# Kuntz-Lab/interactive-rate-tendons

Hardware: AMD Instinct MI355X
Metric: FK+collision checks/sec (3-tendon, 256^3 voxel env) (higher is better)
Workload: dtype f64

## Files before the change

### interactive-rate-tendons_amd/csrc/edge_queue_kernel.hpp

```cpp
#pragma once
#include "verdict_kernel.hpp"
#define TRK_EDGE_DEVICE_ONLY
#include "edge_kernel.hpp"

namespace trk {

__device__ __forceinline__ uint32_t eq_load(const uint32_t *p) { return __hip_atomic_load(p, __ATOMIC_RELAXED, __HIP_MEMORY_SCOPE_AGENT); }
__device__ __forceinline__ void eq_wait_vm() { asm volatile("s_waitcnt vmcnt(0)" ::: "memory"); }
__device__ __forceinline__ void eq_release() {
  eq_wait_vm();
  __builtin_amdgcn_fence(__ATOMIC_RELEASE, "agent");
  eq_wait_vm();
}
__device__ __forceinline__ void eq_acquire() {
  __builtin_amdgcn_fence(__ATOMIC_ACQUIRE, "agent");
  eq_wait_vm();
}
__device__ __forceinline__ int eq_bcast(int v) { return __builtin_amdgcn_readfirstlane(v); }
struct EqClock {
  unsigned long long t;
  __device__ __forceinline__ void start() { t = wall_clock64(); }
  __device__ __forceinline__ void lap(uint32_t *ctl, int word) {
    const unsigned long long n = wall_clock64();
    if (threadIdx.x == 0) __hip_atomic_fetch_add((unsigned long long *)(ctl + word), n - t, __ATOMIC_RELAXED, __HIP_MEMORY_SCOPE_AGENT);
    t = n;
  }
};

constexpr int EQ_GROUP_IV = EQ_MAX_CAND;
#define EQ_MASK(i) (((unsigned long long *)vlds)[(i)])
#define EQ_I(i) (((int32_t *)vlds)[(i)])
#define EQ_U(i) (((uint32_t *)vlds)[(i)])
constexpr int EQ_PRE = 2 * EQ_GROUP_IV / 32, EQ_EOF = EQ_PRE + 64, EQ_BASEOF = EQ_EOF + 64, EQ_CNT = EQ_BASEOF + 64, EQ_DOM = EQ_CNT + 64,
              EQ_NBASE = EQ_DOM + 64, EQ_FILL = EQ_NBASE + 64, EQ_RELW = EQ_FILL + 64;
#define EQ_REL(i) (((double *)vlds)[EQ_RELW / 2 + (i)])

__device__ __forceinline__ int eq_stash_base(int NM) { return VLay<true>::MS + 4 * NM * 64 + SIG_LDS_WORDS; }

__device__ __forceinline__ void signatures_differ_lane2(const uint32_t *__restrict__ ra, const uint32_t *__restrict__ rm,
                                                        const uint32_t *__restrict__ rb, int P, int &fp, int &fd) {
  constexpr int U = 6;
  fp = 0; fd = 0;
  bool open_p = true, open_d = true;
  for (int k = (P - 1) >> 2; k >= 0 && (open_p || open_d); k -= U) {
    uint4 va[U], vm[U], vb[U];
#pragma unroll
    for (int u = 0; u < U; u++) {
      const int kk = k - u >= 0 ? k - u : 0;
      va[u] = *reinterpret_cast<const uint4 *>(ra + 4 * kk);
      vm[u] = *reinterpret_cast<const uint4 *>(rm + 4 * kk);
      vb[u] = *reinterpret_cast<const uint4 *>(rb + 4 * kk);
    }
#pragma unroll
    for (int u = 0; u < U; u++) {
      if (k - u < 0) break;
      const uint32_t wa[4] = {va[u].x, va[u].y, va[u].z, va[u].w}, wm[4] = {vm[u].x, vm[u].y, vm[u].z, vm[u].w},
                     wb[4] = {vb[u].x, vb[u].y, vb[u].z, vb[u].w};
#pragma unroll
      for (int w = 3; w >= 0; w--) {
        if (4 * (k - u) + w >= P) continue;
        const uint32_t a = wa[w], m = wm[w], b = wb[w];
        const uint32_t mx = m & 1023u, my = (m >> 10) & 1023u, mz = (m >> 20) & 1023u;
        const uint32_t px = (a & 1023u) + 1u - mx, py = ((a >> 10) & 1023u) + 1u - my, pz = ((a >> 20) & 1023u) + 1u - mz;
        const uint32_t dx = mx + 1u - (b & 1023u), dy = my + 1u - ((b >> 10) & 1023u), dz = mz + 1u - ((b >> 20) & 1023u);
        const int ep = ((a | m) & SIG_BAD) ? 2 : ((px > 2u || py > 2u || pz > 2u) ? 1 : 0);
        const int ed = ((m | b) & SIG_BAD) ? 2 : ((dx > 2u || dy > 2u || dz > 2u) ? 1 : 0);
        if (open_p && ep) { fp = ep; open_p = false; }
        if (open_d && ed) { fd = ed; open_d = false; }
      }
    }
  }
}

__device__ __forceinline__ bool eq_claim(const EdgeQueueArgs &q, int &pos, int &n) {
  const int lane = threadIdx.x;
  uint32_t *ctl = q.ctl;
  uint32_t seen = 0xffffffffu;
  unsigned idle = 0;
  int patience = 0;
  for (;;) {
    int r_fl = 0, r_pos = 0, r_n = 0, r_end = 0, r_wait = 0;
    uint32_t d = 0, t = 0;
    if (lane == 0) {
      r_fl = (int)eq_load(ctl + EQ_FLAGS);
      d = eq_load(ctl + EQ_DONE);
      eq_wait_vm();
      t = eq_load(ctl + EQ_TAIL);
      const int avail = (int)eq_load(ctl + EQ_AVAIL);
      const int out = (int)(t - d);
      const int want = out >= 4096 ? 64 : (out < 128 ? 1 : out >> 6);
      if (!r_fl && avail > 0 && avail < want && patience < 24) { patience++; r_wait = 1; }
      else if (!r_fl && avail > 0) {
        const int old = (int)__hip_atomic_fetch_add((int *)(ctl + EQ_AVAIL), -want, __ATOMIC_RELAXED, __HIP_MEMORY_SCOPE_AGENT);
        const int got = old >= want ? want : (old > 0 ? old : 0);
        if (got < want) __hip_atomic_fetch_add((int *)(ctl + EQ_AVAIL), want - got, __ATOMIC_RELAXED, __HIP_MEMORY_SCOPE_AGENT);
        if (got > 0) { r_pos = (int)__hip_atomic_fetch_add(ctl + EQ_HEAD, (uint32_t)got, __ATOMIC_RELAXED, __HIP_MEMORY_SCOPE_AGENT); r_n = got; }
      } else if (!r_fl && d == t) r_end = 1;
    }
    if (eq_bcast(r_fl) || eq_bcast(r_end)) return false;
    if (eq_bcast(r_wait)) { __builtin_amdgcn_s_sleep(16); continue; }
    n = eq_bcast(r_n);
    if (n > 0) { pos = eq_bcast(r_pos); return true; }
    d = (uint32_t)eq_bcast((int)d); t = (uint32_t)eq_bcast((int)t);
    if (d + t != seen) { seen = d + t; idle = 0; }
    else if (++idle > (1u << 19)) {
      if (lane == 0) __hip_atomic_fetch_or(ctl + EQ_FLAGS, EQF_STUCK, __ATOMIC_RELAXED, __HIP_MEMORY_SCOPE_AGENT);
      return false;
    }
    __builtin_amdgcn_s_sleep(127);
    if (idle > 16) __builtin_amdgcn_s_sleep(127);
    if (idle > 256) { __builtin_amdgcn_s_sleep(127); __builtin_amdgcn_s_sleep(127); }
  }
}

template <int N, bool ROT>
__global__ __launch_bounds__(64, (N <= TRK_VERDICT_TWO_WAVE_MAXN ? 2 : 1)) void fk_edge_queue(
    RobotK K, const double *__restrict__ tab, const StepK *__restrict__ steps, int nsteps,
    const VerdictArgs *__restrict__ va, const EdgeQueueArgs *__restrict__ qa, const FusedSweepArgs *__restrict__ sa) {
  const int lane = threadIdx.x;
  EqClock clk;
  clk.start();
#ifdef TRK_EQ_TRACE
  int tr_round = 0;
#endif
  for (;;) {
    int zero = 0;
    asm volatile("" : "+s"(zero));
    const EdgeQueueArgs &q = qa[zero];
    int h = 0, cnt = 0;
    if (!eq_claim(q, h, cnt)) break;
    clk.lap(q.ctl, EQ_T_CLAIM);
    const bool live = lane < cnt;
    const int slot = h + lane;
    int e_lane = -1;
    {
      bool bail = false;
      if (live) {
        const uint32_t *flag = (const uint32_t *)q.sample_edge + slot;
        unsigned spins = 0;
        while ((e_lane = (int)eq_load(flag)) < 0) {
          if (eq_load(q.ctl + EQ_FLAGS) != 0u) { bail = true; break; }
          if (++spins > (1u << 22)) {
            __hip_atomic_fetch_or(q.ctl + EQ_FLAGS, EQF_STUCK, __ATOMIC_RELAXED, __HIP_MEMORY_SCOPE_AGENT);
            bail = true; break;
          }
          __builtin_amdgcn_s_sleep(8);
        }
      }
      if (__any(bail)) break;
    }
    eq_acquire();
    clk.lap(q.ctl, EQ_T_READY);

    PointSweep<false, true> ps;
    ps.va = va;
    ps.dn_prev = 0.0f; ps.sph_state = 0u;
    ps.qhead = 0; ps.qcount = 0; ps.active = false;
    ps.P = va->P; ps.CH = va->CH; ps.NM = va->NM; ps.Kl = (ps.P - 1 + ps.CH - 1) / ps.CH; ps.ms_next = 0; ps.ms_k = 0;
    ps.sigst.init(); ps.sig_row_of = -1; ps.sig_first_row = 0; ps.sig_row0 = h; ps.sig_cnt = cnt;
    __syncthreads();
    VL_U(VLay<true>::HIT + lane) = 0u; VL_U(VLay<true>::INPREV + lane) = 0u; VL_F(VLay<true>::DIST + lane) = 0.0f;
    __syncthreads();
    const int S = K.state_size;
    const double *st_eff = q.states + ((int64_t)h - (int64_t)blockIdx.x * 64) * S;
    const int64_t n_eff = (int64_t)blockIdx.x * 64 + cnt;
    {
      const int sb = eq_stash_base(ps.NM);
      VL_I(sb + lane) = e_lane;
      if (lane == 0) { VL_I(sb + 64) = h; VL_I(sb + 65) = cnt; VL_U(sb + 66) = (uint32_t)clk.t; VL_U(sb + 67) = (uint32_t)(clk.t >> 32); }
    }
    FkLane<N> fl_;
    {
      FkOut out{nullptr, nullptr, nullptr, nullptr, nullptr, nullptr, nullptr, nullptr, nullptr, nullptr};
      fk_uniform_body<N, ROT, false, false>(st_eff, n_eff, 0, K, tab, steps, nsteps, out, ps, nullptr, &fl_);
    }
    ps.template sig_finish<false>();
    ps.finish();
    while (ps.qcount > 0) ps.flush();
    __syncthreads();
    LaneVerdict lv;
    int e2, h2, cnt2;
    {
      const VerdictArgs a = *va;
      const int sb = eq_stash_base(a.NM);
      e2 = VL_I(sb + lane); h2 = VL_I(sb + 64); cnt2 = VL_I(sb + 65);
      clk.t = (unsigned long long)VL_U(sb + 66) | ((unsigned long long)VL_U(sb + 67) << 32);
      lv = verdict_decide<N, false, true>(a, fl_, lane < cnt2);
    }
    const bool live2 = lane < cnt2;
    int zero2 = 0;
    asm volatile("" : "+s"(zero2));
    const EdgeQueueArgs &q2 = qa[zero2];
#ifdef TRK_EQ_TRACE
    const uint32_t tr_start = (uint32_t)clk.t;
    const unsigned long long tr_w0 = wall_clock64(), tr_c0 = (unsigned long long)clock64();
    { float x = (float)lane; for (int i = 0; i < 2000; i++) x = __builtin_fmaf(x, 1.0000001f, 0.5f); if (x == 12345.678f) asm volatile("s_nop 0"); }
    const unsigned long long tr_w1 = wall_clock64(), tr_c1 = (unsigned long long)clock64();
    const uint32_t tr_mhz = tr_w1 > tr_w0 ? (uint32_t)((tr_c1 - tr_c0) * 100ull / (tr_w1 - tr_w0)) : 0u;
#endif
    clk.lap(q2.ctl, EQ_T_FK);
#ifdef TRK_EQ_TRACE
    const uint32_t tr_fk = (uint32_t)clk.t;
#endif
    if (__any(lv.pending)) {
      __syncthreads();
      const double *st2 = q2.states + ((int64_t)h2 - (int64_t)blockIdx.x * 64) * K.state_size;
      const int64_t n2 = (int64_t)blockIdx.x * 64 + cnt2;
      fk_uniform_body<N, ROT, false, false>(st2, n2, q2.fb_ld, K, tab, steps, nsteps, q2.fb_out, NoPointHook(), nullptr, nullptr);
      __syncthreads();
      const FusedSweepArgs fa = *sa;
      bool exact = false;
      sweep_body<false>(q2.fb_in, n2, q2.fb_ld, fa.P, fa.CH, fa.NM, K, fa.g, fa.grid, fa.near_grid, 1, fa.debug, nullptr, nullptr, nullptr, &exact);
      __syncthreads();
      const uint32_t npend = (uint32_t)__popcll(__ballot(lv.pending));
      if (lane == 0) __hip_atomic_fetch_add(q2.ctl + EQ_PENDING, npend, __ATOMIC_RELAXED, __HIP_MEMORY_SCOPE_AGENT);
      if (lv.pending) lv.valid = exact;
      clk.lap(q2.ctl, EQ_T_EXACT);
    }

    if (live2 && !lv.valid) q2.edge_ok[e2] = 0u;
    eq_release();
    int old = 0;
    if (live2) old = __hip_atomic_fetch_add(q2.remaining + e2, -1, __ATOMIC_RELAXED, __HIP_MEMORY_SCOPE_AGENT);
    bool fin = live2 && old == 1;
    bool stop = false;
    EqClock sub = clk;
    sub.lap(q2.ctl, EQ_T_F0);
    if (__any(fin)) {
      eq_acquire();
      {
        const uint32_t nfin = (uint32_t)__popcll(__ballot(fin));
        if (lane == 0) __hip_atomic_fetch_add(q2.ctl + EQ_FINISHED, nfin, __ATOMIC_RELAXED, __HIP_MEMORY_SCOPE_AGENT);
      }
      int base_l = 0, ncand_l = 0;
      double rel_l = 0.0;
      if (fin && q2.edge_ok[e2] != 0u) {
        base_l = q2.lvl_base[e2]; ncand_l = q2.lvl_cnt[e2]; rel_l = q2.rel[e2];
        if (2 * ncand_l > EQ_MAX_CAND) {
          __hip_atomic_fetch_or(q2.ctl + EQ_FLAGS, EQF_DEEP, __ATOMIC_RELAXED, __HIP_MEMORY_SCOPE_AGENT);
          ncand_l = 0; stop = true;
        }
      }
      stop = __any(stop);
      sub.lap(q2.ctl, EQ_T_F1);
      unsigned long long todo = __ballot(ncand_l > 0);
      const int P = q2.P;
      const int S2 = q2.sk.S;
      while (todo && !stop) {
        const bool mine = (todo >> lane) & 1ull;
        int pre = mine ? ncand_l : 0;
#pragma unroll
        for (int o = 1; o < 64; o <<= 1) { const int v = __shfl_up(pre, o, 64); if (lane >= o) pre += v; }
        const bool in_group = mine && pre <= EQ_GROUP_IV;
        const unsigned long long gm = __ballot(in_group);
        todo &= ~gm;
        const int n_g = in_group ? ncand_l : 0;
        int ex = n_g;
#pragma unroll
        for (int o = 1; o < 64; o <<= 1) { const int v = __shfl_up(ex, o, 64); if (lane >= o) ex += v; }
        const int T = __shfl(ex, 63, 64);
        ex -= n_g;
        __syncthreads();
        EQ_I(EQ_PRE + lane) = ex; EQ_I(EQ_EOF + lane) = e2; EQ_I(EQ_BASEOF + lane) = base_l;
        EQ_I(EQ_CNT + lane) = 0; EQ_I(EQ_DOM + lane) = 0; EQ_I(EQ_FILL + lane) = 0;
        EQ_REL(lane) = rel_l;
        __syncthreads();
        if (lane == 0) __hip_atomic_fetch_add(q2.ctl + EQ_CAND, (uint32_t)(2 * T), __ATOMIC_RELAXED, __HIP_MEMORY_SCOPE_AGENT);
        auto owner_of = [&](int g) {
          int lo = 0;
#pragma unroll
          for (int st = 32; st > 0; st >>= 1) if (EQ_I(EQ_PRE + lo + st) <= g) lo += st;
          return lo;
        };
        for (int g0 = 0; g0 < T; g0 += 64) {
          const int g = g0 + lane;
          bool emit_p = false, emit_d = false;
          if (g < T) {
#pragma clang fp contract(off)
            const int ow = owner_of(g);
            const int sm = EQ_I(EQ_BASEOF + ow) + (g - EQ_I(EQ_PRE + ow));
            const EdgeIv iv = q2.iv[sm];
            const double tm = (iv.ta + iv.tb) / 2;
            int fp, fd;
            signatures_differ_lane2(q2.sig + (int64_t)iv.sa * q2.sig_stride, q2.sig + (int64_t)sm * q2.sig_stride,
                                    q2.sig + (int64_t)iv.sb * q2.sig_stride, P, fp, fd);
            if (fp == 2 || fd == 2) atomicOr(&EQ_U(EQ_DOM + ow), 1u);
            const double relv = EQ_REL(ow);
            emit_p = fp == 1 && (tm - iv.ta) > relv;
            emit_d = fd == 1 && (iv.tb - tm) > relv;
            const uint32_t k = (emit_p ? 1u : 0u) + (emit_d ? 1u : 0u);
            if (k) atomicAdd(&EQ_U(EQ_CNT + ow), k);
          }
          const unsigned long long mp = __ballot(emit_p), md = __ballot(emit_d);
          if (lane == 0) { EQ_MASK(2 * (g0 >> 6)) = mp; EQ_MASK(2 * (g0 >> 6) + 1) = md; }
        }
        __syncthreads();
        sub.lap(q2.ctl, EQ_T_F2);
        int total_l = 0;
        if (in_group) {
          if (EQ_I(EQ_DOM + lane)) {
            q2.edge_ok[e2] = 0u;
            __hip_atomic_fetch_add(q2.ctl + EQ_DOMAIN, 1u, __ATOMIC_RELAXED, __HIP_MEMORY_SCOPE_AGENT);
          } else total_l = EQ_I(EQ_CNT + lane);
        }
        int nex = total_l;
#pragma unroll
        for (int o = 1; o < 64; o <<= 1) { const int v = __shfl_up(nex, o, 64); if (lane >= o) nex += v; }
        const int Tnew = __shfl(nex, 63, 64);
        nex -= total_l;
        if (Tnew == 0) continue;
        int nb = 0;
        if (lane == 0) nb = (int)__hip_atomic_fetch_add(q2.ctl + EQ_TAIL, (uint32_t)Tnew, __ATOMIC_RELAXED, __HIP_MEMORY_SCOPE_AGENT);
        nb = eq_bcast(nb);
        if (nb + Tnew > q2.slot_hi) {
          if (lane == 0) __hip_atomic_fetch_or(q2.ctl + EQ_FLAGS, EQF_OVERFLOW, __ATOMIC_RELAXED, __HIP_MEMORY_SCOPE_AGENT);
          stop = true; break;
        }
        EQ_I(EQ_NBASE + lane) = nb + nex;
        if (total_l > 0) {
          q2.lvl_base[e2] = nb + nex; q2.lvl_cnt[e2] = total_l; q2.remaining[e2] = total_l;
          q2.nfk[e2] += total_l;
        }
        __syncthreads();
        for (int g0 = 0; g0 < T; g0 += 64) {
          const unsigned long long mp = EQ_MASK(2 * (g0 >> 6)), md = EQ_MASK(2 * (g0 >> 6) + 1);
          const bool ep = (mp >> lane) & 1ull, ed = (md >> lane) & 1ull;
          if (ep || ed) {
#pragma clang fp contract(off)
            const int g = g0 + lane;
            const int ow = owner_of(g);
            if (!EQ_I(EQ_DOM + ow)) {
              const int sm = EQ_I(EQ_BASEOF + ow) + (g - EQ_I(EQ_PRE + ow));
              const EdgeIv iv = q2.iv[sm];
              const double tm = (iv.ta + iv.tb) / 2;
              const int e = EQ_I(EQ_EOF + ow);
              int ns = EQ_I(EQ_NBASE + ow) + (int)atomicAdd(&EQ_U(EQ_FILL + ow), (ep ? 1u : 0u) + (ed ? 1u : 0u));
              if (ed) {
                q2.iv[ns] = EdgeIv{e, sm, iv.sb, 0, tm, iv.tb};
                const double t2 = (tm + iv.tb) / 2;
                interpolate_state_dev(q2.sk, q2.A + (int64_t)e * S2, q2.B + (int64_t)e * S2, t2, q2.states + (int64_t)ns * S2);
                ns++;
              }
              if (ep) {
                q2.iv[ns] = EdgeIv{e, iv.sa, sm, 0, iv.ta, tm};
                const double t2 = (iv.ta + tm) / 2;
                interpolate_state_dev(q2.sk, q2.A + (int64_t)e * S2, q2.B + (int64_t)e * S2, t2, q2.states + (int64_t)ns * S2);
              }
            }
          }
        }
        sub.lap(q2.ctl, EQ_T_F3);
        eq_release();
        for (int g = lane; g < Tnew; g += 64) {
          const int ns = nb + g;
          __hip_atomic_store((uint32_t *)q2.sample_edge + ns, (uint32_t)q2.iv[ns].e, __ATOMIC_RELAXED, __HIP_MEMORY_SCOPE_AGENT);
        }
        eq_wait_vm();
        if (lane == 0) __hip_atomic_fetch_add((int *)(q2.ctl + EQ_AVAIL), Tnew, __ATOMIC_RELAXED, __HIP_MEMORY_SCOPE_AGENT);
        sub.lap(q2.ctl, EQ_T_F4);
      }
    }
// ... 20 lines not shown
```

### interactive-rate-tendons_amd/csrc/fk_inst.hip

```cpp
#include "fk_launch.hpp"
#include "fk_kernel.hpp"
#if TRK_INST_KIND == 1
#include "fk_retract_kernel.hpp"
#elif TRK_INST_KIND == 2
#include "fused_kernel.hpp"
#elif TRK_INST_KIND == 3
#include "verdict_kernel.hpp"
#elif TRK_INST_KIND == 4
#define TRK_WITH_RETRACT_VERDICT
#include "fk_retract_kernel.hpp"
#include "verdict_kernel.hpp"
#elif TRK_INST_KIND == 5
#include "edge_queue_kernel.hpp"
#elif TRK_INST_KIND == 6
#define TRK_LOADED_WITH_INTEGRATOR
#include "fk_loaded_kernel.hpp"
#endif

namespace trk {

#if TRK_INST_KIND == 5
template <> void launch_fk_edge_queue<TRK_INST_N>(const FkLaunch &a, const VerdictArgs *va, size_t lds, const EdgeQueueArgs *qa,
                                                  const FusedSweepArgs *sweep, unsigned waves) {
  if (a.rotation)
    hipLaunchKernelGGL((fk_edge_queue<TRK_INST_N, true>), dim3(waves), dim3(64), lds, a.stream, a.K, a.d_tab, a.d_steps, a.n_steps, va, qa, sweep);
  else
    hipLaunchKernelGGL((fk_edge_queue<TRK_INST_N, false>), dim3(waves), dim3(64), lds, a.stream, a.K, a.d_tab, a.d_steps, a.n_steps, va, qa, sweep);
}
template <> int fk_edge_queue_waves_per_cu<TRK_INST_N>(bool rotation, size_t lds) {
  int nb = 0;
  const hipError_t e = rotation ? hipOccupancyMaxActiveBlocksPerMultiprocessor(&nb, fk_edge_queue<TRK_INST_N, true>, 64, lds)
                                : hipOccupancyMaxActiveBlocksPerMultiprocessor(&nb, fk_edge_queue<TRK_INST_N, false>, 64, lds);
  return e == hipSuccess ? nb : 0;
}
#endif

#if TRK_INST_KIND == 5
#elif TRK_INST_KIND == 6
template <bool ROT, bool WR>
static void go(const FkLaunch &a, const LoadedIn &in) {
  const unsigned grid = (unsigned)((a.n + 63) / 64);
  hipLaunchKernelGGL((fk_loaded_uniform<TRK_INST_N, ROT, WR>), dim3(grid), dim3(64), 0, a.stream, a.d_states, a.n, a.ld, a.K,
                     a.d_tab, a.d_steps, a.n_steps, a.out, in);
}
template <> void launch_fk_loaded<TRK_INST_N>(const FkLaunch &a, const LoadedIn &in) {
  if (a.rotation) { if (a.write_R) go<true, true>(a, in); else go<true, false>(a, in); }
  else            { if (a.write_R) go<false, true>(a, in); else go<false, false>(a, in); }
}
template <> void launch_shoot_start<TRK_INST_N>(const FkLaunch &a, const double *guess, double *vu) {
  const unsigned grid = (unsigned)((a.n + 63) / 64);
  hipLaunchKernelGGL((shoot_start<TRK_INST_N>), dim3(grid), dim3(64), 0, a.stream, a.d_states, a.n, a.K, a.d_tab, guess, vu);
}
#elif TRK_INST_KIND == 4
template <bool ROT, bool SPH, bool SIG>
static void go(const FkLaunch &a, const VerdictArgs *va, size_t lds) {
  const unsigned grid = (unsigned)((a.n + 63) / 64);
  const RetractHandoff ho{a.d_handoff, a.handoff_ld};
  hipLaunchKernelGGL((fk_retract_prologue<TRK_INST_N, ROT>), dim3(grid), dim3(64), 0, a.stream, a.d_states, a.n, a.K, a.d_poly, a.d_tab, a.d_steps,
                     a.n_steps, a.k_first, a.d_tgrid, a.d_hl, a.d_perm, ho);
  hipLaunchKernelGGL((fk_verdict_retract<TRK_INST_N, ROT, SPH, SIG>), dim3(grid), dim3(64), lds, a.stream, a.d_states, a.n, a.K, a.d_poly,
                     a.d_tab, a.d_steps, a.n_steps, a.k_first, a.d_tgrid, a.d_hl, a.out.tips, va, ho);
}
template <bool SPH, bool SIG>
static void go_rot(const FkLaunch &a, const VerdictArgs *va, size_t lds) {
  if (a.rotation) go<true, SPH, SIG>(a, va, lds); else go<false, SPH, SIG>(a, va, lds);
}
template <> void launch_fk_verdict_retract<TRK_INST_N>(const FkLaunch &a, const VerdictArgs *va, size_t lds, bool spheres, bool with_sig) {
  if (spheres) { if (with_sig) go_rot<true, true>(a, va, lds); else go_rot<true, false>(a, va, lds); }
  else         { if (with_sig) go_rot<false, true>(a, va, lds); else go_rot<false, false>(a, va, lds); }
}
template <bool ROT>
static void go_list(const FkLaunch &a, const FusedSweepArgs *sweep, size_t lds, const int32_t *list, const uint32_t *count) {
  const unsigned grid = (unsigned)((a.n + 63) / 64);
  hipLaunchKernelGGL((fk_sweep_retract_list<TRK_INST_N, ROT>), dim3(grid), dim3(64), lds, a.stream, a.d_states, a.n, a.ld, a.K,
                     a.d_poly, a.d_tab, a.d_steps, a.n_steps, a.k_first, a.d_tgrid, a.d_hl, a.out, sweep, list, count);
}
template <> void launch_fk_sweep_retract_list<TRK_INST_N>(const FkLaunch &a, const FusedSweepArgs *sweep, size_t lds, const int32_t *list,
                                                          const uint32_t *count) {
  if (a.rotation) go_list<true>(a, sweep, lds, list, count); else go_list<false>(a, sweep, lds, list, count);
}
#elif TRK_INST_KIND == 3
template <bool ROT, bool SPH, bool SIG>
static void go(const FkLaunch &a, const VerdictArgs *va, size_t lds) {
  const unsigned grid = (unsigned)((a.n + 63) / 64);
  hipLaunchKernelGGL((fk_verdict<TRK_INST_N, ROT, SPH, SIG>), dim3(grid), dim3(64), lds, a.stream, a.d_states, a.n, a.K, a.d_tab, a.d_steps,
                     a.n_steps, a.out.tips, va);
}
template <bool SPH, bool SIG>
static void go_rot(const FkLaunch &a, const VerdictArgs *va, size_t lds) {
  if (a.rotation) go<true, SPH, SIG>(a, va, lds); else go<false, SPH, SIG>(a, va, lds);
}
template <> void launch_fk_verdict<TRK_INST_N>(const FkLaunch &a, const VerdictArgs *va, size_t lds, bool spheres, bool with_sig) {
  if (spheres) { if (with_sig) go_rot<true, true>(a, va, lds); else go_rot<true, false>(a, va, lds); }
  else         { if (with_sig) go_rot<false, true>(a, va, lds); else go_rot<false, false>(a, va, lds); }
}
#elif TRK_INST_KIND == 2
template <bool ROT>
static void go_list(const FkLaunch &a, const FusedSweepArgs *sweep, size_t lds, const int32_t *list, const uint32_t *count) {
  const unsigned grid = (unsigned)((a.n + 63) / 64);
  hipLaunchKernelGGL((fk_sweep_fused_list<TRK_INST_N, ROT>), dim3(grid), dim3(64), lds, a.stream, a.d_states, a.n, a.ld, a.K,
                     a.d_tab, a.d_steps, a.n_steps, a.out, sweep, list, count);
}
template <> void launch_fk_sweep_fused_list<TRK_INST_N>(const FkLaunch &a, const FusedSweepArgs *sweep, size_t lds, const int32_t *list,
                                                        const uint32_t *count) {
  if (a.rotation) go_list<true>(a, sweep, lds, list, count); else go_list<false>(a, sweep, lds, list, count);
}
template <bool ROT>
static void go(const FkLaunch &a, const FusedSweepArgs *sweep, size_t lds) {
  const unsigned grid = (unsigned)((a.n + 63) / 64);
  hipLaunchKernelGGL((fk_sweep_fused<TRK_INST_N, ROT>), dim3(grid), dim3(64), lds, a.stream, a.d_states, a.n, a.ld, a.K,
                     a.d_tab, a.d_steps, a.n_steps, a.out, sweep);
}
template <> void launch_fk_sweep_fused<TRK_INST_N>(const FkLaunch &a, const FusedSweepArgs *sweep, size_t lds) {
  if (a.rotation) go<true>(a, sweep, lds); else go<false>(a, sweep, lds);
}
#else
#if TRK_INST_KIND == 1
template <bool ROT, bool WR>
static void go(const FkLaunch &a) {
  const unsigned grid = (unsigned)((a.n + 63) / 64);
  hipLaunchKernelGGL((fk_rk4_batch_retract<TRK_INST_N, ROT, WR>), dim3(grid), dim3(64), 0, a.stream, a.d_states, a.n, a.ld, a.K,
                     a.d_poly, a.d_tab, a.d_steps, a.n_steps, a.k_first, a.d_tgrid, a.d_hl, a.out, a.d_perm, a.d_wave_k_begin);
}
template <> void launch_fk_retract<TRK_INST_N>(const FkLaunch &a) {
#else
template <bool ROT, bool WR>
static void go(const FkLaunch &a) {
  const unsigned grid = (unsigned)((a.n + 63) / 64);
  hipLaunchKernelGGL((fk_rk4_batch_uniform<TRK_INST_N, ROT, WR>), dim3(grid), dim3(64), 0, a.stream, a.d_states, a.n, a.ld, a.K,
                     a.d_tab, a.d_steps, a.n_steps, a.out);
}
template <> void launch_fk_uniform<TRK_INST_N>(const FkLaunch &a) {
#endif
  if (a.rotation) { if (a.write_R) go<true, true>(a); else go<true, false>(a); }
  else            { if (a.write_R) go<false, true>(a); else go<false, false>(a); }
}
#endif

}
```

### interactive-rate-tendons_amd/csrc/fk_kernel.hpp

```cpp
#pragma once
#include <type_traits>
#include <hip/hip_runtime.h>
#include "tr_types.hpp"

namespace trk {

#ifndef TRK_NEWTON_STEPS
#define TRK_NEWTON_STEPS 1
#endif
__device__ __forceinline__ double fast_rcp(double x) {
  double y = __builtin_amdgcn_rcp(x);
  double e = __builtin_fma(-x, y, 1.0);
  y = __builtin_fma(e, y, y);
#if TRK_NEWTON_STEPS > 1
  e = __builtin_fma(-x, y, 1.0);
  y = __builtin_fma(e, y, y);
#endif
  return y;
}
__device__ __forceinline__ double fast_rsqrt(double x) {
  double y = __builtin_amdgcn_rsq(x);
  double hx = 0.5 * x;
  double t = __builtin_fma(-hx * y, y, 0.5);
  y = __builtin_fma(y, t, y);
#if TRK_NEWTON_STEPS > 1
  t = __builtin_fma(-hx * y, y, 0.5);
  y = __builtin_fma(y, t, y);
#endif
  return y;
}

struct NoLoad {
  __device__ __forceinline__ void operator()(double &, double &, double &, double &, double &, double &) const {}
};

template <int N, class Route, class Load = NoLoad>
__device__ __forceinline__ void strain_rates_routed(const double v[3], const double u[3], const double (&tau)[N],
                                                    Route &&route, const RobotK &K,
                                                    double dv[3], double du[3], double (&sdot)[N], const Load &load = Load()) {
#pragma clang fp contract(fast)
  double Axx = K.ks0, Axy = 0, Axz = 0, Ayy = K.ks0, Ayz = 0, Azz = K.ks2, Z = 0;
  double B00 = 0, B01 = 0, B02 = 0, B10 = 0, B11 = 0, B12 = 0, B20 = 0, B21 = 0, B22 = 0;
  double Hxx = K.kb0, Hxy = 0, Hxz = 0, Hyy = K.kb0, Hyz = 0, Hzz = K.kb2;
  double ax = 0, ay = 0, az = 0, bx = 0, by = 0, bz = 0;
#pragma unroll
  for (int j = 0; j < N; j++) {
    double r6[6];
    route(j, r6);
    const double rx = r6[0], ry = r6[1];
    const double rdx = r6[2], rdy = r6[3];
    const double rddx = r6[4], rddy = r6[5];
    const double pdx = (v[0] + rdx) - u[2] * ry;
    const double pdy = (v[1] + rdy) + u[2] * rx;
    const double pdz = __builtin_fma(u[0], ry, __builtin_fma(-u[1], rx, v[2]));
    const double sxy = __builtin_fma(pdy, pdy, pdx * pdx), s2 = __builtin_fma(pdz, pdz, sxy);
    const double rs = fast_rsqrt(s2);
    sdot[j] = s2 * rs;
    const double cs2 = -tau[j] * rs;
    const double rs2 = rs * rs, c = cs2 * rs2;
    const double qx = c * pdx, qy = c * pdy, qz = c * pdz;
    Axx += qx * pdx; Axy += qx * pdy; Axz += qx * pdz; Ayy += qy * pdy; Ayz += qy * pdz;
    Z += cs2;
    const double ez = __builtin_fma(rx, pdy, -(ry * pdx));
    const double gx = ry * qz, gy = -rx * qz, gz = c * ez;
    B00 += gx * pdx; B01 += gx * pdy;
    B10 += gy * pdx; B11 += gy * pdy;
    B20 += gz * pdx; B21 += gz * pdy; B22 += gz * pdz;
    Hxz += gx * ez; Hyz += gy * ez; Hzz += gz * ez;
    const double mxy = c * sxy, mx = mxy * rx, my = mxy * ry;
    Hxx -= my * ry; Hxy += mx * ry; Hyy -= mx * rx;
    const double t1 = cs2 * rx, t2 = cs2 * ry;
    Hzz -= t1 * rx; Hzz -= t2 * ry;
    {
#pragma clang fp contract(off)
      Azz -= mxy; B02 -= my; B12 += mx; B20 += t2; B21 -= t1;
    }
    const double hx = pdx + rdx, hy = pdy + rdy, hz = pdz;
    const double wx = __builtin_fma(u[1], hz, __builtin_fma(-u[2], hy, rddx));
    const double wy = __builtin_fma(u[2], hx, __builtin_fma(-u[0], hz, rddy));
    const double wz = __builtin_fma(u[0], hy, -(u[1] * hx));
    const double pw = __builtin_fma(pdz, wz, __builtin_fma(pdy, wy, pdx * wx));
    const double kp = pw * rs2;
    const double px = __builtin_fma(pdx, kp, -wx), py = __builtin_fma(pdy, kp, -wy), pz = __builtin_fma(pdz, kp, -wz);
    ax = __builtin_fma(cs2, px, ax); ay = __builtin_fma(cs2, py, ay); az = __builtin_fma(cs2, pz, az);
    bx = __builtin_fma(t2, pz, bx); by = __builtin_fma(-t1, pz, by); bz = __builtin_fma(t1, py, __builtin_fma(-t2, px, bz));
  }
#define TRK_FMA __builtin_fma
  const double svx = K.ks0 * v[0], svy = K.ks0 * v[1], svz = K.ks2 * (v[2] - 1.0);
  const double dku = K.dkb * u[2], w = TRK_FMA(-K.ks0, v[2], svz);
  double cx = TRK_FMA(-u[1], dku, TRK_FMA(-v[1], w, -bx));
  double cy = TRK_FMA(u[0], dku, TRK_FMA(v[0], w, -by));
  double cz = -bz;
  double dx = TRK_FMA(u[2], svy, TRK_FMA(-u[1], svz, -ax));
  double dy = TRK_FMA(u[0], svz, TRK_FMA(-u[2], svx, -ay));
  double dz = TRK_FMA(u[1], svx, TRK_FMA(-u[0], svy, -az));
  load(cx, cy, cz, dx, dy, dz);
  const double m00 = Axx - Z, m01 = Axy, m02 = Axz, m11 = Ayy - Z, m12 = Ayz, m22 = Azz;
#ifndef TRK_SOLVE_SCHUR
  {
#pragma clang fp contract(off)
    const double n00 = Hxx, n01 = Hxy, n02 = Hxz, n11 = Hyy, n12 = Hyz, n22 = Hzz;
    const double p0 = m00;
    const double r0 = fast_rcp(p0);
    const double w10 = m01, l10 = w10 * r0;
    const double w20 = m02, l20 = w20 * r0;
    const double w30 = B00, l30 = w30 * r0;
    const double w40 = B10, l40 = w40 * r0;
    const double w50 = B20, l50 = w50 * r0;
    const double p1 = TRK_FMA(-l10, w10, m11);
    const double r1 = fast_rcp(p1);
    const double w21 = TRK_FMA(-l20, w10, m12), l21 = w21 * r1;
    const double w31 = TRK_FMA(-l30, w10, B01), l31 = w31 * r1;
    const double w41 = TRK_FMA(-l40, w10, B11), l41 = w41 * r1;
    const double w51 = TRK_FMA(-l50, w10, B21), l51 = w51 * r1;
    const double p2 = TRK_FMA(-l21, w21, TRK_FMA(-l20, w20, m22));
    const double r2 = fast_rcp(p2);
    const double w32 = TRK_FMA(-l31, w21, TRK_FMA(-l30, w20, B02)), l32 = w32 * r2;
    const double w42 = TRK_FMA(-l41, w21, TRK_FMA(-l40, w20, B12)), l42 = w42 * r2;
    const double w52 = TRK_FMA(-l51, w21, TRK_FMA(-l50, w20, B22)), l52 = w52 * r2;
    const double p3 = TRK_FMA(-l32, w32, TRK_FMA(-l31, w31, TRK_FMA(-l30, w30, n00)));
    const double r3 = fast_rcp(p3);
    const double w43 = TRK_FMA(-l42, w32, TRK_FMA(-l41, w31, TRK_FMA(-l40, w30, n01))), l43 = w43 * r3;
    const double w53 = TRK_FMA(-l52, w32, TRK_FMA(-l51, w31, TRK_FMA(-l50, w30, n02))), l53 = w53 * r3;
    const double p4 = TRK_FMA(-l43, w43, TRK_FMA(-l42, w42, TRK_FMA(-l41, w41, TRK_FMA(-l40, w40, n11))));
    const double r4 = fast_rcp(p4);
    const double w54 = TRK_FMA(-l53, w43, TRK_FMA(-l52, w42, TRK_FMA(-l51, w41, TRK_FMA(-l50, w40, n12)))), l54 = w54 * r4;
    const double p5 = TRK_FMA(-l54, w54, TRK_FMA(-l53, w53, TRK_FMA(-l52, w52, TRK_FMA(-l51, w51, TRK_FMA(-l50, w50, n22)))));
    const double r5 = fast_rcp(p5);
    const double y0 = dx;
    const double y1 = TRK_FMA(-l10, y0, dy);
    const double y2 = TRK_FMA(-l21, y1, TRK_FMA(-l20, y0, dz));
    const double y3 = TRK_FMA(-l32, y2, TRK_FMA(-l31, y1, TRK_FMA(-l30, y0, cx)));
    const double y4 = TRK_FMA(-l43, y3, TRK_FMA(-l42, y2, TRK_FMA(-l41, y1, TRK_FMA(-l40, y0, cy))));
    const double y5 = TRK_FMA(-l54, y4, TRK_FMA(-l53, y3, TRK_FMA(-l52, y2, TRK_FMA(-l51, y1, TRK_FMA(-l50, y0, cz)))));
    const double x5 = y5 * r5;
    const double x4 = TRK_FMA(-l54, x5, y4 * r4);
    const double x3 = TRK_FMA(-l53, x5, TRK_FMA(-l43, x4, y3 * r3));
    const double x2 = TRK_FMA(-l52, x5, TRK_FMA(-l42, x4, TRK_FMA(-l32, x3, y2 * r2)));
    const double x1 = TRK_FMA(-l51, x5, TRK_FMA(-l41, x4, TRK_FMA(-l31, x3, TRK_FMA(-l21, x2, y1 * r1))));
    const double x0 = TRK_FMA(-l50, x5, TRK_FMA(-l40, x4, TRK_FMA(-l30, x3, TRK_FMA(-l20, x2, TRK_FMA(-l10, x1, y0 * r0)))));
    dv[0] = x0; dv[1] = x1; dv[2] = x2; du[0] = x3; du[1] = x4; du[2] = x5;
  }
#else
  const double c00 = TRK_FMA(m11, m22, -(m12 * m12)), c01 = TRK_FMA(m02, m12, -(m01 * m22)), c02 = TRK_FMA(m01, m12, -(m02 * m11));
  const double c11 = TRK_FMA(m00, m22, -(m02 * m02)), c12 = TRK_FMA(m01, m02, -(m00 * m12)), c22 = TRK_FMA(m00, m11, -(m01 * m01));
  const double idet = fast_rcp(TRK_FMA(m00, c00, TRK_FMA(m01, c01, m02 * c02)));
  const double i00 = c00 * idet, i01 = c01 * idet, i02 = c02 * idet, i11 = c11 * idet, i12 = c12 * idet, i22 = c22 * idet;
  const double yx = TRK_FMA(i00, dx, TRK_FMA(i01, dy, i02 * dz));
  const double yy_ = TRK_FMA(i01, dx, TRK_FMA(i11, dy, i12 * dz));
  const double yz = TRK_FMA(i02, dx, TRK_FMA(i12, dy, i22 * dz));
  const double T00 = TRK_FMA(B00, i00, TRK_FMA(B01, i01, B02 * i02)), T01 = TRK_FMA(B00, i01, TRK_FMA(B01, i11, B02 * i12)),
               T02 = TRK_FMA(B00, i02, TRK_FMA(B01, i12, B02 * i22));
  const double T10 = TRK_FMA(B10, i00, TRK_FMA(B11, i01, B12 * i02)), T11 = TRK_FMA(B10, i01, TRK_FMA(B11, i11, B12 * i12)),
               T12 = TRK_FMA(B10, i02, TRK_FMA(B11, i12, B12 * i22));
  const double T20 = TRK_FMA(B20, i00, TRK_FMA(B21, i01, B22 * i02)), T21 = TRK_FMA(B20, i01, TRK_FMA(B21, i11, B22 * i12)),
               T22 = TRK_FMA(B20, i02, TRK_FMA(B21, i12, B22 * i22));
  const double s00 = TRK_FMA(-T02, B02, TRK_FMA(-T01, B01, TRK_FMA(-T00, B00, Hxx)));
  const double s01 = TRK_FMA(-T02, B12, TRK_FMA(-T01, B11, TRK_FMA(-T00, B10, Hxy)));
  const double s02 = TRK_FMA(-T02, B22, TRK_FMA(-T01, B21, TRK_FMA(-T00, B20, Hxz)));
  const double s11 = TRK_FMA(-T12, B12, TRK_FMA(-T11, B11, TRK_FMA(-T10, B10, Hyy)));
  const double s12 = TRK_FMA(-T12, B22, TRK_FMA(-T11, B21, TRK_FMA(-T10, B20, Hyz)));
  const double s22 = TRK_FMA(-T22, B22, TRK_FMA(-T21, B21, TRK_FMA(-T20, B20, Hzz)));
  const double ex = TRK_FMA(-B02, yz, TRK_FMA(-B01, yy_, TRK_FMA(-B00, yx, cx)));
  const double ey = TRK_FMA(-B12, yz, TRK_FMA(-B11, yy_, TRK_FMA(-B10, yx, cy)));
  const double ez = TRK_FMA(-B22, yz, TRK_FMA(-B21, yy_, TRK_FMA(-B20, yx, cz)));
  const double g00 = TRK_FMA(s11, s22, -(s12 * s12)), g01 = TRK_FMA(s02, s12, -(s01 * s22)), g02 = TRK_FMA(s01, s12, -(s02 * s11));
  const double g11 = TRK_FMA(s00, s22, -(s02 * s02)), g12 = TRK_FMA(s01, s02, -(s00 * s12)), g22 = TRK_FMA(s00, s11, -(s01 * s01));
  const double isd = fast_rcp(TRK_FMA(s00, g00, TRK_FMA(s01, g01, s02 * g02)));
  du[0] = TRK_FMA(g00, ex, TRK_FMA(g01, ey, g02 * ez)) * isd;
  du[1] = TRK_FMA(g01, ex, TRK_FMA(g11, ey, g12 * ez)) * isd;
  du[2] = TRK_FMA(g02, ex, TRK_FMA(g12, ey, g22 * ez)) * isd;
  dv[0] = TRK_FMA(-T20, du[2], TRK_FMA(-T10, du[1], TRK_FMA(-T00, du[0], yx)));
  dv[1] = TRK_FMA(-T21, du[2], TRK_FMA(-T11, du[1], TRK_FMA(-T01, du[0], yy_)));
  dv[2] = TRK_FMA(-T22, du[2], TRK_FMA(-T12, du[1], TRK_FMA(-T02, du[0], yz)));
#endif
#undef TRK_FMA
}

template <int N, class Load = NoLoad>
__device__ __forceinline__ void strain_rates(const double v[3], const double u[3], const double (&tau)[N],
                                             const double *__restrict__ ri, const RobotK &K,
                                             double dv[3], double du[3], double (&sdot)[N], const Load &load = Load()) {
  strain_rates_routed<N>(v, u, tau, [&](int j, double (&r6)[6]) {
#pragma unroll
    for (int q = 0; q < 6; q++) r6[q] = ri[6 * j + q];
  }, K, dv, du, sdot, load);
}

template <int N>
__device__ __forceinline__ void initial_bending(const double (&tau)[N], const double *__restrict__ rb,
                                                const RobotK &K, double v[3], double u[3], bool &converged) {
#pragma clang fp contract(off)
  v[0] = 0; v[1] = 0; v[2] = 1;
  u[0] = 0; u[1] = 0; u[2] = 0;
  bool done = false;
  for (int it = 0; it < 1000; ++it) {
    if (!__any(!done)) break;
    double Fx = 0, Fy = 0, Fz = 0, Lx = 0, Ly = 0, Lz = 0;
#pragma unroll
    for (int k = 0; k < N; k++) {
      const double rx = rb[6 * k + 0], ry = rb[6 * k + 1], rdx = rb[6 * k + 2], rdy = rb[6 * k + 3];
      double px = (-u[2] * ry) + rdx + v[0];
      double py = (u[2] * rx) + rdy + v[1];
      double pz = (u[0] * ry - u[1] * rx) + v[2];
      const double z = px * px + py * py + pz * pz;
      if (z > 0.0) { const double s = sqrt(z); px = px / s; py = py / s; pz = pz / s; }
      Fx -= tau[k] * px; Fy -= tau[k] * py; Fz -= tau[k] * pz;
      const double trx = tau[k] * rx, try_ = tau[k] * ry;
      Lx -= try_ * pz; Ly -= (-trx) * pz; Lz -= ((-try_) * px + trx * py);
    }
    const double nx = K.ks0 * v[0], ny = K.ks0 * v[1], nz = K.ks2 * (v[2] - 1);
    const double mx = K.kb0 * u[0], my = K.kb0 * u[1], mz = K.kb2 * u[2];
    const double e1 = (nx - Fx) * (nx - Fx) + (ny - Fy) * (ny - Fy) + (nz - Fz) * (nz - Fz);
    const double e2 = (mx - Lx) * (mx - Lx) + (my - Ly) * (my - Ly) + (mz - Lz) * (mz - Lz);
    const double residual = sqrt(e1 + e2);
    if (!done && residual < K.residual_threshold) done = true;
    const double vnx = K.iks0 * Fx, vny = K.iks0 * Fy, vnz = K.iks2 * Fz + 1;
    const double unx = K.ikb0 * Lx, uny = K.ikb0 * Ly, unz = K.ikb2 * Lz;
    if (!done) {
      const double dvn = sqrt((vnx - v[0]) * (vnx - v[0]) + (vny - v[1]) * (vny - v[1]) + (vnz - v[2]) * (vnz - v[2]));
      const double dun = sqrt((unx - u[0]) * (unx - u[0]) + (uny - u[1]) * (uny - u[1]) + (unz - u[2]) * (unz - u[2]));
      const double vn = sqrt(v[0] * v[0] + v[1] * v[1] + v[2] * v[2]);
      const double un = sqrt(u[0] * u[0] + u[1] * u[1] + u[2] * u[2]);
      if (dvn < 1e-9 * vn && dun < 1e-9 * un) done = true;
    }
    if (!done) { v[0] = vnx; v[1] = vny; v[2] = vnz; u[0] = unx; u[1] = uny; u[2] = unz; }
  }
  {
    double Fx = 0, Fy = 0, Fz = 0, Lx = 0, Ly = 0, Lz = 0;
#pragma unroll
    for (int k = 0; k < N; k++) {
      const double rx = rb[6 * k + 0], ry = rb[6 * k + 1], rdx = rb[6 * k + 2], rdy = rb[6 * k + 3];
      double px = (u[1] * 0.0 - u[2] * ry) + rdx + v[0];
      double py = (u[2] * rx - u[0] * 0.0) + rdy + v[1];
      double pz = (u[0] * ry - u[1] * rx) + 0.0 + v[2];
      const double z = px * px + py * py + pz * pz;
      if (z > 0.0) { const double s = sqrt(z); px = px / s; py = py / s; pz = pz / s; }
      const double fx = -tau[k] * px, fy = -tau[k] * py, fz = -tau[k] * pz;
      Fx += fx; Fy += fy; Fz += fz;
      Lx += ry * fz - 0.0 * fy; Ly += 0.0 * fx - rx * fz; Lz += rx * fy - ry * fx;
    }
    const double nx = K.ks0 * v[0], ny = K.ks0 * v[1], nz = K.ks2 * (v[2] - 1);
    const double mx = K.kb0 * u[0], my = K.kb0 * u[1], mz = K.kb2 * u[2];
    const double e1 = (nx - Fx) * (nx - Fx) + (ny - Fy) * (ny - Fy) + (nz - Fz) * (nz - Fz);
    const double e2 = (mx - Lx) * (mx - Lx) + (my - Ly) * (my - Ly) + (mz - Lz) * (mz - Lz);
    converged = sqrt(e1 + e2) <= K.residual_threshold;
  }
}

__device__ __forceinline__ void position_quadrature(int st, const double (&sR)[9], const double (&sv)[3], double b1,
                                                    double (&qs)[3], double (&qm)[3], double (&p)[3]) {
#pragma unroll
  for (int c = 0; c < 3; c++) {
    const double r0 = sR[c], r1 = sR[3 + c], r2 = sR[6 + c];
    if (st == 0) qs[c] = __builtin_fma(r2, sv[2], __builtin_fma(r1, sv[1], r0 * sv[0]));
    else if (st == 1) qm[c] = __builtin_fma(r2, sv[2], __builtin_fma(r1, sv[1], r0 * sv[0]));
    else if (st == 2) {
      qm[c] = __builtin_fma(r2, sv[2], __builtin_fma(r1, sv[1], __builtin_fma(r0, sv[0], qm[c])));
      qs[c] = __builtin_fma(2.0, qm[c], qs[c]);
    } else {
      qs[c] = __builtin_fma(r2, sv[2], __builtin_fma(r1, sv[1], __builtin_fma(r0, sv[0], qs[c])));
      p[c] = __builtin_fma(b1, qs[c], p[c]);
    }
  }
}

__device__ __forceinline__ void frame_rate(int st, const double (&sR)[9], const double (&su)[3], double (&dR)[9], double (&aR)[9]) {
#pragma clang fp contract(fast)
#pragma unroll
  for (int r = 0; r < 3; r++) {
    const double r0 = sR[0 + r], r1 = sR[3 + r], r2 = sR[6 + r];
    if (st < 3) {
      dR[0 + r] = __builtin_fma(r1, su[2], -(r2 * su[1]));
      dR[3 + r] = __builtin_fma(r2, su[0], -(r0 * su[2]));
      dR[6 + r] = __builtin_fma(r0, su[1], -(r1 * su[0]));
#pragma unroll
      for (int c = 0; c < 9; c += 3) aR[c + r] = (st == 0) ? dR[c + r] : __builtin_fma(2.0, dR[c + r], aR[c + r]);
    } else {
      aR[0 + r] = __builtin_fma(r1, su[2], __builtin_fma(-r2, su[1], aR[0 + r]));
      aR[3 + r] = __builtin_fma(r2, su[0], __builtin_fma(-r0, su[2], aR[3 + r]));
      aR[6 + r] = __builtin_fma(r0, su[1], __builtin_fma(-r1, su[0], aR[6 + r]));
    }
  }
}

template <int N, class Route>
__device__ __forceinline__ void rk4_step_routed(double (&R)[9], double (&v)[3], double (&u)[3], double (&p)[3], double &Lb,
                                                double (&Li)[N], const double (&tau)[N], const RobotK &K, double t, double h,
                                                Route &&route) {
#pragma clang fp contract(fast)
  const double hh = h * 0.5;
  const double b1 = h * (1.0 / 6.0), b2 = h * (1.0 / 3.0);
  double aR[9], av[3], au[3];
#pragma unroll
  for (int q = 0; q < 3; q++) { av[q] = v[q]; au[q] = u[q]; }
  double sR[9], sv[3], su[3], qs[3], qm[3];
#pragma unroll
  for (int q = 0; q < 9; q++) sR[q] = R[q];
#pragma unroll
  for (int q = 0; q < 3; q++) { sv[q] = v[q]; su[q] = u[q]; }
#pragma unroll
  for (int st = 0; st < 4; st++) {
    double ts = (st == 0) ? t : ((st == 3) ? t + h : t + hh);
    asm volatile("" : "+v"(ts) : "v"(sv[0]), "v"(su[0]));
    const double bw = (st == 0 || st == 3) ? b1 : b2;
    const double aw = (st == 2) ? h : hh;
    double dv[3], du[3], sd[N];
    strain_rates_routed<N>(sv, su, tau, [&](int j, double (&r6)[6]) { route(ts, j, r6); }, K, dv, du, sd);
    position_quadrature(st, sR, sv, b1, qs, qm, p);
    {
      const double v2 = __builtin_fma(sv[2], sv[2], __builtin_fma(sv[1], sv[1], sv[0] * sv[0]));
      Lb += bw * (v2 * fast_rsqrt(v2));
    }
#pragma unroll
    for (int j = 0; j < N; j++) Li[j] += bw * sd[j];
    double dR[9];
    frame_rate(st, sR, su, dR, aR);
#pragma unroll
    for (int q = 0; q < 3; q++) { av[q] += bw * dv[q]; au[q] += bw * du[q]; }
    if (st < 3) {
#pragma unroll
      for (int q = 0; q < 9; q++) sR[q] = R[q] + aw * dR[q];
#pragma unroll
      for (int q = 0; q < 3; q++) { sv[q] = v[q] + aw * dv[q]; su[q] = u[q] + aw * du[q]; }
    }
  }
#pragma unroll
  for (int q = 0; q < 9; q++) R[q] = __builtin_fma(b1, aR[q], R[q]);
#pragma unroll
  for (int q = 0; q < 3; q++) { v[q] = av[q]; u[q] = au[q]; }
}


template <int N>
struct FkLane {
  bool converged;
  double Li[N];
  double tip[3];
};

struct NoPointHook {
  __device__ __forceinline__ void begin(bool) const {}
  __device__ __forceinline__ void operator()(int, double, double, double) const {}
  __device__ __forceinline__ void tip_point(int, bool, bool, double, double, double, bool = true) const {}
};

template <class H, class = void> struct HookLiInLds { static constexpr int from = 1 << 30; };
template <class H> struct HookLiInLds<H, std::void_t<decltype(H::kLiInLdsFrom)>> { static constexpr int from = H::kLiInLdsFrom; };
template <class OnPoint> __host__ __device__ constexpr bool li_in_lds(int N) {
  return N >= HookLiInLds<std::remove_cv_t<std::remove_reference_t<OnPoint>>>::from && N <= 4;
}

template <int N, bool ROT, bool WRITE_R, bool WANT_L = true, class OnPoint = NoPointHook>
__device__ __forceinline__ void fk_uniform_body(
    const double *__restrict__ states, int64_t n, int64_t ld, const RobotK &K,
    const double *__restrict__ tab, const StepK *__restrict__ steps, int nsteps, const FkOut &out,
    OnPoint &&on_point = NoPointHook(), const int32_t *__restrict__ row_map = nullptr, FkLane<N> *lane_out = nullptr) {
#pragma clang fp contract(fast)
  const int64_t i = (int64_t)blockIdx.x * 64 + threadIdx.x;
  const bool live = i < n;
  const int64_t il = live ? i : (n - 1);
  const int64_t ic = row_map ? (int64_t)row_map[il] : il;
  const int S = K.state_size;
  double tau[N];
#pragma unroll
  for (int j = 0; j < N; j++) tau[j] = states[ic * S + j];
  constexpr bool kLiLds = li_in_lds<OnPoint>(N);
  double *li_lds = nullptr;
  if constexpr (kLiLds) {
    __shared__ double li_lds_store[N * 64];
    li_lds = li_lds_store;
#pragma unroll
    for (int j = 0; j < N; j++) li_lds[j * 64 + threadIdx.x] = 0.0;
  }
  double rc = 1.0, rs = 0.0, r22 = 1.0;
  if (ROT) {
    const double th = states[ic * S + N];
    rs = sin(th); rc = cos(th);
    r22 = (1.0 - rc) + rc;
  }

  double v[3], u[3];
  bool conv;
  initial_bending<N>(tau, tab, K, v, u, conv);
  on_point.begin(conv && live);

  double R[9] = {1, 0, 0, 0, 1, 0, 0, 0, 1};
  double p[3] = {0, 0, 0};
  double Lb = 0;
  double Li[N];
#pragma unroll
  for (int j = 0; j < N; j++) Li[j] = 0;

  auto store_point = [&](int j) {
    const int64_t o = (int64_t)j * ld + i;
    double x = p[0], y = p[1], z = p[2];
    if (ROT) { const double x2 = __builtin_fma(rc, x, -(rs * y)), y2 = __builtin_fma(rs, x, rc * y); x = x2; y = y2; z = r22 * z; }
    on_point(j, x, y, z);
    if (!live) return;
    if (out.px) { out.px[o] = x; out.py[o] = y; out.pz[o] = z; }
    if (WRITE_R) {
      const int64_t PS = (int64_t)K.n_points * ld;
#pragma unroll
      for (int c = 0; c < 3; c++) {
        double a = R[c * 3 + 0], b = R[c * 3 + 1], cc = R[c * 3 + 2];
        if (ROT) { const double a2 = rc * a - rs * b, b2 = rs * a + rc * b; a = a2; b = b2; cc = r22 * cc; }
        out.R[(c * 3 + 0) * PS + o] = a; out.R[(c * 3 + 1) * PS + o] = b; out.R[(c * 3 + 2) * PS + o] = cc;
      }
    }
  };
  store_point(0);

  for (int k = 0; k < nsteps; k++) {
    const double h = steps[k].h;
    const int obs = steps[k].obs;
    const double *__restrict__ rt = tab + (size_t)(1 + 3 * k) * (N * 6);
    const double hh = h * 0.5;
    const double b1 = h * (1.0 / 6.0), b2 = h * (1.0 / 3.0);
    double aR[9], av[3], au[3];
#pragma unroll
    for (int q = 0; q < 3; q++) { av[q] = v[q]; au[q] = u[q]; }
    double sR[9], sv[3], su[3];
    double qs[3], qm[3];
#pragma unroll
    for (int q = 0; q < 9; q++) sR[q] = R[q];
#pragma unroll
    for (int q = 0; q < 3; q++) { sv[q] = v[q]; su[q] = u[q]; }

#pragma unroll
    for (int st = 0; st < 4; st++) {
      const double *__restrict__ ri = rt + (st == 0 ? 0 : (st == 3 ? 2 : 1)) * (N * 6);
      const double bw = (st == 0 || st == 3) ? b1 : b2;
      const double aw = (st == 2) ? h : hh;
      double dv[3], du[3], sd[N];
      strain_rates<N>(sv, su, tau, ri, K, dv, du, sd);
      position_quadrature(st, sR, sv, b1, qs, qm, p);
      if (WANT_L && out.L) {
        const double v2 = __builtin_fma(sv[2], sv[2], __builtin_fma(sv[1], sv[1], sv[0] * sv[0]));
        Lb += bw * (v2 * fast_rsqrt(v2));
      }
      if constexpr (kLiLds) {
#pragma unroll
        for (int j = 0; j < N; j++) li_lds[j * 64 + threadIdx.x] += bw * sd[j];
      } else {
#pragma unroll
        for (int j = 0; j < N; j++) Li[j] += bw * sd[j];
      }
      double dR[9];
      frame_rate(st, sR, su, dR, aR);
#pragma unroll
      for (int q = 0; q < 3; q++) { av[q] += bw * dv[q]; au[q] += bw * du[q]; }
      if (st < 3) {
#pragma unroll
        for (int q = 0; q < 9; q++) sR[q] = R[q] + aw * dR[q];
#pragma unroll
        for (int q = 0; q < 3; q++) { sv[q] = v[q] + aw * dv[q]; su[q] = u[q] + aw * du[q]; }
      }
    }
#pragma unroll
    for (int q = 0; q < 9; q++) R[q] = __builtin_fma(b1, aR[q], R[q]);
#pragma unroll
    for (int q = 0; q < 3; q++) { v[q] = av[q]; u[q] = au[q]; }
    if (obs >= 0) store_point(obs);
  }

  if constexpr (kLiLds) {
#pragma unroll
    for (int j = 0; j < N; j++) Li[j] = li_lds[j * 64 + threadIdx.x];
  }
  if (live) {
    if (out.L) out.L[i] = Lb;
    if (out.Li) {
#pragma unroll
      for (int j = 0; j < N; j++) out.Li[(int64_t)j * ld + i] = Li[j];
    }
    if (out.converged) out.converged[i] = conv ? 1 : 0;
    if (out.n_points) out.n_points[i] = K.n_points;
    if (out.tips) {
      double x = p[0], y = p[1], z = p[2];
      if (ROT) { const double x2 = __builtin_fma(rc, x, -(rs * y)), y2 = __builtin_fma(rs, x, rc * y); x = x2; y = y2; z = r22 * z; }
      out.tips[3 * i + 0] = x; out.tips[3 * i + 1] = y; out.tips[3 * i + 2] = z;
    }
  }
  if (lane_out) {
    lane_out->converged = conv;
#pragma unroll
    for (int j = 0; j < N; j++) lane_out->Li[j] = Li[j];
    double x = p[0], y = p[1], z = p[2];
    if (ROT) { const double x2 = __builtin_fma(rc, x, -(rs * y)), y2 = __builtin_fma(rs, x, rc * y); x = x2; y = y2; z = r22 * z; }
    lane_out->tip[0] = x; lane_out->tip[1] = y; lane_out->tip[2] = z;
  }
}

template <int N, bool ROT, bool WRITE_R>
__global__ __launch_bounds__(64, (N <= TRK_K1_TWO_WAVE_MAXN ? 2 : 1)) void fk_rk4_batch_uniform(
    const double *__restrict__ states, int64_t n, int64_t ld, RobotK K,
    const double *__restrict__ tab, const StepK *__restrict__ steps, int nsteps, FkOut out) {
  fk_uniform_body<N, ROT, WRITE_R>(states, n, ld, K, tab, steps, nsteps, out);
}

}
```

### interactive-rate-tendons_amd/csrc/fk_launch.hpp

```cpp
#pragma once
#include <hip/hip_runtime.h>
#include "tr_types.hpp"

namespace trk {

struct FkLaunch {
  const double *d_states; int64_t n, ld;
  RobotK K;
  bool rotation, write_R;
  const double *d_tab; const StepK *d_steps; int n_steps;
  const PolyK *d_poly; int k_first; const double *d_tgrid, *d_hl;
  FkOut out;
  hipStream_t stream;
  double *d_handoff = nullptr; int64_t handoff_ld = 0; const int32_t *d_perm = nullptr;
  const int32_t *d_wave_k_begin = nullptr;
};

struct LoadedIn {
  const double *wrench; int64_t wrench_ld;
  const double *dist; int64_t dist_ld;
  const double *vu;
  const int32_t *list;
  int32_t Q;
  const double *tip_route;
  double *res; int64_t ldr;
  double *vu_tip;
};

struct FusedSweepArgs;
struct VerdictArgs;
struct EdgeQueueArgs;
template <int N> void launch_fk_uniform(const FkLaunch &a);
template <int N> void launch_fk_sweep_fused(const FkLaunch &a, const FusedSweepArgs *sweep, size_t lds);
template <int N> void launch_fk_sweep_fused_list(const FkLaunch &a, const FusedSweepArgs *sweep, size_t lds, const int32_t *list,
                                                 const uint32_t *count);
template <int N> void launch_fk_verdict(const FkLaunch &a, const VerdictArgs *va, size_t lds, bool spheres, bool with_sig);
template <int N> void launch_fk_retract(const FkLaunch &a);
template <int N> void launch_fk_verdict_retract(const FkLaunch &a, const VerdictArgs *va, size_t lds, bool spheres, bool with_sig);
template <int N> void launch_fk_sweep_retract_list(const FkLaunch &a, const FusedSweepArgs *sweep, size_t lds, const int32_t *list,
                                                   const uint32_t *count);

template <int N> void launch_fk_edge_queue(const FkLaunch &a, const VerdictArgs *va, size_t lds, const EdgeQueueArgs *qa,
                                           const FusedSweepArgs *sweep, unsigned waves);
template <int N> int fk_edge_queue_waves_per_cu(bool rotation, size_t lds);

template <int N> void launch_fk_loaded(const FkLaunch &a, const LoadedIn &in);
template <int N> void launch_shoot_start(const FkLaunch &a, const double *guess, double *vu);

#define TRK_DECL_FK(N) template <> void launch_fk_uniform<N>(const FkLaunch &); template <> void launch_fk_retract<N>(const FkLaunch &); \
  template <> void launch_fk_loaded<N>(const FkLaunch &, const LoadedIn &); template <> void launch_shoot_start<N>(const FkLaunch &, const double *, double *); \
  template <> void launch_fk_sweep_fused<N>(const FkLaunch &, const FusedSweepArgs *, size_t); \
  template <> void launch_fk_sweep_fused_list<N>(const FkLaunch &, const FusedSweepArgs *, size_t, const int32_t *, const uint32_t *); \
  template <> void launch_fk_verdict<N>(const FkLaunch &, const VerdictArgs *, size_t, bool, bool); \
  template <> void launch_fk_verdict_retract<N>(const FkLaunch &, const VerdictArgs *, size_t, bool, bool); \
  template <> void launch_fk_sweep_retract_list<N>(const FkLaunch &, const FusedSweepArgs *, size_t, const int32_t *, const uint32_t *); \
  template <> void launch_fk_edge_queue<N>(const FkLaunch &, const VerdictArgs *, size_t, const EdgeQueueArgs *, const FusedSweepArgs *, unsigned); \
  template <> int fk_edge_queue_waves_per_cu<N>(bool, size_t);
TRK_DECL_FK(1) TRK_DECL_FK(2) TRK_DECL_FK(3) TRK_DECL_FK(4) TRK_DECL_FK(5) TRK_DECL_FK(6) TRK_DECL_FK(7) TRK_DECL_FK(8)
#undef TRK_DECL_FK

}
```

### interactive-rate-tendons_amd/csrc/fused_kernel.hpp

```cpp
#pragma once
#include "fk_kernel.hpp"
#define TRK_DEVICE_BODIES_ONLY
#ifndef TRK_K2_PF
#define TRK_K2_PF 8
#endif
#include "sweep_kernel.hpp"

namespace trk {

#ifndef TRK_FUSED_TWO_WAVE_MAXN
#define TRK_FUSED_TWO_WAVE_MAXN 5
#endif

struct FusedKernargs {
  const double *states; int64_t n, ld; RobotK K; const double *tab; const StepK *steps; int nsteps; FkOut out;
  const FusedSweepArgs *sa;
};
static_assert(alignof(RobotK) == 8 && alignof(FkOut) == 8 && sizeof(FusedKernargs) == 24 + sizeof(RobotK) + 24 + sizeof(FkOut) + 8,
              "FusedKernargs must mirror the parameter list of fk_sweep_fused");
typedef const __attribute__((address_space(4))) FusedKernargs *FusedKernargsPtr;
__device__ __forceinline__ FusedKernargsPtr fused_kernargs() {
  FusedKernargsPtr p = (FusedKernargsPtr)__builtin_amdgcn_kernarg_segment_ptr();
  asm volatile("" : "+s"(p));
  return p;
}

template <int N, bool ROT>
__global__ __launch_bounds__(64, (N <= TRK_FUSED_TWO_WAVE_MAXN ? 2 : 1)) void fk_sweep_fused(
    const double *__restrict__ states, int64_t n, int64_t ld, RobotK K, const double *__restrict__ tab,
    const StepK *__restrict__ steps, int nsteps, FkOut out, const FusedSweepArgs *__restrict__ sa) {
  SignatureHook hook{sa, n, sa->sig != nullptr, {}};
  hook.st.init();
  fk_uniform_body<N, ROT, false, false>(states, n, ld, K, tab, steps, nsteps, out, hook);
  hook.finish();
  __syncthreads();
  const FusedKernargsPtr ka = fused_kernargs();
  const FusedSweepArgs a = *ka->sa;
  sweep_body<false>(a.in, ka->n, ka->ld, a.P, a.CH, a.NM, ka->K, a.g, a.grid, a.near_grid, a.check_voxels, a.debug, a.valid_bits, a.flags);
}

template <int N, bool ROT>
__global__ __launch_bounds__(64, (N <= TRK_FUSED_TWO_WAVE_MAXN ? 2 : 1)) void fk_sweep_fused_list(
    const double *__restrict__ states, int64_t cap, int64_t ld, RobotK K, const double *__restrict__ tab,
    const StepK *__restrict__ steps, int nsteps, FkOut out, const FusedSweepArgs *__restrict__ sa,
    const int32_t *__restrict__ list, const uint32_t *__restrict__ count) {
  const int64_t total = (int64_t)*count;
  for (int64_t offset = 0; offset < total; offset += cap) {
    const int64_t left = total - offset;
    const int64_t m = left < cap ? left : cap;
    if ((int64_t)blockIdx.x * 64 >= m) break;
    fk_uniform_body<N, ROT, false, false>(states, m, ld, K, tab, steps, nsteps, out, NoPointHook(), list + offset);
    __syncthreads();
    const FusedKernargsPtr ka = fused_kernargs();
    const FusedSweepArgs a = *ka->sa;
    sweep_body<false>(a.in, m, ka->ld, a.P, a.CH, a.NM, ka->K, a.g, a.grid, a.near_grid, a.check_voxels, a.debug, a.valid_bits, a.flags, list + offset);
    __syncthreads();
  }
}

}
```

### interactive-rate-tendons_amd/csrc/tendon_hip.hip

```cpp
#include <hip/hip_runtime.h>
#include <sched.h>

#include <algorithm>
#include <cfloat>
#include <cmath>
#include <cstdio>
#include <cstdlib>
#include <cstring>
#include <functional>
#include <chrono>
#include <thread>
#include <ctime>
#include <limits>
#include <mutex>
#include <string>
#include <vector>

#include "../../include/tendon_hip.h"
#include "tr_types.hpp"
#include "fk_launch.hpp"
#include "fk_lin_launch.hpp"
#include "sweep_kernel.hpp"
#include "sphere_kernel.hpp"
#include "verdict_kernel.hpp"
#include "edge_kernel.hpp"
#include "edge_plan.hpp"
#include "knn_kernel.hpp"
#include "cache_merge.hpp"
#include "env_kernel.hpp"
#include "sample.hpp"
#include "ik_kernel.hpp"
#include "fk_loaded_kernel.hpp"
#include "loaded_edge_kernel.hpp"
#include "loaded_roadmap_kernel.hpp"
#include "loaded_ik_kernel.hpp"

void tr_dev_cache_trim();
struct tr_ctx;
namespace { void ik_release(tr_ctx *c); }
namespace { void shoot_release(tr_ctx *c); }
namespace { void ikl_release(tr_ctx *c); }

namespace {

std::string g_create_error;

struct Workspace {
  int64_t ld = 0;
  double *px = nullptr, *py = nullptr, *pz = nullptr, *acc = nullptr;
  double *Li = nullptr;
  double *homeLi = nullptr;
  int32_t *np = nullptr;
  uint8_t *conv = nullptr;
  int64_t st_cap = 0;
  double *states = nullptr;
  uint64_t *bits = nullptr;
  double *tips = nullptr;
  uint8_t *flags = nullptr;
  double *L = nullptr;
  int32_t *npts = nullptr;
};

struct EventPair { hipEvent_t a, b; };

constexpr int64_t kRetractSortMin = 8192;
constexpr int64_t kSmallBatch = 4096;

struct EdgeDev {
  int64_t cap = 0;
  double *lvl_states = nullptr;
  uint64_t *bits = nullptr;
  int32_t *sample_edge = nullptr;
  double *sample_t = nullptr;
  trk::EdgeIv *open = nullptr, *frontier = nullptr;
  double *A = nullptr, *B = nullptr, *rel = nullptr;
  uint32_t *edge_ok = nullptr; int32_t *nfk = nullptr;
  unsigned long long *first_inv = nullptr, *last_t = nullptr;
  uint32_t *nd = nullptr; int64_t *cnt = nullptr;
  uint32_t *sig = nullptr; int64_t sig_stride = 0;
  int32_t *sig_np = nullptr;
  trk::EdgeIv *open2 = nullptr; double *lvl_states2 = nullptr;
  int32_t *q_remaining = nullptr, *q_lvl_base = nullptr, *q_lvl_cnt = nullptr;
  uint32_t *q_ctl = nullptr, *q_hctl = nullptr;
  trk::EdgeQueueArgs *q_args = nullptr, *q_hargs = nullptr;
  double *ix_states = nullptr; int64_t ix_states_cap = 0;
  int32_t *ix_idx = nullptr; int64_t ix_idx_cap = 0;
};

}

struct tr_ctx {
  std::recursive_mutex mu;
  int device = 0;
  std::string err;
  RobotK K{};
  std::vector<double> C, D, max_tension;
  std::vector<double> t;
  std::vector<StepK> steps;
  double *d_tab = nullptr;
  StepK *d_steps = nullptr;
  PolyK *d_poly = nullptr;
  double *d_tgrid = nullptr;
  double *d_hl = nullptr;
  int k_first = 0;
  bool has_grid = false;
  GridK G{};
  uint64_t *d_grid = nullptr;
  uint64_t *d_near = nullptr;
  uint32_t n_blocks = 0;
  int checker = TR_CHECKER_BACKBONE;
  float *d_sph_near = nullptr, *d_sph_tmp = nullptr;
  bool sph_near_valid = false;
  uint64_t *d_envw[2] = {nullptr, nullptr};
  uint32_t envw_blocks = 0;
  Workspace ws;
  EdgeDev edge;
  trk::MergeScratch merge;
  int64_t max_chunk = 1 << 20;
  int64_t edge_pool_max = 1 << 22;
  int64_t edge_slots_max = 1 << 24;
  int64_t edge_slots_now = 0;
  double ch_scale = 2.0;
  int64_t k1_round = 1 << 17;
  int fuse = 2;
  int64_t fb_cap = 1 << 17;
  struct RetractOrder {
    uint32_t *keys[2] = {nullptr, nullptr}; int32_t *vals[2] = {nullptr, nullptr}; int64_t cap = 0;
    int32_t *kbegin = nullptr;
    double *handoff = nullptr; int64_t handoff_cap = 0;
    trk::MergeScratch ms;
  };
  static constexpr int kMaxLanes = edge_plan::kMaxLanes;
  struct EdgeLaneDev {
    hipStream_t stream = nullptr;
    uint32_t *hc = nullptr;
    uint32_t *counters = nullptr;
    int32_t *fb_list = nullptr; uint32_t *fb_count = nullptr; int64_t fb_list_cap = 0;
    RetractOrder ro;
  } lane[kMaxLanes];
  int edge_lanes = kMaxLanes;
  bool edge_lanes_fixed = false;
  bool edge_kernels_loaded = false;
  bool edge_queue = true;
  bool edge_queue_forced = false;
  int edge_queue_waves = 0;
  uint32_t edge_queue_last[4] = {0, 0, 0, 0};
  double edge_rate_seen = 0.0;
  bool edge_lane_guess_forced = false;
  double edge_lane_guess = 6.0;
  int64_t retract_sort_min = kRetractSortMin;
  bool rows_one_step = false;
  bool retract_wave_start = true;
  struct VerdictRing {
    static constexpr int kSlots = 16;
    trk::VerdictArgs *d_slots = nullptr, *h_slots = nullptr;
    hipEvent_t ev[kSlots];
    bool used[kSlots] = {};
    int next = 0;
  } vring;
  struct FusedRing {
    static constexpr int kSlots = 16;
    trk::FusedSweepArgs *d_slots = nullptr, *h_slots = nullptr;
    hipEvent_t ev[kSlots];
    bool used[kSlots] = {};
    int next = 0;
  } fused;
  struct KnnScratch { void *p[13] = {}; size_t cap[13] = {}; } knn;
  struct VoxStore { uint32_t *ids = nullptr; uint64_t *masks = nullptr; int64_t cap = 0, n = 0; } vstore;
  uint32_t *d_vids = nullptr; uint64_t *d_vmasks = nullptr; int32_t *d_vcounts = nullptr;
  uint64_t *d_vbits = nullptr;
  int64_t vox_cap = 0;
  int32_t *d_item_src = nullptr, *d_item_edge = nullptr; int64_t vox_items_cap = 0;
  struct Pipe {
    bool ready = false;
    int64_t chunk = 0;
    hipStream_t s_up = nullptr, s_comp = nullptr, s_down = nullptr;
    double *h_states[2] = {nullptr, nullptr}; double *h_tips[2] = {nullptr, nullptr};
    uint64_t *h_bits[2] = {nullptr, nullptr}; uint8_t *h_flags[2] = {nullptr, nullptr};
    hipEvent_t up[2], done[2], down[2];
  } pipe;
  hipEvent_t last_dev_ev = nullptr;
  bool last_dev_used = false;
  hipStream_t last_dev_stream = nullptr;
  struct Sampler {
    int64_t cap = 0;
    double *states = nullptr; uint64_t *bits = nullptr; double *tips = nullptr; uint32_t *wprefix = nullptr;
    uint32_t *wprefix2 = nullptr; int64_t wp2_cap = 0;
    trk::SampleCounters *d_ctr = nullptr, *h_ctr = nullptr;
    int64_t out_cap = 0;
    double *out_states = nullptr, *out_tips = nullptr; int64_t *out_index = nullptr;
    double rate_seen = 0.0;
    uint32_t *sig = nullptr; int64_t sig_cap = 0;
    int64_t *sig_index = nullptr; int64_t sig_index_cap = 0;
  } samp;
  void *h_stage = nullptr; size_t h_stage_cap = 0;
  struct IkDev {
    int64_t probs = 0, lanes = 0;
    double *xs = nullptr, *tips = nullptr;
    double *p = nullptr, *pn = nullptr, *f = nullptr, *J = nullptr, *des = nullptr;
    double *err2 = nullptr, *mu = nullptr, *nu = nullptr;
    int32_t *iters = nullptr, *calls = nullptr, *list[2] = {nullptr, nullptr};
    uint32_t *d_count = nullptr, *h_count = nullptr;
    double *io_s = nullptr, *io_3 = nullptr, *io_e = nullptr;
    int32_t *io_i = nullptr, *io_c = nullptr;
  } ik;
  struct ShootDev {
    int64_t probs = 0, lanes = 0;
    double *xs = nullptr, *res = nullptr;
    double *p = nullptr, *pn = nullptr, *e = nullptr, *J = nullptr;
    double *err2 = nullptr, *mu = nullptr, *nu = nullptr;
    int32_t *iters = nullptr, *calls = nullptr, *list[2] = {nullptr, nullptr};
    uint32_t *d_count = nullptr, *h_count = nullptr;
    double *tip_route = nullptr, *zero6 = nullptr;
    int64_t io_probs = 0, io_R_probs = 0;
    double *io_states = nullptr, *io_w = nullptr, *io_d = nullptr, *io_g = nullptr;
    double *io_px = nullptr, *io_py = nullptr, *io_pz = nullptr, *io_R = nullptr, *io_L = nullptr, *io_Li = nullptr;
    double *io_vu = nullptr, *io_vuL = nullptr, *io_e = nullptr;
    int32_t *io_np = nullptr, *io_it = nullptr, *io_fc = nullptr;
    uint8_t *io_conv = nullptr;
  } shoot;
  struct LoadedEdgeDev {
    int64_t cap = 0, n_vertices = 0;
    double *vu_pool = nullptr, *w = nullptr, *d = nullptr, *g = nullptr;
    int32_t *calls = nullptr;
    unsigned long long *tally = nullptr;
    int64_t last[4] = {0, 0, 0, 0};
    double *out_vu = nullptr; int64_t *out_index = nullptr; int64_t out_cap = 0;
    unsigned long long *vtally = nullptr;
    double rate_seen = 0.0;
  } ledge;
  struct IklDev {
    int64_t probs = 0, lanes = 0;
    double *lin = nullptr;
    double *p = nullptr, *pn = nullptr, *y = nullptr, *W = nullptr, *J = nullptr, *f = nullptr, *des = nullptr;
    double *err2 = nullptr, *mu = nullptr, *nu = nullptr;
    int32_t *iters = nullptr, *calls = nullptr, *list[2] = {nullptr, nullptr};
    uint8_t *eq = nullptr;
    double *row_s = nullptr, *row_w = nullptr, *row_d = nullptr, *row_g = nullptr, *row_vu = nullptr;
    uint8_t *row_conv = nullptr; int32_t *row_calls = nullptr;
    uint32_t *d_count = nullptr, *h_count = nullptr;
    double *io_s = nullptr, *io_3 = nullptr, *io_g = nullptr, *io_e = nullptr, *io_vu = nullptr;
    int32_t *io_i = nullptr, *io_c = nullptr;
    uint8_t *io_eq = nullptr;
  } ikl;
  int64_t loaded_vertex_batch = 0;
  int64_t shoot_chunk = 0;
  bool profiling = false;
  std::vector<EventPair> events[TR_PROFILE_SLOTS];
  uint32_t debug = 0;
};

namespace {

int fail(tr_ctx *ctx, int code, const std::string &msg) {
  if (ctx) ctx->err = msg; else g_create_error = msg;
  return code;
}

#define HIP_TRY(ctx, expr)                                                                   \
  do {                                                                                       \
    hipError_t e_ = (expr);                                                                  \
    if (e_ != hipSuccess)                                                                    \
      return fail(ctx, TR_ERR_HIP, std::string(#expr) + ": " + hipGetErrorString(e_));       \
  } while (0)

std::vector<double> t_range(double start, double end, double dt) {
  std::vector<double> vals;
  for (double p = start; p <= end - (dt / 2); p += dt) vals.push_back(p);
  vals.push_back(end);
  for (auto &v : vals) v = end - (v - start);
  std::reverse(vals.begin(), vals.end());
  return vals;
}

void routing_at(const tr_ctx *c, double t, double *out) {
  const int N_a = c->K.n_a, N_m = c->K.n_m, N_s = std::max(N_a, N_m);
  double S[TRK_MAX_COEF], Sd[TRK_MAX_COEF], Sdd[TRK_MAX_COEF];
  S[0] = 1; Sd[0] = 0; Sdd[0] = 0;
  if (N_s >= 2) { S[1] = t; Sd[1] = 1; Sdd[1] = 0; }
  for (int i = 2; i < N_s; i++) { S[i] = t * S[i - 1]; Sd[i] = i * S[i - 1]; Sdd[i] = i * (i - 1) * S[i - 2]; }
  for (int j = 0; j < c->K.n_tendons; j++) {
    const double *Cj = &c->C[(size_t)j * N_a], *Dj = &c->D[(size_t)j * N_m];
    double C_a = 0, C_ad = 0, C_add = 0, D_m = 0, D_md = 0, D_mdd = 0;
    for (int i = 0; i < N_a; i++) { C_a += Cj[i] * S[i]; C_ad += Cj[i] * Sd[i]; C_add += Cj[i] * Sdd[i]; }
    for (int i = 0; i < N_m; i++) { D_m += Dj[i] * S[i]; D_md += Dj[i] * Sd[i]; D_mdd += Dj[i] * Sdd[i]; }
    const double sa = std::sin(C_a), ca = std::cos(C_a);
    double *o = out + 6 * j;
    o[0] = D_m * sa;
    o[1] = D_m * ca;
    o[2] = D_md * sa + D_m * (ca * C_ad);
    o[3] = D_md * ca + D_m * (-sa * C_ad);
    o[4] = D_mdd * sa + 2 * D_md * (ca * C_ad) - D_m * (sa * C_ad * C_ad) + D_m * (ca * C_add);
    o[5] = D_mdd * ca + 2 * D_md * (-sa * C_ad) - D_m * (ca * C_ad * C_ad) + D_m * (-sa * C_add);
  }
}

int poly_degree(const double *c, int n) {
  for (int i = n - 1; i > 0; i--) if (std::fabs(c[i]) > 0.0) return i;
  return 0;
}
double poly_at(const double *c, int n, double t) {
  double val = 0.0, tpow = 1;
  for (int i = 0; i < n; i++) { val += c[i] * tpow; tpow *= t; }
  return val;
}

void home_lengths(const tr_ctx *c, const std::vector<double> &t, double s_start, double *Li) {
  const double Lh = c->K.L - s_start;
  const int N_a = c->K.n_a, N_m = c->K.n_m;
  for (int j = 0; j < c->K.n_tendons; j++) {
    const double *Cj = &c->C[(size_t)j * N_a], *Dj = &c->D[(size_t)j * N_m];
    const int rdeg = poly_degree(Dj, N_m), tdeg = poly_degree(Cj, N_a);
    if (rdeg == 0 && tdeg == 0) {
      Li[j] = Lh;
    } else if (rdeg == 0 && tdeg == 1) {
      const double d0 = Dj[0], c1 = Cj[1];
      Li[j] = Lh * std::sqrt(1 + d0 * d0 * c1 * c1);
    } else {
      double Cdot[TRK_MAX_COEF] = {0}, Ddot[TRK_MAX_COEF] = {0};
      for (int k = 1; k < N_a; k++) Cdot[k - 1] = k * Cj[k];
      for (int k = 1; k < N_m; k++) Ddot[k - 1] = k * Dj[k];
      const int n = (int)t.size();
      std::vector<double> vals(n);
      for (int q = 0; q < n; q++) {
        const double dd = poly_at(Ddot, N_m, t[q]), d = poly_at(Dj, N_m, t[q]), cd = poly_at(Cdot, N_a, t[q]);
        vals[q] = std::sqrt(dd * dd + (d * d) * (cd * cd) + 1);
      }
      const double dx = c->K.dL;
      double res = 0.0;
      if (n >= 2) {
        int nint = n - 1;
        double odd = 0.0;
        if (nint % 2 != 0) { odd = 0.5 * dx * (vals[n - 2] + vals[n - 1]); nint--; }
        if (nint == 0) res = odd;
        else {
          double integral = vals[0] + vals[nint];
          for (int i = 1; i < nint; i++) integral += ((i % 2) ? 4 : 2) * vals[i];
          res = odd + (integral * dx / 3.0);
        }
      }
      Li[j] = res;
    }
  }
}

int64_t round_up(int64_t x, int64_t m) { return (x + m - 1) / m * m; }

template <typename T>
int dev_alloc(tr_ctx *ctx, T **p, size_t count) {
  if (*p) { (void)hipFree(*p); *p = nullptr; }
  if (count == 0) count = 1;
  hipError_t e = hipMalloc((void **)p, count * sizeof(T));
  if (e == hipErrorOutOfMemory) {
    (void)hipGetLastError();
    tr_dev_cache_trim();
    e = hipMalloc((void **)p, count * sizeof(T));
  }
  HIP_TRY(ctx, e);
  return TR_OK;
}

int vstore_append(tr_ctx *c, const uint32_t *d_ids, const uint64_t *d_masks, int64_t count) {
  tr_ctx::VoxStore &v = c->vstore;
  if (count <= 0) return TR_OK;
  if (v.n + count > v.cap) {
    const int64_t ncap = std::max<int64_t>({v.n + count, 2 * v.cap, (int64_t)1 << 22});
    uint32_t *ni = nullptr; uint64_t *nm = nullptr;
    HIP_TRY(c, hipMalloc((void **)&ni, (size_t)ncap * sizeof(uint32_t)));
    if (hipMalloc((void **)&nm, (size_t)ncap * sizeof(uint64_t)) != hipSuccess) { (void)hipFree(ni); return fail(c, TR_ERR_HIP, "hipMalloc failed (block-list store)"); }
    if (v.n > 0) {
      HIP_TRY(c, hipMemcpyAsync(ni, v.ids, (size_t)v.n * sizeof(uint32_t), hipMemcpyDeviceToDevice, nullptr));
      HIP_TRY(c, hipMemcpyAsync(nm, v.masks, (size_t)v.n * sizeof(uint64_t), hipMemcpyDeviceToDevice, nullptr));
    }
    HIP_TRY(c, hipStreamSynchronize(nullptr));
    if (v.ids) (void)hipFree(v.ids);
    if (v.masks) (void)hipFree(v.masks);
    v.ids = ni; v.masks = nm; v.cap = ncap;
  }
  HIP_TRY(c, hipMemcpyAsync(v.ids + v.n, d_ids, (size_t)count * sizeof(uint32_t), hipMemcpyDeviceToDevice, nullptr));
  HIP_TRY(c, hipMemcpyAsync(v.masks + v.n, d_masks, (size_t)count * sizeof(uint64_t), hipMemcpyDeviceToDevice, nullptr));
  v.n += count;
  return TR_OK;
}

int ensure_workspace(tr_ctx *ctx, int64_t n) {
  Workspace &w = ctx->ws;
  const int64_t want = round_up(std::min<int64_t>(std::max<int64_t>(n, 64), ctx->max_chunk), 64);
  if (w.ld >= want) return TR_OK;
  HIP_TRY(ctx, hipDeviceSynchronize());
  const size_t P = (size_t)ctx->K.n_points, N = (size_t)ctx->K.n_tendons;
  int rc;
  if ((rc = dev_alloc(ctx, &w.px, P * want))) return rc;
  if ((rc = dev_alloc(ctx, &w.py, P * want))) return rc;
  if ((rc = dev_alloc(ctx, &w.pz, P * want))) return rc;
  if ((rc = dev_alloc(ctx, &w.acc, P * want))) return rc;
  if ((rc = dev_alloc(ctx, &w.Li, N * want))) return rc;
  if ((rc = dev_alloc(ctx, &w.conv, (size_t)want))) return rc;
  if (ctx->K.enable_retraction) {
    if ((rc = dev_alloc(ctx, &w.homeLi, N * want))) return rc;
    if ((rc = dev_alloc(ctx, &w.np, (size_t)want))) return rc;
  }
  w.ld = want;
  return TR_OK;
}

int ensure_staging(tr_ctx *ctx, int64_t n) {
  Workspace &w = ctx->ws;
  const int64_t want = round_up(std::max<int64_t>(n, 64), 64);
  if (w.st_cap >= want) return TR_OK;
  HIP_TRY(ctx, hipDeviceSynchronize());
  int rc;
  if ((rc = dev_alloc(ctx, &w.states, (size_t)want * ctx->K.state_size))) return rc;
  if ((rc = dev_alloc(ctx, &w.bits, (size_t)want / 64))) return rc;
  if ((rc = dev_alloc(ctx, &w.tips, (size_t)want * 3))) return rc;
  if ((rc = dev_alloc(ctx, &w.flags, (size_t)want))) return rc;
  if ((rc = dev_alloc(ctx, &w.L, (size_t)want))) return rc;
  if ((rc = dev_alloc(ctx, &w.npts, (size_t)want))) return rc;
  w.st_cap = want;
  return TR_OK;
}

int upload_staged(tr_ctx *c, void *d_dst, const void *h_src, size_t bytes, hipStream_t s) {
  if (bytes == 0) return TR_OK;
  if (bytes % 8) return fail(c, TR_ERR_INVALID_ARG, "upload_staged: whole 8-byte words only");
  if (c->h_stage_cap < bytes) {
    if (c->h_stage) { HIP_TRY(c, hipDeviceSynchronize()); (void)hipHostFree(c->h_stage); c->h_stage = nullptr; c->h_stage_cap = 0; }
    const size_t want = bytes + bytes / 4;
    HIP_TRY(c, hipHostMalloc(&c->h_stage, want, hipHostMallocDefault));
    c->h_stage_cap = want;
  }
  std::memcpy(c->h_stage, h_src, bytes);
  const int64_t words = (int64_t)(bytes / 8);
  hipLaunchKernelGGL(trk::copy_words, dim3((unsigned)std::min<int64_t>((words + 255) / 256, 2048)), dim3(256), 0, s, (uint64_t *)d_dst,
                     (const uint64_t *)c->h_stage, words);
  HIP_TRY(c, hipGetLastError());
  HIP_TRY(c, hipStreamSynchronize(s));
  return TR_OK;
}

int download_staged(tr_ctx *c, void *h_dst, const void *d_src, size_t bytes, hipStream_t s) {
  if (bytes == 0) return TR_OK;
  const size_t padded = (bytes + 7) / 8 * 8;
  if (c->h_stage_cap < padded) {
    if (c->h_stage) { HIP_TRY(c, hipDeviceSynchronize()); (void)hipHostFree(c->h_stage); c->h_stage = nullptr; c->h_stage_cap = 0; }
    const size_t want = padded + padded / 4;
    HIP_TRY(c, hipHostMalloc(&c->h_stage, want, hipHostMallocDefault));
    c->h_stage_cap = want;
  }
// ... 185 lines not shown
  const int64_t fcol = lane * ctx->fb_cap;
  tr_ctx::VerdictRing &vr = ctx->vring;
  if (!vr.d_slots) {
    HIP_TRY(ctx, hipMalloc((void **)&vr.d_slots, sizeof(trk::VerdictArgs) * tr_ctx::VerdictRing::kSlots));
    HIP_TRY(ctx, hipHostMalloc((void **)&vr.h_slots, sizeof(trk::VerdictArgs) * tr_ctx::VerdictRing::kSlots, hipHostMallocDefault));
    for (auto &e : vr.ev) HIP_TRY(ctx, hipEventCreateWithFlags(&e, hipEventDisableTiming));
  }
  const int vslot = vr.next;
  vr.next = (vr.next + 1) % tr_ctx::VerdictRing::kSlots;
  if (vr.used[vslot]) HIP_TRY(ctx, hipEventSynchronize(vr.ev[vslot]));
  trk::VerdictArgs &a = vr.h_slots[vslot];
  a = trk::VerdictArgs{};
  size_t lds_k2;
  sweep_geometry(ctx, a.CH, a.NM, lds_k2);
  a.P = ctx->K.n_points; a.debug = ctx->debug;
  a.g = ctx->G; a.grid = ctx->d_grid; a.near_grid = ctx->d_near; a.valid_bits = d_bits; a.flags = d_flags;
  {
    const GridK &g = ctx->G;
    a.box[0] = g.xmin + 1e-6 * (g.xmax - g.xmin); a.box[1] = g.xmax - 1e-6 * (g.xmax - g.xmin);
    a.box[2] = g.ymin + 1e-6 * (g.ymax - g.ymin); a.box[3] = g.ymax - 1e-6 * (g.ymax - g.ymin);
    a.box[4] = g.zmin + 1e-6 * (g.zmax - g.zmin); a.box[5] = g.zmax - 1e-6 * (g.zmax - g.zmin);
  }
  a.fb_list = fb_list; a.fb_count = fb_count;
  a.sig = sig; a.sig_stride = sig_stride; a.np_out = np_out;
  a.radius = ctx->K.radius;
  for (int j = 0; j < TRK_MAX_TENDONS; j++) { a.home_Li[j] = ctx->K.home_Li[j]; a.min_len[j] = ctx->K.min_len[j]; a.max_len[j] = ctx->K.max_len[j]; }
  if (spheres) {
    a.field = ctx->d_sph_near; a.radius = ctx->K.radius;
    a.r_lo = (float)ctx->K.radius - 2e-6f; a.r_hi = (float)ctx->K.radius + 2e-6f;
  }
  if (ctx->K.enable_retraction && ctx->retract_sort_min > 0 && n >= ctx->retract_sort_min) {
    tr_ctx::RetractOrder &ro = ctx->lane[lane].ro;
    if ((rc = ensure_lane_order(ctx, lane, round_up(n, 64)))) return rc;
    const hipError_t e = trk::retraction_order(order_scratch(ctx, lane), d_states, n, ctx->K.state_size, ctx->K.L, ro.keys, ro.vals, &a.perm, s,
                                               ctx->K.dL, ctx->k_first, ctx->rows_one_step, ro.kbegin);
    a.wave_k_begin = ctx->retract_wave_start ? ro.kbegin : nullptr;
    if (e != hipSuccess) return fail(ctx, TR_ERR_HIP, std::string("retraction order: ") + hipGetErrorString(e));
    HIP_TRY(ctx, hipMemsetAsync(d_bits, 0, (size_t)((n + 63) / 64) * sizeof(uint64_t), s));
  }
  a.finish_hot();
  HIP_TRY(ctx, hipMemcpyAsync(vr.d_slots + vslot, &a, sizeof(a), hipMemcpyHostToDevice, s));
  HIP_TRY(ctx, hipMemsetAsync(fb_count, 0, sizeof(uint32_t), s));
  const bool ret = ctx->K.enable_retraction;
  const trk::FusedSweepArgs *d_fargs; size_t lds_f; int fslot;
  if ((rc = fused_args_slot(ctx, ws_sweep_in(ctx, fcol), spheres ? 2 : 1, d_bits, d_flags, s, &d_fargs, &lds_f, &fslot))) return rc;
  const trk::FkOut vout{nullptr, nullptr, nullptr, nullptr, nullptr, nullptr, d_tips, nullptr, nullptr, nullptr};
  trk::FkLaunch vl{d_states, n, 0, ctx->K, (bool)ctx->K.enable_rotation, false, ctx->d_tab, ctx->d_steps,
                   (int)ctx->steps.size(), ctx->d_poly, ctx->k_first, ctx->d_tgrid, ctx->d_hl, vout, s};
  if (ctx->K.enable_retraction) {
    tr_ctx::RetractOrder &ro = ctx->lane[lane].ro;
    const int64_t hld = round_up(n, 64);
    if (ro.handoff_cap < hld) {
      HIP_TRY(ctx, hipDeviceSynchronize());
      const int64_t want = hld + hld / 8;
      if ((rc = dev_alloc(ctx, &ro.handoff, (size_t)want * (19 + 2 * TRK_MAX_TENDONS + 3)))) return rc;
      ro.handoff_cap = want;
    }
    vl.d_handoff = ro.handoff; vl.handoff_ld = hld; vl.d_perm = a.perm;
  }
  const trk::FkOut fout = ws_fk_out(ctx, fcol);
  const trk::FkLaunch fl{d_states, cap, w.ld, ctx->K, (bool)ctx->K.enable_rotation, false, ctx->d_tab, ctx->d_steps,
                         (int)ctx->steps.size(), ctx->d_poly, ctx->k_first, ctx->d_tgrid, ctx->d_hl, fout, s};
  const size_t lds_v = trk::verdict_lds_bytes(a.NM, sig != nullptr);
  {
    ProfScope ps(ctx, 5, s);
    switch (ctx->K.n_tendons) {
#define TRK_CASE(N) case N: if (ret) trk::launch_fk_verdict_retract<N>(vl, vr.d_slots + vslot, lds_v, spheres, sig != nullptr); \
                            else trk::launch_fk_verdict<N>(vl, vr.d_slots + vslot, lds_v, spheres, sig != nullptr); break;
      TRK_CASE(1) TRK_CASE(2) TRK_CASE(3) TRK_CASE(4) TRK_CASE(5) TRK_CASE(6) TRK_CASE(7) TRK_CASE(8)
#undef TRK_CASE
      default: return fail(ctx, TR_ERR_OUT_OF_RANGE, "n_tendons out of range");
    }
    HIP_TRY(ctx, hipGetLastError());
  }
  {
    ProfScope ps(ctx, 4, s);
    switch (ctx->K.n_tendons) {
#define TRK_CASE(N) case N: if (ret) trk::launch_fk_sweep_retract_list<N>(fl, d_fargs, lds_f, fb_list, fb_count); \
                            else trk::launch_fk_sweep_fused_list<N>(fl, d_fargs, lds_f, fb_list, fb_count); break;
      TRK_CASE(1) TRK_CASE(2) TRK_CASE(3) TRK_CASE(4) TRK_CASE(5) TRK_CASE(6) TRK_CASE(7) TRK_CASE(8)
#undef TRK_CASE
      default: break;
    }
    HIP_TRY(ctx, hipGetLastError());
  }
  HIP_TRY(ctx, hipEventRecord(vr.ev[vslot], s));
  vr.used[vslot] = true;
  HIP_TRY(ctx, hipEventRecord(ctx->fused.ev[fslot], s));
  ctx->fused.used[fslot] = true;
  return TR_OK;
}

int launch_edge_queue(tr_ctx *ctx, hipStream_t s, uint32_t *sig, int64_t sig_stride, const trk::EdgeQueueArgs *qa, unsigned waves) {
  if (!ctx->has_grid) return fail(ctx, TR_ERR_INVALID_ARG, "no obstacle grid set (tr_set_grid)");
  Workspace &w = ctx->ws;
  if (w.ld < (int64_t)waves * 64) return fail(ctx, TR_ERR_RUNTIME, "edge queue: workspace smaller than the launch");
  tr_ctx::VerdictRing &vr = ctx->vring;
  if (!vr.d_slots) {
    HIP_TRY(ctx, hipMalloc((void **)&vr.d_slots, sizeof(trk::VerdictArgs) * tr_ctx::VerdictRing::kSlots));
    HIP_TRY(ctx, hipHostMalloc((void **)&vr.h_slots, sizeof(trk::VerdictArgs) * tr_ctx::VerdictRing::kSlots, hipHostMallocDefault));
    for (auto &e : vr.ev) HIP_TRY(ctx, hipEventCreateWithFlags(&e, hipEventDisableTiming));
  }
  const int vslot = vr.next;
  vr.next = (vr.next + 1) % tr_ctx::VerdictRing::kSlots;
  if (vr.used[vslot]) HIP_TRY(ctx, hipEventSynchronize(vr.ev[vslot]));
  trk::VerdictArgs &a = vr.h_slots[vslot];
  a = trk::VerdictArgs{};
  size_t lds_k2;
  sweep_geometry(ctx, a.CH, a.NM, lds_k2);
  a.P = ctx->K.n_points; a.debug = ctx->debug;
  a.g = ctx->G; a.grid = ctx->d_grid; a.near_grid = ctx->d_near;
  {
    const GridK &g = ctx->G;
    a.box[0] = g.xmin + 1e-6 * (g.xmax - g.xmin); a.box[1] = g.xmax - 1e-6 * (g.xmax - g.xmin);
    a.box[2] = g.ymin + 1e-6 * (g.ymax - g.ymin); a.box[3] = g.ymax - 1e-6 * (g.ymax - g.ymin);
    a.box[4] = g.zmin + 1e-6 * (g.zmax - g.zmin); a.box[5] = g.zmax - 1e-6 * (g.zmax - g.zmin);
  }
  a.sig = sig; a.sig_stride = sig_stride;
  a.radius = ctx->K.radius;
  for (int j = 0; j < TRK_MAX_TENDONS; j++) { a.home_Li[j] = ctx->K.home_Li[j]; a.min_len[j] = ctx->K.min_len[j]; a.max_len[j] = ctx->K.max_len[j]; }
  a.finish_hot();
  HIP_TRY(ctx, hipMemcpyAsync(vr.d_slots + vslot, &a, sizeof(a), hipMemcpyHostToDevice, s));
  int rc;
  const trk::FusedSweepArgs *d_fargs; size_t lds_f; int fslot;
  if ((rc = fused_args_slot(ctx, ws_sweep_in(ctx, 0), 1, nullptr, nullptr, s, &d_fargs, &lds_f, &fslot))) return rc;
  const size_t lds_v = std::max(trk::verdict_lds_bytes(a.NM, true) + (size_t)trk::EQ_STASH_WORDS * 4, lds_f);
  const trk::FkOut none{nullptr, nullptr, nullptr, nullptr, nullptr, nullptr, nullptr, nullptr, nullptr, nullptr};
  const trk::FkLaunch fl{nullptr, 0, 0, ctx->K, (bool)ctx->K.enable_rotation, false, ctx->d_tab, ctx->d_steps,
                         (int)ctx->steps.size(), ctx->d_poly, ctx->k_first, ctx->d_tgrid, ctx->d_hl, none, s};
  {
    ProfScope ps(ctx, 5, s);
    switch (ctx->K.n_tendons) {
#define TRK_CASE(N) case N: trk::launch_fk_edge_queue<N>(fl, vr.d_slots + vslot, lds_v, qa, d_fargs, waves); break;
      TRK_CASE(1) TRK_CASE(2) TRK_CASE(3) TRK_CASE(4) TRK_CASE(5) TRK_CASE(6) TRK_CASE(7) TRK_CASE(8)
#undef TRK_CASE
      default: return fail(ctx, TR_ERR_OUT_OF_RANGE, "n_tendons out of range");
    }
    HIP_TRY(ctx, hipGetLastError());
  }
  HIP_TRY(ctx, hipEventRecord(vr.ev[vslot], s));
  vr.used[vslot] = true;
  HIP_TRY(ctx, hipEventRecord(ctx->fused.ev[fslot], s));
  ctx->fused.used[fslot] = true;
  return TR_OK;
}

int edge_queue_waves(tr_ctx *ctx) {
  if (ctx->edge_queue_waves > 0) return ctx->edge_queue_waves;
  int CH, NM; size_t lds_k2;
  sweep_geometry(ctx, CH, NM, lds_k2);
  const size_t lds_v = std::max(trk::verdict_lds_bytes(NM, true) + (size_t)trk::EQ_STASH_WORDS * 4, lds_k2);
  int per_cu = 0;
  switch (ctx->K.n_tendons) {
#define TRK_CASE(N) case N: per_cu = trk::fk_edge_queue_waves_per_cu<N>((bool)ctx->K.enable_rotation, lds_v); break;
    TRK_CASE(1) TRK_CASE(2) TRK_CASE(3) TRK_CASE(4) TRK_CASE(5) TRK_CASE(6) TRK_CASE(7) TRK_CASE(8)
#undef TRK_CASE
    default: break;
  }
  hipDeviceProp_t prop;
  if (per_cu <= 0 || hipGetDeviceProperties(&prop, ctx->device) != hipSuccess) return 0;
  ctx->edge_queue_waves = per_cu * prop.multiProcessorCount;
  return ctx->edge_queue_waves;
}

int ensure_sphere_near(tr_ctx *c, hipStream_t s) {
  if (c->sph_near_valid) return TR_OK;
  HIP_TRY(c, hipDeviceSynchronize());
  const size_t ncell = (size_t)c->G.N * c->G.N * c->G.N;
  if (c->d_sph_near) { (void)hipFree(c->d_sph_near); c->d_sph_near = nullptr; }
  if (c->d_sph_tmp) { (void)hipFree(c->d_sph_tmp); c->d_sph_tmp = nullptr; }
  HIP_TRY(c, hipMalloc((void **)&c->d_sph_near, ncell * sizeof(float)));
  HIP_TRY(c, hipMalloc((void **)&c->d_sph_tmp, ncell * sizeof(float)));
  const double reach = c->K.radius + std::sqrt(c->G.dx * c->G.dx + c->G.dy * c->G.dy + c->G.dz * c->G.dz);
  const int R[3] = {(int)std::ceil(reach / c->G.dx) + 1, (int)std::ceil(reach / c->G.dy) + 1, (int)std::ceil(reach / c->G.dz) + 1};
  const unsigned gcell = (unsigned)((ncell + 255) / 256);
  hipLaunchKernelGGL(trk::obstacle_distance_x, dim3(c->n_blocks), dim3(64), 0, s, c->d_grid, c->d_sph_near, c->G.Nb, R[0], (float)c->G.dx);
  hipLaunchKernelGGL(trk::obstacle_distance_axis, dim3(gcell), dim3(256), 0, s, c->d_sph_near, c->d_sph_tmp, c->G.N, 1, R[1], (float)c->G.dy, 0);
  hipLaunchKernelGGL(trk::obstacle_distance_axis, dim3(gcell), dim3(256), 0, s, c->d_sph_tmp, c->d_sph_near, c->G.N, 2, R[2], (float)c->G.dz, 1);
  HIP_TRY(c, hipGetLastError());
  HIP_TRY(c, hipStreamSynchronize(s));
  c->sph_near_valid = true;
  return TR_OK;
}

bool edge_signatures(const tr_ctx *ctx, bool with_points) {
  return ctx->K.enable_retraction ? (ctx->fuse == 2 && !with_points) : ctx->fuse != 0;
}

int launch_fk_sweep(tr_ctx *ctx, const double *d_states, int64_t n, int64_t ld, const trk::FkOut &out, const trk::SweepIn &in,
                    int voxel_test, uint64_t *d_bits, uint8_t *d_flags, hipStream_t s, uint32_t *sig = nullptr, int64_t sig_stride = 0,
                    bool points_unused = false, int32_t *sig_np = nullptr ,
                    int lane = 0) {
  const int check_voxels = voxel_test == 1 ? 1 : 0;
  int rc;
  if (voxel_test == 2) {
    if (!ctx->has_grid) return fail(ctx, TR_ERR_INVALID_ARG, "no obstacle grid set (tr_set_grid)");
    if ((rc = ensure_sphere_near(ctx, s))) return rc;
  }
  if (ctx->fuse == 2 && voxel_test != 0 && points_unused && !out.R && !out.L && !out.tips) {
    return launch_verdict(ctx, d_states, n, d_bits, nullptr, d_flags, s, sig, sig_stride, voxel_test == 2, sig ? sig_np : nullptr, lane);
  }
  if (ctx->fuse != 0 && !ctx->K.enable_retraction && !out.R && !out.L) {
    if ((rc = launch_fused(ctx, d_states, n, ld, out, in, check_voxels, d_bits, d_flags, s, sig, sig_stride))) return rc;
  } else {
    if ((rc = launch_fk(ctx, d_states, n, ld, out, s, lane))) return rc;
    if ((rc = launch_sweep(ctx, in, n, ld, check_voxels, d_bits, d_flags, s))) return rc;
  }
  if (voxel_test == 2) {
    ProfScope ps(ctx, 3, s);
    hipLaunchKernelGGL(trk::spheres_vs_grid, dim3((unsigned)((n + 63) / 64)), dim3(64), 0, s, in.px, in.py, in.pz, in.n_points, n, ld,
                       (int)ctx->K.n_points, ctx->K.radius, ctx->G, ctx->d_grid, ctx->d_sph_near, d_bits, d_flags);
    HIP_TRY(ctx, hipGetLastError());
  }
  return TR_OK;
}

}

extern "C" {

const char *tr_last_error(const tr_ctx *ctx) { return ctx ? ctx->err.c_str() : g_create_error.c_str(); }

int tr_create(const tr_robot_desc *rb, int device, tr_ctx **out) {
  if (!rb || !out) return fail(nullptr, TR_ERR_INVALID_ARG, "null argument");
  *out = nullptr;
  if (rb->n_tendons < 1 || rb->n_tendons > TR_MAX_TENDONS)
    return fail(nullptr, TR_ERR_OUT_OF_RANGE, "n_tendons must be in 1..8");
  if (rb->n_a < 1 || rb->n_a > TR_MAX_COEF || rb->n_m < 1 || rb->n_m > TR_MAX_COEF)
    return fail(nullptr, TR_ERR_OUT_OF_RANGE, "polynomial sizes must be in 1..8");
  if (!rb->C || !rb->D || !rb->max_tension || !rb->min_length || !rb->max_length)
    return fail(nullptr, TR_ERR_INVALID_ARG, "null tendon arrays");
  if (!(rb->L > 0) || !(rb->dL > 0) || !(rb->ro > rb->ri) || !(rb->E > 0))
    return fail(nullptr, TR_ERR_INVALID_ARG, "backbone specs must be positive (L, dL, E) with ro > ri");
  if (rb->L / rb->dL > 65536)
    return fail(nullptr, TR_ERR_INVALID_ARG, "more than 65536 backbone points");
  int ndev = 0;
  if (hipGetDeviceCount(&ndev) != hipSuccess || ndev <= 0)
    return fail(nullptr, TR_ERR_HIP, "no HIP device available (libtendon_hip has no CPU fallback)");
  if (device < 0 || device >= ndev) return fail(nullptr, TR_ERR_INVALID_ARG, "bad device ordinal");
  tr_ctx *c = new tr_ctx();
  c->device = device;
  if (const char *e = std::getenv("TENDON_HIP_FUSED")) { const int v = std::atoi(e); c->fuse = v < 0 ? 0 : (v > 2 ? 2 : v); }
  if (const char *e = std::getenv("TENDON_HIP_RETRACT_SORT")) c->retract_sort_min = std::atoll(e);
  if (std::getenv("TENDON_HIP_RETRACT_KBEGIN_OFF")) c->retract_wave_start = false;
  if (const char *e = std::getenv("TENDON_HIP_EDGE_LANES")) { c->edge_lanes = std::max(1, std::min(tr_ctx::kMaxLanes, std::atoi(e))); c->edge_lanes_fixed = true; }
  if (const char *e = std::getenv("TENDON_HIP_EDGE_QUEUE")) { c->edge_queue = std::atoi(e) != 0; c->edge_queue_forced = c->edge_queue; }
  if (const char *e = std::getenv("TENDON_HIP_EDGE_QUEUE_WAVES")) { const int v = std::atoi(e); if (v >= 1 && v <= 8192) c->edge_queue_waves = v; }
  if (const char *e = std::getenv("TENDON_HIP_EDGE_LANE_GUESS")) { const double v = std::atof(e); if (v >= 0.5 && v <= 64.0) { c->edge_lane_guess = v; c->edge_lane_guess_forced = true; } }
  if (const char *e = std::getenv("TENDON_HIP_EDGE_POOL")) {
    const long long v = std::atoll(e);
    if (v >= 256 && v <= (1ll << 24)) c->edge_pool_max = c->edge_slots_max = (int64_t)round_up(v, 64);
  }
  if (const char *e = std::getenv("TENDON_HIP_SHOOT_CHUNK")) { const long long v = std::atoll(e); if (v >= 1 && v <= (1ll << 20)) c->shoot_chunk = (int64_t)v; }
  if (const char *e = std::getenv("TENDON_HIP_LOADED_VERTEX_BATCH")) { const long long v = std::atoll(e); if (v >= 64 && v <= (1ll << 20)) c->loaded_vertex_batch = (int64_t)round_up(v, 64); }
  if (hipSetDevice(device) != hipSuccess) { delete c; return fail(nullptr, TR_ERR_HIP, "hipSetDevice failed"); }
  {
    int cus = 0;
    if (hipDeviceGetAttribute(&cus, hipDeviceAttributeMultiprocessorCount, device) == hipSuccess && cus > 0)
      c->k1_round = (int64_t)cus * 4 * (rb->n_tendons <= TRK_K1_TWO_WAVE_MAXN ? 2 : 1) * 64;
    c->fb_cap = c->k1_round;
  }
  if (const char *e = std::getenv("TENDON_HIP_FB_CAP")) { const long long v = std::atoll(e); if (v >= 64 && v <= (1ll << 20)) c->fb_cap = (int64_t)round_up(v, 64); }

  RobotK &K = c->K;
  const int N = rb->n_tendons;
  K.n_tendons = N; K.n_a = rb->n_a; K.n_m = rb->n_m;
  K.enable_rotation = rb->enable_rotation ? 1 : 0;
  K.enable_retraction = rb->enable_retraction ? 1 : 0;
  K.state_size = N + K.enable_rotation + K.enable_retraction;
  K.residual_threshold = rb->residual_threshold;
  K.radius = rb->r; K.L = rb->L; K.dL = rb->dL;
  c->C.assign(rb->C, rb->C + (size_t)N * rb->n_a);
  c->D.assign(rb->D, rb->D + (size_t)N * rb->n_m);
  c->max_tension.assign(rb->max_tension, rb->max_tension + N);
  for (int j = 0; j < N; j++) { K.min_len[j] = rb->min_length[j]; K.max_len[j] = rb->max_length[j]; }
  {
    const double ro2 = rb->ro * rb->ro, ri2 = rb->ri * rb->ri;
    const double I = (1.0 / 4.0) * M_PI * (ro2 * ro2 - ri2 * ri2);
    const double Ar = M_PI * (ro2 - ri2);
    const double J = 2 * I;
    const double Gmod = rb->E / (2 * (1 + rb->nu));
    K.kb0 = rb->E * I; K.kb2 = J * Gmod; K.dkb = K.kb2 - K.kb0;
    K.ikb0 = 1 / (rb->E * I); K.ikb2 = 1 / (J * Gmod);
    K.ks0 = Gmod * Ar; K.ks2 = rb->E * Ar;
    K.iks0 = 1 / (Gmod * Ar); K.iks2 = 1 / (rb->E * Ar);
  }
  c->t = t_range(0.0, rb->L, rb->dL);
  K.n_points = (int)c->t.size();
  std::vector<double> step_t;
  for (size_t j = 0; j + 1 < c->t.size(); j++) {
    double cur = c->t[j];
    const double tn = c->t[j + 1];
    bool any = false;
    while (tn - cur > DBL_EPSILON) {
      const double h = std::min(rb->dL, tn - cur);
      c->steps.push_back(StepK{h, -1, 0});
      step_t.push_back(cur);
      cur += h;
      any = true;
    }
    if (!any) { c->steps.push_back(StepK{0.0, -1, 0}); step_t.push_back(cur); }
    c->steps.back().obs = (int)j + 1;
  }
  const size_t ent = (size_t)N * 6;
  std::vector<double> tab((1 + 3 * c->steps.size()) * ent);
  routing_at(c, 0.0, tab.data());
  for (size_t k = 0; k < c->steps.size(); k++) {
    const double tk = step_t[k], h = c->steps[k].h;
    routing_at(c, tk, &tab[(1 + 3 * k + 0) * ent]);
    routing_at(c, tk + h * 0.5, &tab[(1 + 3 * k + 1) * ent]);
    routing_at(c, tk + h, &tab[(1 + 3 * k + 2) * ent]);
  }
  home_lengths(c, c->t, 0.0, K.home_Li);
  for (size_t k = 0; k < c->steps.size(); k++) if (c->steps[k].obs == 1) c->k_first = (int)k + 1;
  c->rows_one_step = (int)c->steps.size() - c->k_first == K.n_points - 2;
  for (size_t k = (size_t)c->k_first; k < c->steps.size() && c->rows_one_step; k++)
    if (c->steps[k].obs != (int)k - c->k_first + 2) c->rows_one_step = false;
  std::vector<double> hl(c->t.size() * (size_t)N);
  for (size_t q = 0; q < c->t.size(); q++)
    for (int j = 0; j < N; j++) {
      const double *Cj = &c->C[(size_t)j * rb->n_a], *Dj = &c->D[(size_t)j * rb->n_m];
      double Cdot[TRK_MAX_COEF] = {0}, Ddot[TRK_MAX_COEF] = {0};
      for (int k = 1; k < rb->n_a; k++) Cdot[k - 1] = k * Cj[k];
      for (int k = 1; k < rb->n_m; k++) Ddot[k - 1] = k * Dj[k];
      const double dd = poly_at(Ddot, rb->n_m, c->t[q]), dv = poly_at(Dj, rb->n_m, c->t[q]), cd = poly_at(Cdot, rb->n_a, c->t[q]);
      hl[q * N + j] = std::sqrt(dd * dd + (dv * dv) * (cd * cd) + 1);
    }
  PolyK poly{};
  for (int j = 0; j < N; j++) {
    for (int i = 0; i < rb->n_a; i++) poly.C[j][i] = c->C[(size_t)j * rb->n_a + i];
    for (int i = 0; i < rb->n_m; i++) poly.D[j][i] = c->D[(size_t)j * rb->n_m + i];
    const int rdeg = poly_degree(&c->D[(size_t)j * rb->n_m], rb->n_m), tdeg = poly_degree(&c->C[(size_t)j * rb->n_a], rb->n_a);
    poly.home_kind[j] = (rdeg == 0 && tdeg == 0) ? 0 : ((rdeg == 0 && tdeg == 1) ? 1 : 2);
    const double d0 = poly.D[j][0], c1 = rb->n_a > 1 ? poly.C[j][1] : 0.0;
    poly.helix_scale[j] = std::sqrt(1 + d0 * d0 * c1 * c1);
  }

  auto bail = [&](const char *what) { std::string m = what; tr_destroy(c); return fail(nullptr, TR_ERR_HIP, m); };
  if (hipMalloc((void **)&c->d_poly, sizeof(PolyK)) != hipSuccess) return bail("hipMalloc(poly)");
  if (hipMemcpy(c->d_poly, &poly, sizeof(PolyK), hipMemcpyHostToDevice) != hipSuccess) return bail("hipMemcpy(poly)");
  if (hipMalloc((void **)&c->d_tgrid, c->t.size() * sizeof(double)) != hipSuccess ||
      hipMalloc((void **)&c->d_hl, hl.size() * sizeof(double)) != hipSuccess) return bail("hipMalloc(tgrid)");
  if (hipMemcpy(c->d_tgrid, c->t.data(), c->t.size() * sizeof(double), hipMemcpyHostToDevice) != hipSuccess ||
      hipMemcpy(c->d_hl, hl.data(), hl.size() * sizeof(double), hipMemcpyHostToDevice) != hipSuccess) return bail("hipMemcpy(tgrid)");
  if (hipMalloc((void **)&c->d_tab, tab.size() * sizeof(double)) != hipSuccess) return bail("hipMalloc(tab)");
  if (hipMemcpy(c->d_tab, tab.data(), tab.size() * sizeof(double), hipMemcpyHostToDevice) != hipSuccess) return bail("hipMemcpy(tab)");
  if (hipMalloc((void **)&c->d_steps, std::max<size_t>(1, c->steps.size()) * sizeof(StepK)) != hipSuccess) return bail("hipMalloc(steps)");
  if (!c->steps.empty() &&
      hipMemcpy(c->d_steps, c->steps.data(), c->steps.size() * sizeof(StepK), hipMemcpyHostToDevice) != hipSuccess) return bail("hipMemcpy(steps)");
  *out = c;
  return TR_OK;
}

void tr_destroy(tr_ctx *c) {
  if (!c) return;
  (void)hipSetDevice(c->device);
  (void)hipDeviceSynchronize();
  for (auto &v : c->events) for (auto &e : v) { (void)hipEventDestroy(e.a); (void)hipEventDestroy(e.b); }
  if (c->pipe.ready) {
    for (int b = 0; b < 2; b++) {
      (void)hipHostFree(c->pipe.h_states[b]); (void)hipHostFree(c->pipe.h_tips[b]); (void)hipHostFree(c->pipe.h_bits[b]); (void)hipHostFree(c->pipe.h_flags[b]);
      (void)hipEventDestroy(c->pipe.up[b]); (void)hipEventDestroy(c->pipe.done[b]); (void)hipEventDestroy(c->pipe.down[b]);
    }
    (void)hipStreamDestroy(c->pipe.s_up); (void)hipStreamDestroy(c->pipe.s_comp); (void)hipStreamDestroy(c->pipe.s_down);
  }
  Workspace &w = c->ws;
  void *ptrs[] = {c->d_tab, c->d_steps, c->d_poly, c->d_tgrid, c->d_hl, c->d_grid, c->d_near, w.homeLi, w.np, c->d_vids, c->d_vmasks, c->d_vcounts,
                  c->d_vbits, w.px, w.py, w.pz, w.acc, w.Li, w.conv,
                  w.states, w.bits, w.tips, w.flags, w.L, w.npts,
                  c->edge.lvl_states, c->edge.bits, c->edge.sample_edge, c->edge.sample_t, c->edge.open, c->edge.frontier,
                  c->edge.A, c->edge.B, c->edge.rel, c->edge.edge_ok, c->edge.nfk, c->edge.first_inv, c->edge.last_t, c->edge.nd, c->edge.cnt, c->edge.sig, c->edge.sig_np, c->edge.ix_states, c->edge.ix_idx, c->edge.open2, c->edge.lvl_states2, c->edge.q_remaining, c->edge.q_lvl_base, c->edge.q_lvl_cnt, c->edge.q_ctl, c->edge.q_args, c->d_envw[0], c->d_envw[1], c->d_sph_near, c->d_sph_tmp};
  for (void *p : ptrs) if (p) (void)hipFree(p);
  trk::merge_free(c->merge);
  if (c->fused.d_slots) { (void)hipFree(c->fused.d_slots); (void)hipHostFree(c->fused.h_slots); for (auto &e : c->fused.ev) (void)hipEventDestroy(e); }
  if (c->vring.d_slots) { (void)hipFree(c->vring.d_slots); (void)hipHostFree(c->vring.h_slots); for (auto &e : c->vring.ev) (void)hipEventDestroy(e); }
  if (c->last_dev_ev) (void)hipEventDestroy(c->last_dev_ev);
  {
    tr_ctx::Sampler &sm = c->samp;
    void *sp[] = {sm.states, sm.bits, sm.tips, sm.wprefix, sm.wprefix2, sm.d_ctr, sm.out_states, sm.out_tips, sm.out_index, sm.sig, sm.sig_index};
    for (void *q : sp) if (q) (void)hipFree(q);
    if (sm.h_ctr) (void)hipHostFree(sm.h_ctr);
  }
  if (c->d_item_src) (void)hipFree(c->d_item_src);
  if (c->d_item_edge) (void)hipFree(c->d_item_edge);
  for (void *q : c->knn.p) if (q) (void)hipFree(q);
  if (c->vstore.ids) (void)hipFree(c->vstore.ids);
  if (c->vstore.masks) (void)hipFree(c->vstore.masks);
  if (c->edge.q_hctl) (void)hipHostFree(c->edge.q_hctl);
  if (c->edge.q_hargs) (void)hipHostFree(c->edge.q_hargs);
  if (c->h_stage) (void)hipHostFree(c->h_stage);
  for (auto &ln : c->lane) {
    tr_ctx::RetractOrder &ro = ln.ro;
    void *lp[] = {ln.counters, ln.fb_list, ln.fb_count, ro.keys[0], ro.keys[1], ro.vals[0], ro.vals[1], ro.kbegin, ro.handoff};
    for (void *q : lp) if (q) (void)hipFree(q);
    if (ln.stream) (void)hipStreamDestroy(ln.stream);
    if (ln.hc) (void)hipHostFree(ln.hc);
    trk::merge_free(ro.ms);
  }
  ik_release(c);
  shoot_release(c);
  ikl_release(c);
  {
    tr_ctx::LoadedEdgeDev &le = c->ledge;
    void *lp[] = {le.vu_pool, le.w, le.d, le.g, le.calls, le.tally, le.out_vu, le.out_index, le.vtally};
    for (void *q : lp) if (q) (void)hipFree(q);
  }
  delete c;
}

int tr_state_size(const tr_ctx *c) { return c ? c->K.state_size : -1; }
int tr_num_points(const tr_ctx *c) { return c ? c->K.n_points : -1; }
int tr_device(const tr_ctx *c) { return c ? c->device : -1; }

int tr_home_lengths(const tr_ctx *c, double *L_i) {
  if (!c || !L_i) return TR_ERR_INVALID_ARG;
  for (int j = 0; j < c->K.n_tendons; j++) L_i[j] = c->K.home_Li[j];
  return TR_OK;
}

int tr_set_checker(tr_ctx *c, int32_t checker) {
  if (!c) return TR_ERR_INVALID_ARG;
  std::lock_guard<std::recursive_mutex> lock_(c->mu);
  if (checker != TR_CHECKER_BACKBONE && checker != TR_CHECKER_SPHERES) return fail(c, TR_ERR_INVALID_ARG, "unknown checker");
  if (checker == TR_CHECKER_BACKBONE && c->has_grid && c->K.dL > std::max({c->G.dx, c->G.dy, c->G.dz}))
    return fail(c, TR_ERR_INVALID_ARG, "robot.specs.dL is larger than expected by VoxelBackboneValidityChecker");
  c->checker = checker;
  return TR_OK;
}
// ... 1018 lines not shown
```

### interactive-rate-tendons_amd/csrc/tr_types.hpp

```cpp
#pragma once
#include <stdint.h>

#define TRK_MAX_TENDONS 8
#define TRK_MAX_COEF    8

struct RobotK {
  double ks0, ks2;
  double kb0, kb2;
  double dkb;
  double iks0, iks2;
  double ikb0, ikb2;
  double residual_threshold;
  double radius;
  double L, dL;
  double min_len[TRK_MAX_TENDONS];
  double max_len[TRK_MAX_TENDONS];
  double home_Li[TRK_MAX_TENDONS];
  int32_t n_tendons, n_a, n_m;
  int32_t enable_rotation, enable_retraction;
  int32_t state_size;
  int32_t n_points;
  int32_t pad_;
};

struct PolyK {
  double C[TRK_MAX_TENDONS][TRK_MAX_COEF];
  double D[TRK_MAX_TENDONS][TRK_MAX_COEF];
  double helix_scale[TRK_MAX_TENDONS];
  int32_t home_kind[TRK_MAX_TENDONS];
};

struct StepK {
  double h;
  int32_t obs;
  int32_t pad_;
};

struct GridK {
  double xmin, xmax, ymin, ymax, zmin, zmax;
  double dx, dy, dz;
  double inv_dx, inv_dy, inv_dz;
  double inv_rot[9];
  int32_t N, Nb;
  int32_t rot_is_identity;
  int32_t pad_;
};

#ifndef TRK_K1_TWO_WAVE_MAXN
#define TRK_K1_TWO_WAVE_MAXN 6
#endif

namespace trk {

struct FkOut {
  double *__restrict__ px, *__restrict__ py, *__restrict__ pz;
  double *__restrict__ R;
  double *__restrict__ L;
  double *__restrict__ Li;
  double *__restrict__ tips;
  uint8_t *__restrict__ converged;
  int32_t *__restrict__ n_points;
  double *__restrict__ home_Li;
};

}
```

### interactive-rate-tendons_amd/csrc/verdict_kernel.hpp

```cpp
#pragma once
#include "fk_kernel.hpp"
#define TRK_DEVICE_BODIES_ONLY
#include "sweep_kernel.hpp"
#include "sphere_kernel.hpp"

namespace trk {

struct VerdictHot {
  double box[6];
  double org[3], inv_d[3];
  const uint64_t *near_grid;
  int32_t Nb, rot_is_identity, P, CH;
  int32_t use_near;
  int32_t pad_;
};
static_assert(sizeof(VerdictHot) == 128, "one 128-byte block");

struct alignas(128) VerdictArgs {
  VerdictHot hot;
  int P, CH, NM, pad0_;
  uint32_t debug, pad1_;
  double box[6];
  GridK g;
  const uint64_t *grid, *near_grid;
// ... 302 lines not shown
            pr.y = g.inv_rot[3] * pv.x + g.inv_rot[4] * pv.y + g.inv_rot[5] * pv.z;
            pr.z = g.inv_rot[6] * pv.x + g.inv_rot[7] * pv.y + g.inv_rot[8] * pv.z;
          }
          const float dl = VL_F(Lay::DELTA + lane);
          if (dn_prev - dl > a.r_hi) {}
          else if ((sph_state & 2u) && dn_prev + dl < a.r_lo) VL_U(Lay::HIT + lane) = 1u;
          else need = true;
        }
        sph_state = 0;
        if (!VL_U(Lay::HIT + lane)) request(a, q);
      }
    } else
    if (active && !VL_U(Lay::HIT + lane)) need = voxel_test(a.hot, j == 0, in_q, cq);
    const unsigned long long wm = __ballot(need);
    if (wm) {
      if (need) {
        if constexpr (!SPH) pr = to_voxel_frame(a, pv);
        const int slot = Lay::wrap(qhead + qcount + __popcll(wm & (((unsigned long long)1 << lane) - 1)));
        VL_D(Lay::QE + 0 * VQ + slot) = pr.x; VL_D(Lay::QE + 1 * VQ + slot) = pr.y; VL_D(Lay::QE + 2 * VQ + slot) = pr.z;
        if constexpr (!SPH) { VL_D(Lay::QE + 3 * VQ + slot) = qr.x; VL_D(Lay::QE + 4 * VQ + slot) = qr.y; VL_D(Lay::QE + 5 * VQ + slot) = qr.z; }
        Lay::set_owner(slot, lane);
      }
      qcount += __popcll(wm);
      if (qcount >= VQ - 64) flush();
    }
    VL_BARRIER();
  }

  __device__ __forceinline__ void tip_point(int row, bool on, bool first, double x, double y, double z, bool wave_row = true) {
#pragma clang fp contract(off)
    VL_BARRIER();
    const VerdictArgs &a = args();
    const GridK &g = a.g;
    const int lane = threadIdx.x;
    const V3 q = {x, y, z};
    V3 pv = q;
    bool need = false;
    V3 pr = pv, qr = q;
    bool in_q = false;
    int cq[3] = {0, 0, 0};
    double tq[3] = {0.0, 0.0, 0.0};
    if constexpr (!SPH) point_cell(a, q, qr, in_q, cq, tq);
    if constexpr (SIG) {
      uint32_t sg = 0u;
      if constexpr (!SPH) sg = on ? signature_of(a, in_q, cq, tq, x, y, z) : 0u;
      else sg = on ? cell_signature(x, y, z, g) : 0u;
      if (!wave_row) {
        if (on && sig_row_of >= 0) a.sig[(int64_t)sig_row_of * a.sig_stride + row] = sg;
        if (first) sig_first_row = row + 2;
      } else sig_put(a, row, on, sg, sig_row_of, sig_first_row);
    }
    if (on) {
      float d = 0.0f;
      if (!first) { pv = V3{VL_D(lane), VL_D(64 + lane), VL_D(128 + lane)}; d = VL_F(Lay::DIST + lane); }
      pr = pv;
      {
        const float dx = (float)(q.x - pv.x), dy = (float)(q.y - pv.y), dz = (float)(q.z - pv.z);
        d += __builtin_amdgcn_sqrtf(dx * dx + dy * dy + dz * dz);
        VL_F(Lay::DIST + lane) = d;
      }
      {
        const int back = P - 1 - row;
        const int k = (int)(((float)back + 0.5f) * (1.0f / (float)CH));
        const bool ms_row = (back - k * CH) == 0;
        if (first || ms_row) {
          const int slot = (first && !ms_row) ? k + 1 : k;
          const int o = Lay::MS + slot * 64 + lane, pl = NM * 64;
          VL_F(o) = (float)q.x; VL_F(o + pl) = (float)q.y; VL_F(o + 2 * pl) = (float)q.z; VL_F(o + 3 * pl) = -d;
        }
      }
      VL_D(lane) = q.x; VL_D(64 + lane) = q.y; VL_D(128 + lane) = q.z;
      if constexpr (SPH) {
        if (active && !VL_U(Lay::HIT + lane)) {
          if (sph_state & 1u) {
            if (!g.rot_is_identity) {
              pr.x = g.inv_rot[0] * pv.x + g.inv_rot[1] * pv.y + g.inv_rot[2] * pv.z;
              pr.y = g.inv_rot[3] * pv.x + g.inv_rot[4] * pv.y + g.inv_rot[5] * pv.z;
              pr.z = g.inv_rot[6] * pv.x + g.inv_rot[7] * pv.y + g.inv_rot[8] * pv.z;
            }
            const float dl = VL_F(Lay::DELTA + lane);
            if (dn_prev - dl > a.r_hi) {}
            else if ((sph_state & 2u) && dn_prev + dl < a.r_lo) VL_U(Lay::HIT + lane) = 1u;
            else need = true;
          }
          sph_state = 0;
          if (!VL_U(Lay::HIT + lane)) request(a, q);
        }
      } else
      if (active && !VL_U(Lay::HIT + lane)) need = voxel_test(a.hot, first, in_q, cq);
    }
    const unsigned long long wm = __ballot(need);
    if (wm) {
      if (need) {
        if constexpr (!SPH) pr = to_voxel_frame(a, pv);
        const int slot = Lay::wrap(qhead + qcount + __popcll(wm & (((unsigned long long)1 << lane) - 1)));
        VL_D(Lay::QE + 0 * VQ + slot) = pr.x; VL_D(Lay::QE + 1 * VQ + slot) = pr.y; VL_D(Lay::QE + 2 * VQ + slot) = pr.z;
        if constexpr (!SPH) { VL_D(Lay::QE + 3 * VQ + slot) = qr.x; VL_D(Lay::QE + 4 * VQ + slot) = qr.y; VL_D(Lay::QE + 5 * VQ + slot) = qr.z; }
        Lay::set_owner(slot, lane);
      }
      qcount += __popcll(wm);
      if (qcount >= VQ - 64) flush();
    }
    VL_BARRIER();
  }
};

struct LaneVerdict { bool valid, pending; uint32_t fl; };
template <int N, bool SPH, bool SIG>
__device__ __forceinline__ LaneVerdict verdict_decide(const VerdictArgs &a, const FkLane<N> &fl_, bool live) {
  using Lay = VLay<SIG>;
  const int lane = threadIdx.x;
  const int P = a.P;
  const int Kl = (P - 1 + a.CH - 1) / a.CH;
  const bool conv_ok = live && fl_.converged;
  bool len_ok = false;
  if (conv_ok) {
    bool ok = true;
#pragma unroll
    for (int j = 0; j < N; j++) {
      const double dl = a.home_Li[j] - fl_.Li[j];
      if (dl < a.min_len[j] || a.max_len[j] < dl) ok = false;
    }
    len_ok = ok;
  }
  bool alive = conv_ok && len_ok;
  const uint32_t hf = VL_U(Lay::HIT + lane);
  const bool hit = (hf & 1u) != 0;
  bool bad = (hf & 2u) != 0;
  if (alive && !(VL_F(Lay::DIST + lane) < 1e30f)) { alive = false; bad = true; }
  bool need_exact = alive && P > 2;
  if (!(a.debug & 2u) && __any(need_exact)) {
    const float *mx = (const float *)vlds + Lay::MS + lane, *my = mx + (size_t)a.NM * 64, *mz = my + (size_t)a.NM * 64, *ma = mz + (size_t)a.NM * 64;
    need_exact = milestones_unresolved(mx, my, mz, ma, a.NM, Kl, need_exact, (float)a.radius);
  }

  uint32_t fl = 0;
  if (conv_ok) fl |= 1u;
  if (conv_ok && len_ok) fl |= 2u;
  bool valid = conv_ok && len_ok;
  if (valid && bad) { fl |= 16u; valid = false; }
  const bool pending = valid && need_exact && (a.flags != nullptr || !hit);
  if (valid && !pending) {
    if (!need_exact) { fl |= 4u; if (!hit) fl |= 8u; else valid = false; }
    else valid = false;
  }
  if (pending) valid = false;
  if (SPH && pending && !hit) fl |= 8u;
  return LaneVerdict{valid, pending, fl};
}

#ifndef TRK_VERDICT_TWO_WAVE_MAXN
#define TRK_VERDICT_TWO_WAVE_MAXN 4
#endif
template <int N, bool ROT, bool SPH, bool SIG = false>
__global__ __launch_bounds__(64, (N <= TRK_VERDICT_TWO_WAVE_MAXN ? 2 : 1)) void fk_verdict(
    const double *__restrict__ states, int64_t n, RobotK K, const double *__restrict__ tab, const StepK *__restrict__ steps,
    int nsteps, double *__restrict__ tips, const VerdictArgs *__restrict__ va) {
  using Lay = VLay<SIG>;
  const int lane = threadIdx.x;
  PointSweep<SPH, SIG> ps;
  ps.va = va;
  ps.dn_prev = 0.0f; ps.sph_state = 0u;
  ps.qhead = 0; ps.qcount = 0; ps.active = false;
  ps.P = va->P; ps.CH = va->CH; ps.NM = va->NM; ps.Kl = (ps.P - 1 + ps.CH - 1) / ps.CH; ps.ms_next = 0; ps.ms_k = 0;
  VL_U(Lay::HIT + lane) = 0u; VL_U(Lay::INPREV + lane) = 0u; VL_F(Lay::DIST + lane) = 0.0f;
  {
    const int64_t i0 = (int64_t)blockIdx.x * 64 + lane;
    ps.sigst.init(); ps.sig_row_of = -1; ps.sig_first_row = 0; ps.sig_rows_of_launch(n);
  }
  __syncthreads();

  FkLane<N> fl_;
  FkOut out{nullptr, nullptr, nullptr, nullptr, nullptr, nullptr, nullptr, nullptr, nullptr, nullptr};
  fk_uniform_body<N, ROT, false, false>(states, n, 0, K, tab, steps, nsteps, out, ps, nullptr, &fl_);

  ps.template sig_finish<false>();
  ps.finish();
  while (ps.qcount > 0) ps.flush();
  __syncthreads();
  if (tips) {
    VL_D(lane) = fl_.tip[0]; VL_D(64 + lane) = fl_.tip[1]; VL_D(128 + lane) = fl_.tip[2];
    __syncthreads();
    const int64_t e0 = (int64_t)blockIdx.x * 192, etot = 3 * n;
#pragma unroll
    for (int q = 0; q < 3; q++) {
      const int e = q * 64 + lane;
      if (e0 + e < etot) tips[e0 + e] = VL_D((e % 3) * 64 + e / 3);
    }
    __syncthreads();
  }
  const VerdictArgs a = *va;
  const int64_t i = (int64_t)blockIdx.x * 64 + lane;
  const bool live = i < n;
  const LaneVerdict lv = verdict_decide<N, SPH, SIG>(a, fl_, live);
  const bool valid = lv.valid, pending = lv.pending;
  const uint32_t fl = lv.fl;
  const uint64_t bits = __ballot(valid && live);
  if (lane == 0 && live) a.valid_bits[i >> 6] = bits;
  if (a.flags && live) a.flags[i] = (uint8_t)fl;
  const unsigned long long pm = __ballot(pending);
  if (pm) {
    uint32_t base = 0;
    if (lane == 0) base = atomicAdd(a.fb_count, (uint32_t)__popcll(pm));
    base = __shfl(base, 0, 64);
    if (pending) a.fb_list[base + __popcll(pm & (((unsigned long long)1 << lane) - 1))] = (int32_t)i;
  }
}

#ifdef TRK_WITH_RETRACT_VERDICT
template <int N, bool ROT, bool SPH, bool SIG = false>
__global__ __launch_bounds__(64, (N <= TRK_VR_TWO_WAVE_MAXN ? 2 : 1)) void fk_verdict_retract(
    const double *__restrict__ states, int64_t n, RobotK K, const PolyK *__restrict__ pk, const double *__restrict__ tab,
    const StepK *__restrict__ steps, int nsteps, int k_first, const double *__restrict__ tgrid, const double *__restrict__ hl,
    double *__restrict__ tips, const VerdictArgs *__restrict__ va, RetractHandoff ho) {
  using Lay = VLay<SIG>;
  const int lane = threadIdx.x;
  PointSweep<SPH, SIG> ps;
  ps.va = va;
  ps.dn_prev = 0.0f; ps.sph_state = 0u;
  ps.qhead = 0; ps.qcount = 0; ps.active = false;
  ps.P = va->P; ps.CH = va->CH; ps.NM = va->NM; ps.Kl = 0; ps.ms_next = 0; ps.ms_k = 0;
  const int32_t *__restrict__ perm = va->perm;
  {
    const int64_t i0 = (int64_t)blockIdx.x * 64 + lane;
    ps.sigst.init(); ps.sig_row_of = i0 < n ? (perm ? perm[i0] : (int)i0) : -1; ps.sig_first_row = 0; ps.sig_row0 = 0; ps.sig_cnt = 0;
  }
  VL_U(Lay::HIT + lane) = 0u; VL_U(Lay::INPREV + lane) = 0u; VL_F(Lay::DIST + lane) = 0.0f;
  __syncthreads();

  FkLaneR<N> fl_;
  FkOut out{nullptr, nullptr, nullptr, nullptr, nullptr, nullptr, tips, nullptr, nullptr, nullptr};
  const int32_t *__restrict__ wkb = va->wave_k_begin;
  fk_retract_body<N, ROT, false, PointSweep<SPH, SIG> &, 2>(states, n, 0, K, pk, tab, steps, nsteps, k_first, tgrid, hl, out, ps, perm, &fl_,
                                                            wkb ? wkb[blockIdx.x] : 0, &ho);

  ps.template sig_finish<true>();
  ps.finish();
  while (ps.qcount > 0) ps.flush();
  __syncthreads();
  const VerdictArgs a = *va;
  const int64_t i = (int64_t)blockIdx.x * 64 + lane;
  const bool live = i < n;
  const int64_t c = (perm && live) ? (int64_t)perm[i] : i;
  const int np = fl_.np;
  const int Kl = (np - 1 + a.CH - 1) / a.CH;
  const bool conv_ok = live && fl_.converged;
  bool len_ok = false;
  if (conv_ok) {
    bool ok = true;
#pragma unroll
    for (int j = 0; j < N; j++) {
      const double dl = fl_.home_Li[j] - fl_.Li[j];
      if (dl < a.min_len[j] || a.max_len[j] < dl) ok = false;
    }
    len_ok = ok;
  }
  bool alive = conv_ok && len_ok;
  const uint32_t hf = VL_U(Lay::HIT + lane);
  const bool hit = (hf & 1u) != 0;
  bool bad = (hf & 2u) != 0;
  if (alive && !(VL_F(Lay::DIST + lane) < 1e30f)) { alive = false; bad = true; }
  bool need_exact = alive && np > 2;
  if (!(a.debug & 2u) && __any(need_exact)) {
    const float *mx = (const float *)vlds + Lay::MS + lane, *my = mx + (size_t)a.NM * 64, *mz = my + (size_t)a.NM * 64, *ma = mz + (size_t)a.NM * 64;
    need_exact = milestones_unresolved(mx, my, mz, ma, a.NM, Kl, need_exact, (float)a.radius);
  }

  uint32_t fl = 0;
  if (conv_ok) fl |= 1u;
  if (conv_ok && len_ok) fl |= 2u;
  bool valid = conv_ok && len_ok;
  if (valid && bad) { fl |= 16u; valid = false; }
  const bool pending = valid && need_exact && (a.flags != nullptr || !hit);
  if (valid && !pending) {
    if (!need_exact) { fl |= 4u; if (!hit) fl |= 8u; else valid = false; }
    else valid = false;
  }
  if (pending) valid = false;
  if (SPH && pending && !hit) fl |= 8u;
  if (perm) {
    if (valid && live) atomicOr((unsigned long long *)&a.valid_bits[c >> 6], 1ull << (c & 63));
  } else {
    const uint64_t bits = __ballot(valid && live);
    if (lane == 0 && live) a.valid_bits[i >> 6] = bits;
  }
  if (a.flags && live) a.flags[c] = (uint8_t)fl;
  if (a.np_out && live) a.np_out[c] = np;
  const unsigned long long pm = __ballot(pending);
  if (pm) {
    uint32_t base = 0;
    if (lane == 0) base = atomicAdd(a.fb_count, (uint32_t)__popcll(pm));
    base = __shfl(base, 0, 64);
    if (pending) a.fb_list[base + __popcll(pm & (((unsigned long long)1 << lane) - 1))] = (int32_t)c;
  }
}

template <int N, bool ROT>
__global__ __launch_bounds__(64, (N <= TRK_K1R_TWO_WAVE_MAXN ? 2 : 1)) void fk_sweep_retract_list(
    const double *__restrict__ states, int64_t cap, int64_t ld, RobotK K, const PolyK *__restrict__ pk, const double *__restrict__ tab,
    const StepK *__restrict__ steps, int nsteps, int k_first, const double *__restrict__ tgrid, const double *__restrict__ hl,
    FkOut out, const FusedSweepArgs *__restrict__ sa, const int32_t *__restrict__ list, const uint32_t *__restrict__ count) {
  const int64_t total = (int64_t)*count;
  for (int64_t offset = 0; offset < total; offset += cap) {
    const int64_t left = total - offset;
    const int64_t m = left < cap ? left : cap;
    if ((int64_t)blockIdx.x * 64 >= m) break;
    fk_retract_body<N, ROT, false>(states, m, ld, K, pk, tab, steps, nsteps, k_first, tgrid, hl, out, NoPointHook(), list + offset);
    __syncthreads();
    const FusedSweepArgs a = *sa;
    sweep_body<true>(a.in, m, ld, a.P, a.CH, a.NM, K, a.g, a.grid, a.near_grid, a.check_voxels, a.debug, a.valid_bits, a.flags, list + offset);
    __syncthreads();
  }
}
#endif

}
```

### profiles/count_isa.py

```python
#!/usr/bin/env python3
import collections
import json
import os
import re
import subprocess
import sys
import tempfile

ROOT = os.path.dirname(os.path.dirname(os.path.abspath(__file__)))
CSRC = os.path.join(ROOT, "interactive-rate-tendons_amd", "csrc")
OUT = os.path.join(ROOT, "profiles", "isa_counts.json")
FLAGS = ["--offload-arch=gfx950", "-O3", "-std=c++17", "-ffp-contract=off"]

FLOPS = {"v_fma_f64": 2, "v_fmac_f64": 2, "v_mul_f64": 1, "v_add_f64": 1, "v_rcp_f64": 1, "v_rsq_f64": 1, "v_sqrt_f64": 1,
         "v_div_fmas_f64": 2, "v_div_fixup_f64": 1, "v_div_scale_f64": 1, "v_pk_fma_f64": 4, "v_pk_mul_f64": 2,
         "v_pk_add_f64": 2}

_RK4_ONLY = r'''
#include <hip/hip_runtime.h>
#include "tr_types.hpp"
#include "fk_kernel.hpp"
namespace trk {
// the RK4 step as fk_verdict and fk_sweep_fused hold it (no rotation, no R output, no backbone-length quadrature), without
// any per-point hook: the reference count of useful flops per step
template <int N> __global__ __launch_bounds__(64, 2) void rk4_step_only(const double *states, int64_t n, int64_t ld, RobotK K,
                                                                         const double *tab, const StepK *steps, int nsteps, FkOut out) {
  fk_uniform_body<N, false, false, false>(states, n, ld, K, tab, steps, nsteps, out);
}
}
template __global__ void trk::rk4_step_only<%d>(const double*, int64_t, int64_t, RobotK, const double*, const StepK*, int, trk::FkOut);
'''

KERNELS = {
    "rk4_step<3>": _RK4_ONLY % 3,
    "rk4_step<4>": _RK4_ONLY % 4,
    "fk_verdict<3,false>": r'''
#include <hip/hip_runtime.h>
#include "tr_types.hpp"
#include "verdict_kernel.hpp"
template __global__ void trk::fk_verdict<3, false, false>(const double*, int64_t, RobotK, const double*, const StepK*, int, double*, const trk::VerdictArgs*);
''',
    "fk_verdict<4,false>": r'''
#include <hip/hip_runtime.h>
#include "tr_types.hpp"
#include "verdict_kernel.hpp"
template __global__ void trk::fk_verdict<4, false, false>(const double*, int64_t, RobotK, const double*, const StepK*, int, double*, const trk::VerdictArgs*);
''',
    "fk_sweep_fused<3,false>": r'''
#include <hip/hip_runtime.h>
#include "tr_types.hpp"
#include "fused_kernel.hpp"
template __global__ void trk::fk_sweep_fused<3, false>(const double*, int64_t, int64_t, RobotK, const double*, const StepK*, int,
                                                       trk::FkOut, const trk::FusedSweepArgs*);
''',
    "fk_sweep_fused<4,false>": r'''
#include <hip/hip_runtime.h>
#include "tr_types.hpp"
#include "fused_kernel.hpp"
template __global__ void trk::fk_sweep_fused<4, false>(const double*, int64_t, int64_t, RobotK, const double*, const StepK*, int,
                                                       trk::FkOut, const trk::FusedSweepArgs*);
''',
    "fk_rk4_batch_uniform<3,false,false>": r'''
#include <hip/hip_runtime.h>
#include "tr_types.hpp"
#include "fk_kernel.hpp"
template __global__ void trk::fk_rk4_batch_uniform<3, false, false>(const double*, int64_t, int64_t, RobotK,
                                                                     const double*, const StepK*, int, trk::FkOut);
''',
    "fk_rk4_batch_uniform<4,false,false>": r'''
#include <hip/hip_runtime.h>
#include "tr_types.hpp"
#include "fk_kernel.hpp"
template __global__ void trk::fk_rk4_batch_uniform<4, false, false>(const double*, int64_t, int64_t, RobotK,
                                                                     const double*, const StepK*, int, trk::FkOut);
''',
}

_BLOCK = re.compile(r"^(\.LBB\d+_\d+):\s*(?:;\s*(.*))?$")
_FALL = re.compile(r"^; (%bb\.\d+):\s*(?:;\s*(.*))?$")
_HDR = re.compile(r"Header=(BB\d+_\d+)")
_INSN = re.compile(r"^\s+([vs]_[a-z0-9_]+)")


def count_asm(asm):
    blocks = []
    cur, hist, nv = None, collections.Counter(), 0
    for line in asm.splitlines():
        m = _BLOCK.match(line) or _FALL.match(line)
        if m:
            blocks.append((cur, hist, nv))
            hist, nv = collections.Counter(), 0
            note = m.group(2) or ""
            if "Loop Header" in note and "This" in note:
                cur = m.group(1)[2:] if m.group(1).startswith(".L") else None
            else:
                h = _HDR.search(note)
                cur = h.group(1) if h else None
            continue
        m = _INSN.match(line)
        if not m:
            continue
        op = m.group(1)
        for suffix in ("_e32", "_e64", "_dpp", "_sdwa"):
            if op.endswith(suffix):
                op = op[: -len(suffix)]
        if op.startswith("v_"):
            nv += 1
            if op.endswith("_f64"):
                hist[op] += 1
    blocks.append((cur, hist, nv))
    loops = collections.defaultdict(collections.Counter)
    valu, rare = collections.Counter(), collections.Counter()
    for hdr, h, n in blocks:
        if hdr is None:
            continue
        if any(op.startswith("v_div_") for op in h):
            rare[hdr] += 1
            continue
        loops[hdr].update(h)
        valu[hdr] += n
    if not loops:
        raise RuntimeError("no fp64 loop found in the assembly")
    hdr = max(loops, key=lambda h: loops[h]["v_fma_f64"] + loops[h]["v_fmac_f64"])
    hist = dict(sorted(loops[hdr].items()))
    return {"loop": hdr, "fp64_valu_instructions_per_step": int(sum(hist.values())),
            "valu_instructions_per_step": int(valu[hdr]), "rare_blocks": int(rare[hdr]),
            "flops_per_step": int(sum(FLOPS.get(op, 0) * c for op, c in hist.items())),
            "opcodes": hist}


def compile_asm(tu, workdir):
    src = os.path.join(workdir, "k.hip")
    with open(src, "w") as f:
        f.write(tu)
    out = os.path.join(workdir, "k.s")
    subprocess.run(["hipcc"] + FLAGS + ["--cuda-device-only", "-S", "-I", CSRC, src, "-o", out], check=True,
                   stdout=subprocess.DEVNULL, stderr=subprocess.DEVNULL)
    return open(out).read()


def count_all(names=None):
    res = {}
    for name, tu in KERNELS.items():
        if names and name not in names:
            continue
        with tempfile.TemporaryDirectory() as d:
            res[name] = count_asm(compile_asm(tu, d))
    return res


def main():
    res = count_all()
    if "--check" in sys.argv:
        old = json.load(open(OUT))
        bad = [k for k in res if old.get(k, {}).get("flops_per_step") != res[k]["flops_per_step"]]
        if bad:
            print("stale:", bad)
            sys.exit(1)
        return
    json.dump(res, open(OUT, "w"), indent=1, sort_keys=True)
    for k, v in res.items():
        print(k, v["fp64_valu_instructions_per_step"], "fp64 instr/step,", v["flops_per_step"], "flop/step")


if __name__ == "__main__":
    main()
```

### profiles/kbench.hip

```cpp
#include <hip/hip_runtime.h>
#include <algorithm>
#include <cmath>
#include <cstdio>
#include <cstdlib>
#include <vector>
#include "tr_types.hpp"
#include "fk_kernel.hpp"
#ifdef KB_VERDICT
#include "verdict_kernel.hpp"
#ifdef KB_SIG
constexpr bool kSig = true;
#else
constexpr bool kSig = false;
#endif
#endif

#ifndef KB_N
#define KB_N 3
#endif
#ifndef KB_LOG2
#define KB_LOG2 20
#endif
#ifndef KB_REPS
#define KB_REPS 7
#endif
#ifndef KB_WAVES
#define KB_WAVES 2
#endif

namespace trk {
template <int N> __global__ __launch_bounds__(64, KB_WAVES) void rk4_only(const double *__restrict__ states, int64_t n, RobotK K,
                                                                           const double *__restrict__ tab, const StepK *__restrict__ steps,
                                                                           int nsteps, double *__restrict__ tips) {
  FkOut out{nullptr, nullptr, nullptr, nullptr, nullptr, nullptr, tips, nullptr, nullptr, nullptr};
  fk_uniform_body<N, false, false, false>(states, n, 0, K, tab, steps, nsteps, out);
}
}

#define CK(x) do { hipError_t e_ = (x); if (e_ != hipSuccess) { std::fprintf(stderr, "%s: %s\n", #x, hipGetErrorString(e_)); return 1; } } while (0)

static void routing_at(int N, const double C[][3], const double D[][3], double t, double *out) {
  for (int j = 0; j < N; j++) {
    const double th = C[j][0] + C[j][1] * t + C[j][2] * t * t, th1 = C[j][1] + 2 * C[j][2] * t, th2 = 2 * C[j][2];
    const double rho = D[j][0] + D[j][1] * t + D[j][2] * t * t, rho1 = D[j][1] + 2 * D[j][2] * t, rho2 = 2 * D[j][2];
    const double sa = std::sin(th), ca = std::cos(th);
    double *o = out + 6 * j;
    o[0] = rho * sa; o[1] = rho * ca;
    o[2] = rho1 * sa + rho * (ca * th1);
    o[3] = rho1 * ca + rho * (-sa * th1);
    o[4] = rho2 * sa + 2 * rho1 * (ca * th1) - rho * (sa * th1 * th1) + rho * (ca * th2);
    o[5] = rho2 * ca + 2 * rho1 * (-sa * th1) - rho * (ca * th1 * th1) + rho * (-sa * th2);
  }
}

int main() {
  constexpr int N = KB_N;
  const double L = 0.2, dL = L / 128, ro = 0.01, ri = 0.0, E = 2.1e6, nu = 0.3;
  double C[8][3] = {}, D[8][3] = {};
  if (N == 3) for (int k = 0; k < 3; k++) { C[k][0] = 2 * M_PI * k / 3; C[k][1] = 5.0; D[k][0] = 0.01; }
  else {
    const double c1[4] = {3.0, -2.0, 4.0, -5.0}, c2[4] = {10.0, 15.0, -12.0, 8.0}, d1[4] = {-0.01, 0.005, 0.0, -0.005};
    for (int k = 0; k < N; k++) { C[k][0] = M_PI * k / 2; C[k][1] = c1[k % 4]; C[k][2] = c2[k % 4]; D[k][0] = 0.01; D[k][1] = d1[k % 4]; }
  }
  RobotK K{};
  {
    const double ro2 = ro * ro, ri2 = ri * ri, I = 0.25 * M_PI * (ro2 * ro2 - ri2 * ri2), Ar = M_PI * (ro2 - ri2), J = 2 * I, G = E / (2 * (1 + nu));
    K.kb0 = E * I; K.kb2 = J * G; K.dkb = K.kb2 - K.kb0; K.ikb0 = 1 / K.kb0; K.ikb2 = 1 / K.kb2; K.ks0 = G * Ar; K.ks2 = E * Ar; K.iks0 = 1 / K.ks0; K.iks2 = 1 / K.ks2;
  }
  K.residual_threshold = 5e-6; K.radius = 0.015; K.L = L; K.dL = dL; K.n_tendons = N; K.n_a = 3; K.n_m = 3; K.state_size = N; K.n_points = 129;
  std::vector<StepK> steps;
  std::vector<double> tab((1 + 3 * 128) * N * 6);
  routing_at(N, C, D, 0.0, tab.data());
  for (int k = 0; k < 128; k++) {
    const double tk = k * dL;
    steps.push_back(StepK{dL, k + 1, 0});
    for (int q = 0; q < 3; q++) routing_at(N, C, D, tk + 0.5 * q * dL, &tab[(size_t)(1 + 3 * k + q) * N * 6]);
  }
#ifdef KB_COUNT
  const int64_t n = KB_COUNT;
#else
  const int64_t n = (int64_t)1 << KB_LOG2;
#endif
  std::vector<double> st((size_t)n * N);
  unsigned long long lcg = 88172645463325252ull;
  const double tmax = N == 3 ? 10.0 : 20.0;
  for (auto &x : st) { lcg = lcg * 6364136223846793005ull + 1442695040888963407ull; x = tmax * (double)(lcg >> 11) * (1.0 / 9007199254740992.0); }
  double *d_st, *d_tab, *d_tips; StepK *d_steps;
  CK(hipMalloc(&d_st, st.size() * 8)); CK(hipMalloc(&d_tab, tab.size() * 8)); CK(hipMalloc(&d_tips, (size_t)n * 24)); CK(hipMalloc(&d_steps, steps.size() * sizeof(StepK)));
  CK(hipMemcpy(d_st, st.data(), st.size() * 8, hipMemcpyHostToDevice)); CK(hipMemcpy(d_tab, tab.data(), tab.size() * 8, hipMemcpyHostToDevice));
  CK(hipMemcpy(d_steps, steps.data(), steps.size() * sizeof(StepK), hipMemcpyHostToDevice));
  hipEvent_t a, b; CK(hipEventCreate(&a)); CK(hipEventCreate(&b));
#ifdef KB_VERDICT
  trk::VerdictArgs va{};
  va.P = 129; va.CH = (int)std::lround(2.0 * K.radius / dL); va.NM = (128 + va.CH - 1) / va.CH + 1;
  GridK &g = va.g;
  g.xmin = g.ymin = g.zmin = -0.25; g.xmax = g.ymax = g.zmax = 0.25; g.N = 256; g.Nb = 64; g.rot_is_identity = 1;
  g.dx = g.dy = g.dz = 0.5 / 256; g.inv_dx = g.inv_dy = g.inv_dz = 1 / g.dx;
  for (int q = 0; q < 9; q++) g.inv_rot[q] = (q % 4 == 0) ? 1.0 : 0.0;
  for (int q = 0; q < 3; q++) { va.box[2 * q] = -0.25 + 1e-6 * 0.5; va.box[2 * q + 1] = 0.25 - 1e-6 * 0.5; }
  uint64_t *d_grid, *d_bits; int32_t *d_fb; uint32_t *d_fbc; trk::VerdictArgs *d_va;
  CK(hipMalloc(&d_grid, (size_t)64 * 64 * 64 * 8 * 2)); CK(hipMemset(d_grid, 0, (size_t)64 * 64 * 64 * 8 * 2));
  CK(hipMalloc(&d_bits, (size_t)((n + 63) / 64) * 8)); CK(hipMalloc(&d_fb, (size_t)n * 4)); CK(hipMalloc(&d_fbc, 4)); CK(hipMemset(d_fbc, 0, 4));
  va.grid = d_grid; va.near_grid = d_grid + 64 * 64 * 64; va.valid_bits = d_bits; va.fb_list = d_fb; va.fb_count = d_fbc;
  va.radius = K.radius;
  uint32_t *d_sig = nullptr;
  if (kSig) { va.sig_stride = (129 + 15) / 16 * 16; CK(hipMalloc(&d_sig, (size_t)n * va.sig_stride * 4)); va.sig = d_sig; }
  for (int j = 0; j < N; j++) { va.min_len[j] = K.min_len[j] = -1.0; va.max_len[j] = K.max_len[j] = 1.0; va.home_Li[j] = K.home_Li[j] = L; }
  va.finish_hot();
  CK(hipMalloc(&d_va, sizeof(va))); CK(hipMemcpy(d_va, &va, sizeof(va), hipMemcpyHostToDevice));
  const size_t lds = trk::verdict_lds_bytes(va.NM, kSig);
#endif
  std::vector<float> ms;
  for (int r = 0; r < KB_REPS + 2; r++) {
    CK(hipEventRecord(a));
#ifdef KB_VERDICT
    hipLaunchKernelGGL((trk::fk_verdict<N, false, false, kSig>), dim3((unsigned)((n + 63) / 64)), dim3(64), lds, nullptr, d_st, n, K, d_tab, d_steps, 128, d_tips, d_va);
#else
    hipLaunchKernelGGL((trk::rk4_only<N>), dim3((unsigned)((n + 63) / 64)), dim3(64), 0, nullptr, d_st, n, K, d_tab, d_steps, 128, d_tips);
#endif
    CK(hipEventRecord(b)); CK(hipEventSynchronize(b));
    float t; CK(hipEventElapsedTime(&t, a, b));
    if (r >= 2) ms.push_back(t);
  }
  std::vector<double> tips((size_t)n * 3);
  CK(hipMemcpy(tips.data(), d_tips, tips.size() * 8, hipMemcpyDeviceToHost));
  double sum = 0, asum = 0; for (double v : tips) { sum += v; asum += std::fabs(v); }
  std::sort(ms.begin(), ms.end());
  hipFuncAttributes fa;
#ifdef KB_VERDICT
  CK(hipFuncGetAttributes(&fa, (const void *)trk::fk_verdict<N, false, false, kSig>));
  {
    std::vector<uint64_t> bits((size_t)((n + 63) / 64));
    CK(hipMemcpy(bits.data(), d_bits, bits.size() * 8, hipMemcpyDeviceToHost));
    uint32_t fbc = 0; CK(hipMemcpy(&fbc, d_fbc, 4, hipMemcpyDeviceToHost));
    long valid = 0; for (uint64_t w : bits) valid += __builtin_popcountll(w);
    std::printf("fk_verdict: valid %ld of %ld, fallback entries %u (summed over launches)\n", valid, (long)n, fbc);
  }
#else
  CK(hipFuncGetAttributes(&fa, (const void *)trk::rk4_only<N>));
#endif
  std::printf("N=%d n=%ld (2^%d unless KB_COUNT) waves/SIMD<=%d: best %.3f ms  median %.3f ms  -> %.4g FK/s   regs %d  scratch %zu B   tips sum %.17g abs %.17g\n", N, (long)n, KB_LOG2, KB_WAVES,
              ms.front(), ms[ms.size() / 2], (double)n / (ms.front() * 1e-3), fa.numRegs, (size_t)fa.localSizeBytes, sum, asum);
  return 0;
}
```

Baseline: 141.2 million.

## Specialize strain-rate kernel for uniform helical tendon routing

Adds a compile-time routing form template parameter and a host-side classifier that detects tendons routed as a uniform helix. For that case the strain-rate computation uses the closed-form relation r' = omega × r, which simplifies pd and folds the Hzz update into a single FMA using rho². This removes some per-tendon double-precision arithmetic in the RK4 inner loop. All launchers dispatch between the helix and table variants at runtime, which doubles template instantiations, and correctness depends on the classifier recognizing only truly helical routing.

```diff
diff --git a/interactive-rate-tendons_amd/csrc/edge_queue_kernel.hpp b/interactive-rate-tendons_amd/csrc/edge_queue_kernel.hpp
--- a/interactive-rate-tendons_amd/csrc/edge_queue_kernel.hpp
+++ b/interactive-rate-tendons_amd/csrc/edge_queue_kernel.hpp
@@ -113,7 +113,7 @@
   }
 }
 
-template <int N, bool ROT>
+template <int N, bool ROT, class Form = TableRouting>
 __global__ __launch_bounds__(64, (N <= TRK_VERDICT_TWO_WAVE_MAXN ? 2 : 1)) void fk_edge_queue(
     RobotK K, const double *__restrict__ tab, const StepK *__restrict__ steps, int nsteps,
     const VerdictArgs *__restrict__ va, const EdgeQueueArgs *__restrict__ qa, const FusedSweepArgs *__restrict__ sa) {
@@ -172,7 +172,7 @@
     FkLane<N> fl_;
     {
       FkOut out{nullptr, nullptr, nullptr, nullptr, nullptr, nullptr, nullptr, nullptr, nullptr, nullptr};
-      fk_uniform_body<N, ROT, false, false>(st_eff, n_eff, 0, K, tab, steps, nsteps, out, ps, nullptr, &fl_);
+      fk_uniform_body<N, ROT, false, false, Form>(st_eff, n_eff, 0, K, tab, steps, nsteps, out, ps, nullptr, &fl_);
     }
     ps.template sig_finish<false>();
     ps.finish();
@@ -206,7 +206,7 @@
       __syncthreads();
       const double *st2 = q2.states + ((int64_t)h2 - (int64_t)blockIdx.x * 64) * K.state_size;
       const int64_t n2 = (int64_t)blockIdx.x * 64 + cnt2;
-      fk_uniform_body<N, ROT, false, false>(st2, n2, q2.fb_ld, K, tab, steps, nsteps, q2.fb_out, NoPointHook(), nullptr, nullptr);
+      fk_uniform_body<N, ROT, false, false, Form>(st2, n2, q2.fb_ld, K, tab, steps, nsteps, q2.fb_out, NoPointHook(), nullptr, nullptr);
       __syncthreads();
       const FusedSweepArgs fa = *sa;
       bool exact = false;
diff --git a/interactive-rate-tendons_amd/csrc/fk_inst.hip b/interactive-rate-tendons_amd/csrc/fk_inst.hip
--- a/interactive-rate-tendons_amd/csrc/fk_inst.hip
+++ b/interactive-rate-tendons_amd/csrc/fk_inst.hip
@@ -19,19 +19,30 @@
 
 namespace trk {
 
+using HelixForm = std::conditional_t<(TRK_INST_N <= TRK_K1_TWO_WAVE_MAXN), UniformHelix, TableRouting>;
+[[maybe_unused]] static bool helix_form(const RobotK &K) { return TRK_INST_N <= TRK_K1_TWO_WAVE_MAXN && K.routing_form == TRK_ROUTING_HELIX; }
+
 #if TRK_INST_KIND == 5
+template <class Form>
+static void go_queue(const FkLaunch &a, const VerdictArgs *va, size_t lds, const EdgeQueueArgs *qa, const FusedSweepArgs *sweep, unsigned waves) {
+  if (a.rotation)
+    hipLaunchKernelGGL((fk_edge_queue<TRK_INST_N, true, Form>), dim3(waves), dim3(64), lds, a.stream, a.K, a.d_tab, a.d_steps, a.n_steps, va, qa, sweep);
+  else
+    hipLaunchKernelGGL((fk_edge_queue<TRK_INST_N, false, Form>), dim3(waves), dim3(64), lds, a.stream, a.K, a.d_tab, a.d_steps, a.n_steps, va, qa, sweep);
+}
+template <class Form>
+static int queue_waves_per_cu(bool rotation, size_t lds) {
+  int nb = 0;
+  const hipError_t e = rotation ? hipOccupancyMaxActiveBlocksPerMultiprocessor(&nb, fk_edge_queue<TRK_INST_N, true, Form>, 64, lds)
+                                : hipOccupancyMaxActiveBlocksPerMultiprocessor(&nb, fk_edge_queue<TRK_INST_N, false, Form>, 64, lds);
+  return e == hipSuccess ? nb : 0;
+}
 template <> void launch_fk_edge_queue<TRK_INST_N>(const FkLaunch &a, const VerdictArgs *va, size_t lds, const EdgeQueueArgs *qa,
                                                   const FusedSweepArgs *sweep, unsigned waves) {
-  if (a.rotation)
-    hipLaunchKernelGGL((fk_edge_queue<TRK_INST_N, true>), dim3(waves), dim3(64), lds, a.stream, a.K, a.d_tab, a.d_steps, a.n_steps, va, qa, sweep);
-  else
-    hipLaunchKernelGGL((fk_edge_queue<TRK_INST_N, false>), dim3(waves), dim3(64), lds, a.stream, a.K, a.d_tab, a.d_steps, a.n_steps, va, qa, sweep);
+  if (helix_form(a.K)) go_queue<HelixForm>(a, va, lds, qa, sweep, waves); else go_queue<TableRouting>(a, va, lds, qa, sweep, waves);
 }
-template <> int fk_edge_queue_waves_per_cu<TRK_INST_N>(bool rotation, size_t lds) {
-  int nb = 0;
-  const hipError_t e = rotation ? hipOccupancyMaxActiveBlocksPerMultiprocessor(&nb, fk_edge_queue<TRK_INST_N, true>, 64, lds)
-                                : hipOccupancyMaxActiveBlocksPerMultiprocessor(&nb, fk_edge_queue<TRK_INST_N, false>, 64, lds);
-  return e == hipSuccess ? nb : 0;
+template <> int fk_edge_queue_waves_per_cu<TRK_INST_N>(const RobotK &K, size_t lds) {
+  return helix_form(K) ? queue_waves_per_cu<HelixForm>((bool)K.enable_rotation, lds) : queue_waves_per_cu<TableRouting>((bool)K.enable_rotation, lds);
 }
 #endif
 
@@ -80,39 +91,42 @@
   if (a.rotation) go_list<true>(a, sweep, lds, list, count); else go_list<false>(a, sweep, lds, list, count);
 }
 #elif TRK_INST_KIND == 3
-template <bool ROT, bool SPH, bool SIG>
+template <bool ROT, bool SPH, bool SIG, class Form>
 static void go(const FkLaunch &a, const VerdictArgs *va, size_t lds) {
   const unsigned grid = (unsigned)((a.n + 63) / 64);
-  hipLaunchKernelGGL((fk_verdict<TRK_INST_N, ROT, SPH, SIG>), dim3(grid), dim3(64), lds, a.stream, a.d_states, a.n, a.K, a.d_tab, a.d_steps,
+  hipLaunchKernelGGL((fk_verdict<TRK_INST_N, ROT, SPH, SIG, Form>), dim3(grid), dim3(64), lds, a.stream, a.d_states, a.n, a.K, a.d_tab, a.d_steps,
                      a.n_steps, a.out.tips, va);
 }
 template <bool SPH, bool SIG>
 static void go_rot(const FkLaunch &a, const VerdictArgs *va, size_t lds) {
-  if (a.rotation) go<true, SPH, SIG>(a, va, lds); else go<false, SPH, SIG>(a, va, lds);
+  if (helix_form(a.K)) { if (a.rotation) go<true, SPH, SIG, HelixForm>(a, va, lds); else go<false, SPH, SIG, HelixForm>(a, va, lds); }
+  else                 { if (a.rotation) go<true, SPH, SIG, TableRouting>(a, va, lds); else go<false, SPH, SIG, TableRouting>(a, va, lds); }
 }
 template <> void launch_fk_verdict<TRK_INST_N>(const FkLaunch &a, const VerdictArgs *va, size_t lds, bool spheres, bool with_sig) {
   if (spheres) { if (with_sig) go_rot<true, true>(a, va, lds); else go_rot<true, false>(a, va, lds); }
   else         { if (with_sig) go_rot<false, true>(a, va, lds); else go_rot<false, false>(a, va, lds); }
 }
 #elif TRK_INST_KIND == 2
-template <bool ROT>
+template <bool ROT, class Form>
 static void go_list(const FkLaunch &a, const FusedSweepArgs *sweep, size_t lds, const int32_t *list, const uint32_t *count) {
   const unsigned grid = (unsigned)((a.n + 63) / 64);
-  hipLaunchKernelGGL((fk_sweep_fused_list<TRK_INST_N, ROT>), dim3(grid), dim3(64), lds, a.stream, a.d_states, a.n, a.ld, a.K,
+  hipLaunchKernelGGL((fk_sweep_fused_list<TRK_INST_N, ROT, Form>), dim3(grid), dim3(64), lds, a.stream, a.d_states, a.n, a.ld, a.K,
                      a.d_tab, a.d_steps, a.n_steps, a.out, sweep, list, count);
 }
 template <> void launch_fk_sweep_fused_list<TRK_INST_N>(const FkLaunch &a, const FusedSweepArgs *sweep, size_t lds, const int32_t *list,
                                                         const uint32_t *count) {
-  if (a.rotation) go_list<true>(a, sweep, lds, list, count); else go_list<false>(a, sweep, lds, list, count);
+  if (helix_form(a.K)) { if (a.rotation) go_list<true, HelixForm>(a, sweep, lds, list, count); else go_list<false, HelixForm>(a, sweep, lds, list, count); }
+  else                 { if (a.rotation) go_list<true, TableRouting>(a, sweep, lds, list, count); else go_list<false, TableRouting>(a, sweep, lds, list, count); }
 }
-template <bool ROT>
+template <bool ROT, class Form>
 static void go(const FkLaunch &a, const FusedSweepArgs *sweep, size_t lds) {
   const unsigned grid = (unsigned)((a.n + 63) / 64);
-  hipLaunchKernelGGL((fk_sweep_fused<TRK_INST_N, ROT>), dim3(grid), dim3(64), lds, a.stream, a.d_states, a.n, a.ld, a.K,
+  hipLaunchKernelGGL((fk_sweep_fused<TRK_INST_N, ROT, Form>), dim3(grid), dim3(64), lds, a.stream, a.d_states, a.n, a.ld, a.K,
                      a.d_tab, a.d_steps, a.n_steps, a.out, sweep);
 }
 template <> void launch_fk_sweep_fused<TRK_INST_N>(const FkLaunch &a, const FusedSweepArgs *sweep, size_t lds) {
-  if (a.rotation) go<true>(a, sweep, lds); else go<false>(a, sweep, lds);
+  if (helix_form(a.K)) { if (a.rotation) go<true, HelixForm>(a, sweep, lds); else go<false, HelixForm>(a, sweep, lds); }
+  else                 { if (a.rotation) go<true, TableRouting>(a, sweep, lds); else go<false, TableRouting>(a, sweep, lds); }
 }
 #else
 #if TRK_INST_KIND == 1
@@ -127,8 +141,12 @@
 template <bool ROT, bool WR>
 static void go(const FkLaunch &a) {
   const unsigned grid = (unsigned)((a.n + 63) / 64);
-  hipLaunchKernelGGL((fk_rk4_batch_uniform<TRK_INST_N, ROT, WR>), dim3(grid), dim3(64), 0, a.stream, a.d_states, a.n, a.ld, a.K,
-                     a.d_tab, a.d_steps, a.n_steps, a.out);
+  if (helix_form(a.K))
+    hipLaunchKernelGGL((fk_rk4_batch_uniform<TRK_INST_N, ROT, WR, HelixForm>), dim3(grid), dim3(64), 0, a.stream, a.d_states, a.n, a.ld, a.K,
+                       a.d_tab, a.d_steps, a.n_steps, a.out);
+  else
+    hipLaunchKernelGGL((fk_rk4_batch_uniform<TRK_INST_N, ROT, WR>), dim3(grid), dim3(64), 0, a.stream, a.d_states, a.n, a.ld, a.K,
+                       a.d_tab, a.d_steps, a.n_steps, a.out);
 }
 template <> void launch_fk_uniform<TRK_INST_N>(const FkLaunch &a) {
 #endif
diff --git a/interactive-rate-tendons_amd/csrc/fk_kernel.hpp b/interactive-rate-tendons_amd/csrc/fk_kernel.hpp
--- a/interactive-rate-tendons_amd/csrc/fk_kernel.hpp
+++ b/interactive-rate-tendons_amd/csrc/fk_kernel.hpp
@@ -34,11 +34,16 @@
   __device__ __forceinline__ void operator()(double &, double &, double &, double &, double &, double &) const {}
 };
 
-template <int N, class Route, class Load = NoLoad>
+struct TableRouting { static constexpr bool kHelix = false; };
+struct UniformHelix { static constexpr bool kHelix = true; };
+
+template <int N, class Route, class Load = NoLoad, class Form = TableRouting>
 __device__ __forceinline__ void strain_rates_routed(const double v[3], const double u[3], const double (&tau)[N],
                                                     Route &&route, const RobotK &K,
                                                     double dv[3], double du[3], double (&sdot)[N], const Load &load = Load()) {
 #pragma clang fp contract(fast)
+  double kh = 0;
+  if constexpr (Form::kHelix) kh = u[2] - K.helix_omega;
   double Axx = K.ks0, Axy = 0, Axz = 0, Ayy = K.ks0, Ayz = 0, Azz = K.ks2, Z = 0;
   double B00 = 0, B01 = 0, B02 = 0, B10 = 0, B11 = 0, B12 = 0, B20 = 0, B21 = 0, B22 = 0;
   double Hxx = K.kb0, Hxy = 0, Hxz = 0, Hyy = K.kb0, Hyz = 0, Hzz = K.kb2;
@@ -50,8 +55,14 @@
     const double rx = r6[0], ry = r6[1];
     const double rdx = r6[2], rdy = r6[3];
     const double rddx = r6[4], rddy = r6[5];
-    const double pdx = (v[0] + rdx) - u[2] * ry;
-    const double pdy = (v[1] + rdy) + u[2] * rx;
+    double pdx, pdy;
+    if constexpr (Form::kHelix) {
+      pdx = __builtin_fma(-kh, ry, v[0]);
+      pdy = __builtin_fma(kh, rx, v[1]);
+    } else {
+      pdx = (v[0] + rdx) - u[2] * ry;
+      pdy = (v[1] + rdy) + u[2] * rx;
+    }
     const double pdz = __builtin_fma(u[0], ry, __builtin_fma(-u[1], rx, v[2]));
     const double sxy = __builtin_fma(pdy, pdy, pdx * pdx), s2 = __builtin_fma(pdz, pdz, sxy);
     const double rs = fast_rsqrt(s2);
@@ -70,7 +81,7 @@
     const double mxy = c * sxy, mx = mxy * rx, my = mxy * ry;
     Hxx -= my * ry; Hxy += mx * ry; Hyy -= mx * rx;
     const double t1 = cs2 * rx, t2 = cs2 * ry;
-    Hzz -= t1 * rx; Hzz -= t2 * ry;
+    if constexpr (!Form::kHelix) { Hzz -= t1 * rx; Hzz -= t2 * ry; }
     {
 #pragma clang fp contract(off)
       Azz -= mxy; B02 -= my; B12 += mx; B20 += t2; B21 -= t1;
@@ -85,6 +96,7 @@
     ax = __builtin_fma(cs2, px, ax); ay = __builtin_fma(cs2, py, ay); az = __builtin_fma(cs2, pz, az);
     bx = __builtin_fma(t2, pz, bx); by = __builtin_fma(-t1, pz, by); bz = __builtin_fma(t1, py, __builtin_fma(-t2, px, bz));
   }
+  if constexpr (Form::kHelix) Hzz = __builtin_fma(-K.helix_rho2, Z, Hzz);
 #define TRK_FMA __builtin_fma
   const double svx = K.ks0 * v[0], svy = K.ks0 * v[1], svz = K.ks2 * (v[2] - 1.0);
   const double dku = K.dkb * u[2], w = TRK_FMA(-K.ks0, v[2], svz);
@@ -177,14 +189,15 @@
 #undef TRK_FMA
 }
 
-template <int N, class Load = NoLoad>
+template <int N, class Load = NoLoad, class Form = TableRouting>
 __device__ __forceinline__ void strain_rates(const double v[3], const double u[3], const double (&tau)[N],
                                              const double *__restrict__ ri, const RobotK &K,
                                              double dv[3], double du[3], double (&sdot)[N], const Load &load = Load()) {
-  strain_rates_routed<N>(v, u, tau, [&](int j, double (&r6)[6]) {
+  auto row = [&](int j, double (&r6)[6]) {
 #pragma unroll
     for (int q = 0; q < 6; q++) r6[q] = ri[6 * j + q];
-  }, K, dv, du, sdot, load);
+  };
+  strain_rates_routed<N, decltype(row) &, Load, Form>(v, u, tau, row, K, dv, du, sdot, load);
 }
 
 template <int N>
@@ -351,7 +364,7 @@
   return N >= HookLiInLds<std::remove_cv_t<std::remove_reference_t<OnPoint>>>::from && N <= 4;
 }
 
-template <int N, bool ROT, bool WRITE_R, bool WANT_L = true, class OnPoint = NoPointHook>
+template <int N, bool ROT, bool WRITE_R, bool WANT_L = true, class Form = TableRouting, class OnPoint = NoPointHook>
 __device__ __forceinline__ void fk_uniform_body(
     const double *__restrict__ states, int64_t n, int64_t ld, const RobotK &K,
     const double *__restrict__ tab, const StepK *__restrict__ steps, int nsteps, const FkOut &out,
@@ -433,7 +446,7 @@
       const double bw = (st == 0 || st == 3) ? b1 : b2;
       const double aw = (st == 2) ? h : hh;
       double dv[3], du[3], sd[N];
-      strain_rates<N>(sv, su, tau, ri, K, dv, du, sd);
+      strain_rates<N, NoLoad, Form>(sv, su, tau, ri, K, dv, du, sd);
       position_quadrature(st, sR, sv, b1, qs, qm, p);
       if (WANT_L && out.L) {
         const double v2 = __builtin_fma(sv[2], sv[2], __builtin_fma(sv[1], sv[1], sv[0] * sv[0]));
@@ -492,11 +505,11 @@
   }
 }
 
-template <int N, bool ROT, bool WRITE_R>
+template <int N, bool ROT, bool WRITE_R, class Form = TableRouting>
 __global__ __launch_bounds__(64, (N <= TRK_K1_TWO_WAVE_MAXN ? 2 : 1)) void fk_rk4_batch_uniform(
     const double *__restrict__ states, int64_t n, int64_t ld, RobotK K,
     const double *__restrict__ tab, const StepK *__restrict__ steps, int nsteps, FkOut out) {
-  fk_uniform_body<N, ROT, WRITE_R>(states, n, ld, K, tab, steps, nsteps, out);
-}
-
-}
+  fk_uniform_body<N, ROT, WRITE_R, true, Form>(states, n, ld, K, tab, steps, nsteps, out);
+}
+
+}
diff --git a/interactive-rate-tendons_amd/csrc/fk_launch.hpp b/interactive-rate-tendons_amd/csrc/fk_launch.hpp
--- a/interactive-rate-tendons_amd/csrc/fk_launch.hpp
+++ b/interactive-rate-tendons_amd/csrc/fk_launch.hpp
@@ -42,7 +42,7 @@
 
 template <int N> void launch_fk_edge_queue(const FkLaunch &a, const VerdictArgs *va, size_t lds, const EdgeQueueArgs *qa,
                                            const FusedSweepArgs *sweep, unsigned waves);
-template <int N> int fk_edge_queue_waves_per_cu(bool rotation, size_t lds);
+template <int N> int fk_edge_queue_waves_per_cu(const RobotK &K, size_t lds);
 
 template <int N> void launch_fk_loaded(const FkLaunch &a, const LoadedIn &in);
 template <int N> void launch_shoot_start(const FkLaunch &a, const double *guess, double *vu);
@@ -55,7 +55,7 @@
   template <> void launch_fk_verdict_retract<N>(const FkLaunch &, const VerdictArgs *, size_t, bool, bool); \
   template <> void launch_fk_sweep_retract_list<N>(const FkLaunch &, const FusedSweepArgs *, size_t, const int32_t *, const uint32_t *); \
   template <> void launch_fk_edge_queue<N>(const FkLaunch &, const VerdictArgs *, size_t, const EdgeQueueArgs *, const FusedSweepArgs *, unsigned); \
-  template <> int fk_edge_queue_waves_per_cu<N>(bool, size_t);
+  template <> int fk_edge_queue_waves_per_cu<N>(const RobotK &, size_t);
 TRK_DECL_FK(1) TRK_DECL_FK(2) TRK_DECL_FK(3) TRK_DECL_FK(4) TRK_DECL_FK(5) TRK_DECL_FK(6) TRK_DECL_FK(7) TRK_DECL_FK(8)
 #undef TRK_DECL_FK
 
diff --git a/interactive-rate-tendons_amd/csrc/fused_kernel.hpp b/interactive-rate-tendons_amd/csrc/fused_kernel.hpp
--- a/interactive-rate-tendons_amd/csrc/fused_kernel.hpp
+++ b/interactive-rate-tendons_amd/csrc/fused_kernel.hpp
@@ -25,13 +25,13 @@
   return p;
 }
 
-template <int N, bool ROT>
+template <int N, bool ROT, class Form = TableRouting>
 __global__ __launch_bounds__(64, (N <= TRK_FUSED_TWO_WAVE_MAXN ? 2 : 1)) void fk_sweep_fused(
     const double *__restrict__ states, int64_t n, int64_t ld, RobotK K, const double *__restrict__ tab,
     const StepK *__restrict__ steps, int nsteps, FkOut out, const FusedSweepArgs *__restrict__ sa) {
   SignatureHook hook{sa, n, sa->sig != nullptr, {}};
   hook.st.init();
-  fk_uniform_body<N, ROT, false, false>(states, n, ld, K, tab, steps, nsteps, out, hook);
+  fk_uniform_body<N, ROT, false, false, Form>(states, n, ld, K, tab, steps, nsteps, out, hook);
   hook.finish();
   __syncthreads();
   const FusedKernargsPtr ka = fused_kernargs();
@@ -39,7 +39,7 @@
   sweep_body<false>(a.in, ka->n, ka->ld, a.P, a.CH, a.NM, ka->K, a.g, a.grid, a.near_grid, a.check_voxels, a.debug, a.valid_bits, a.flags);
 }
 
-template <int N, bool ROT>
+template <int N, bool ROT, class Form = TableRouting>
 __global__ __launch_bounds__(64, (N <= TRK_FUSED_TWO_WAVE_MAXN ? 2 : 1)) void fk_sweep_fused_list(
     const double *__restrict__ states, int64_t cap, int64_t ld, RobotK K, const double *__restrict__ tab,
     const StepK *__restrict__ steps, int nsteps, FkOut out, const FusedSweepArgs *__restrict__ sa,
@@ -49,7 +49,7 @@
     const int64_t left = total - offset;
     const int64_t m = left < cap ? left : cap;
     if ((int64_t)blockIdx.x * 64 >= m) break;
-    fk_uniform_body<N, ROT, false, false>(states, m, ld, K, tab, steps, nsteps, out, NoPointHook(), list + offset);
+    fk_uniform_body<N, ROT, false, false, Form>(states, m, ld, K, tab, steps, nsteps, out, NoPointHook(), list + offset);
     __syncthreads();
     const FusedKernargsPtr ka = fused_kernargs();
     const FusedSweepArgs a = *ka->sa;
diff --git a/interactive-rate-tendons_amd/csrc/routing_form.hpp b/interactive-rate-tendons_amd/csrc/routing_form.hpp
--- /dev/null
+++ b/interactive-rate-tendons_amd/csrc/routing_form.hpp
@@ -0,0 +1,61 @@
+#pragma once
+#include <cmath>
+#include <cstring>
+#include "tr_types.hpp"
+
+namespace routing_form {
+
+struct Spec {
+  int n_tendons, n_a, n_m;
+  const double *C, *D;
+  bool enable_retraction;
+};
+
+struct Form {
+  int form;
+  double omega, rho;
+};
+
+inline void row(const Spec &s, double t, double *out) {
+  const int N_a = s.n_a, N_m = s.n_m, N_s = N_a > N_m ? N_a : N_m;
+  double S[TRK_MAX_COEF], Sd[TRK_MAX_COEF], Sdd[TRK_MAX_COEF];
+  S[0] = 1; Sd[0] = 0; Sdd[0] = 0;
+  if (N_s >= 2) { S[1] = t; Sd[1] = 1; Sdd[1] = 0; }
+  for (int i = 2; i < N_s; i++) { S[i] = t * S[i - 1]; Sd[i] = i * S[i - 1]; Sdd[i] = i * (i - 1) * S[i - 2]; }
+  for (int j = 0; j < s.n_tendons; j++) {
+    const double *Cj = s.C + (size_t)j * N_a, *Dj = s.D + (size_t)j * N_m;
+    double C_a = 0, C_ad = 0, C_add = 0, D_m = 0, D_md = 0, D_mdd = 0;
+    for (int i = 0; i < N_a; i++) { C_a += Cj[i] * S[i]; C_ad += Cj[i] * Sd[i]; C_add += Cj[i] * Sdd[i]; }
+    for (int i = 0; i < N_m; i++) { D_m += Dj[i] * S[i]; D_md += Dj[i] * Sd[i]; D_mdd += Dj[i] * Sdd[i]; }
+    const double sa = std::sin(C_a), ca = std::cos(C_a);
+    double *o = out + 6 * j;
+    o[0] = D_m * sa;
+    o[1] = D_m * ca;
+    o[2] = D_md * sa + D_m * (ca * C_ad);
+    o[3] = D_md * ca + D_m * (-sa * C_ad);
+    o[4] = D_mdd * sa + 2 * D_md * (ca * C_ad) - D_m * (sa * C_ad * C_ad) + D_m * (ca * C_add);
+    o[5] = D_mdd * ca + 2 * D_md * (-sa * C_ad) - D_m * (ca * C_ad * C_ad) + D_m * (-sa * C_add);
+  }
+}
+
+inline int degree(const double *c, int n) {
+  for (int i = n - 1; i > 0; i--) if (std::fabs(c[i]) > 0.0) return i;
+  return 0;
+}
+
+inline Form classify(const Spec &s, const char *forced, int max_tendons) {
+  const Form table{TRK_ROUTING_TABLE, 0.0, 0.0};
+  if (forced && std::strcmp(forced, "table") == 0) return table;
+  if (s.enable_retraction || s.n_tendons < 1 || s.n_tendons > max_tendons) return table;
+  const double omega = s.n_a > 1 ? s.C[1] : 0.0, rho = s.D[0];
+  if (!std::isfinite(omega) || !std::isfinite(rho)) return table;
+  for (int j = 0; j < s.n_tendons; j++) {
+    const double *Cj = s.C + (size_t)j * s.n_a, *Dj = s.D + (size_t)j * s.n_m;
+    if (degree(Dj, s.n_m) != 0 || degree(Cj, s.n_a) > 1) return table;
+    const double w = s.n_a > 1 ? Cj[1] : 0.0;
+    if (std::memcmp(&w, &omega, sizeof(double)) != 0 || std::memcmp(&Dj[0], &rho, sizeof(double)) != 0) return table;
+  }
+  return Form{TRK_ROUTING_HELIX, omega, rho};
+}
+
+}
diff --git a/interactive-rate-tendons_amd/csrc/tendon_hip.hip b/interactive-rate-tendons_amd/csrc/tendon_hip.hip
--- a/interactive-rate-tendons_amd/csrc/tendon_hip.hip
+++ b/interactive-rate-tendons_amd/csrc/tendon_hip.hip
@@ -25,6 +25,7 @@
 #include "verdict_kernel.hpp"
 #include "edge_kernel.hpp"
 #include "edge_plan.hpp"
+#include "routing_form.hpp"
 #include "knn_kernel.hpp"
 #include "cache_merge.hpp"
 #include "env_kernel.hpp"
@@ -273,27 +274,10 @@
   return vals;
 }
 
-void routing_at(const tr_ctx *c, double t, double *out) {
-  const int N_a = c->K.n_a, N_m = c->K.n_m, N_s = std::max(N_a, N_m);
-  double S[TRK_MAX_COEF], Sd[TRK_MAX_COEF], Sdd[TRK_MAX_COEF];
-  S[0] = 1; Sd[0] = 0; Sdd[0] = 0;
-  if (N_s >= 2) { S[1] = t; Sd[1] = 1; Sdd[1] = 0; }
-  for (int i = 2; i < N_s; i++) { S[i] = t * S[i - 1]; Sd[i] = i * S[i - 1]; Sdd[i] = i * (i - 1) * S[i - 2]; }
-  for (int j = 0; j < c->K.n_tendons; j++) {
-    const double *Cj = &c->C[(size_t)j * N_a], *Dj = &c->D[(size_t)j * N_m];
-    double C_a = 0, C_ad = 0, C_add = 0, D_m = 0, D_md = 0, D_mdd = 0;
-    for (int i = 0; i < N_a; i++) { C_a += Cj[i] * S[i]; C_ad += Cj[i] * Sd[i]; C_add += Cj[i] * Sdd[i]; }
-    for (int i = 0; i < N_m; i++) { D_m += Dj[i] * S[i]; D_md += Dj[i] * Sd[i]; D_mdd += Dj[i] * Sdd[i]; }
-    const double sa = std::sin(C_a), ca = std::cos(C_a);
-    double *o = out + 6 * j;
-    o[0] = D_m * sa;
-    o[1] = D_m * ca;
-    o[2] = D_md * sa + D_m * (ca * C_ad);
-    o[3] = D_md * ca + D_m * (-sa * C_ad);
-    o[4] = D_mdd * sa + 2 * D_md * (ca * C_ad) - D_m * (sa * C_ad * C_ad) + D_m * (ca * C_add);
-    o[5] = D_mdd * ca + 2 * D_md * (-sa * C_ad) - D_m * (ca * C_ad * C_ad) + D_m * (-sa * C_add);
-  }
-}
+routing_form::Spec routing_spec(const tr_ctx *c) {
+  return routing_form::Spec{c->K.n_tendons, c->K.n_a, c->K.n_m, c->C.data(), c->D.data(), c->K.enable_retraction != 0};
+}
+void routing_at(const tr_ctx *c, double t, double *out) { routing_form::row(routing_spec(c), t, out); }
 
 int poly_degree(const double *c, int n) {
   for (int i = n - 1; i > 0; i--) if (std::fabs(c[i]) > 0.0) return i;
@@ -785,7 +769,7 @@
   const size_t lds_v = std::max(trk::verdict_lds_bytes(NM, true) + (size_t)trk::EQ_STASH_WORDS * 4, lds_k2);
   int per_cu = 0;
   switch (ctx->K.n_tendons) {
-#define TRK_CASE(N) case N: per_cu = trk::fk_edge_queue_waves_per_cu<N>((bool)ctx->K.enable_rotation, lds_v); break;
+#define TRK_CASE(N) case N: per_cu = trk::fk_edge_queue_waves_per_cu<N>(ctx->K, lds_v); break;
     TRK_CASE(1) TRK_CASE(2) TRK_CASE(3) TRK_CASE(4) TRK_CASE(5) TRK_CASE(6) TRK_CASE(7) TRK_CASE(8)
 #undef TRK_CASE
     default: break;
@@ -876,6 +860,7 @@
   if (const char *e = std::getenv("TENDON_HIP_FUSED")) { const int v = std::atoi(e); c->fuse = v < 0 ? 0 : (v > 2 ? 2 : v); }
   if (const char *e = std::getenv("TENDON_HIP_RETRACT_SORT")) c->retract_sort_min = std::atoll(e);
   if (std::getenv("TENDON_HIP_RETRACT_KBEGIN_OFF")) c->retract_wave_start = false;
+  const char *routing_env = std::getenv("TENDON_HIP_ROUTING");
   if (const char *e = std::getenv("TENDON_HIP_EDGE_LANES")) { c->edge_lanes = std::max(1, std::min(tr_ctx::kMaxLanes, std::atoi(e))); c->edge_lanes_fixed = true; }
   if (const char *e = std::getenv("TENDON_HIP_EDGE_QUEUE")) { c->edge_queue = std::atoi(e) != 0; c->edge_queue_forced = c->edge_queue; }
   if (const char *e = std::getenv("TENDON_HIP_EDGE_QUEUE_WAVES")) { const int v = std::atoi(e); if (v >= 1 && v <= 8192) c->edge_queue_waves = v; }
@@ -907,6 +892,10 @@
   c->D.assign(rb->D, rb->D + (size_t)N * rb->n_m);
   c->max_tension.assign(rb->max_tension, rb->max_tension + N);
   for (int j = 0; j < N; j++) { K.min_len[j] = rb->min_length[j]; K.max_len[j] = rb->max_length[j]; }
+  {
+    const routing_form::Form rf = routing_form::classify(routing_spec(c), routing_env, TRK_K1_TWO_WAVE_MAXN);
+    K.routing_form = rf.form; K.helix_omega = rf.omega; K.helix_rho2 = rf.rho * rf.rho;
+  }
   {
     const double ro2 = rb->ro * rb->ro, ri2 = rb->ri * rb->ri;
     const double I = (1.0 / 4.0) * M_PI * (ro2 * ro2 - ri2 * ri2);
diff --git a/interactive-rate-tendons_amd/csrc/tr_types.hpp b/interactive-rate-tendons_amd/csrc/tr_types.hpp
--- a/interactive-rate-tendons_amd/csrc/tr_types.hpp
+++ b/interactive-rate-tendons_amd/csrc/tr_types.hpp
@@ -16,12 +16,15 @@
   double min_len[TRK_MAX_TENDONS];
   double max_len[TRK_MAX_TENDONS];
   double home_Li[TRK_MAX_TENDONS];
+  double helix_omega, helix_rho2;
   int32_t n_tendons, n_a, n_m;
   int32_t enable_rotation, enable_retraction;
   int32_t state_size;
   int32_t n_points;
-  int32_t pad_;
+  int32_t routing_form;
 };
+#define TRK_ROUTING_TABLE 0
+#define TRK_ROUTING_HELIX 1
 
 struct PolyK {
   double C[TRK_MAX_TENDONS][TRK_MAX_COEF];
diff --git a/interactive-rate-tendons_amd/csrc/verdict_kernel.hpp b/interactive-rate-tendons_amd/csrc/verdict_kernel.hpp
--- a/interactive-rate-tendons_amd/csrc/verdict_kernel.hpp
+++ b/interactive-rate-tendons_amd/csrc/verdict_kernel.hpp
@@ -478,7 +478,7 @@
 #ifndef TRK_VERDICT_TWO_WAVE_MAXN
 #define TRK_VERDICT_TWO_WAVE_MAXN 4
 #endif
-template <int N, bool ROT, bool SPH, bool SIG = false>
+template <int N, bool ROT, bool SPH, bool SIG = false, class Form = TableRouting>
 __global__ __launch_bounds__(64, (N <= TRK_VERDICT_TWO_WAVE_MAXN ? 2 : 1)) void fk_verdict(
     const double *__restrict__ states, int64_t n, RobotK K, const double *__restrict__ tab, const StepK *__restrict__ steps,
     int nsteps, double *__restrict__ tips, const VerdictArgs *__restrict__ va) {
@@ -498,7 +498,7 @@
 
   FkLane<N> fl_;
   FkOut out{nullptr, nullptr, nullptr, nullptr, nullptr, nullptr, nullptr, nullptr, nullptr, nullptr};
-  fk_uniform_body<N, ROT, false, false>(states, n, 0, K, tab, steps, nsteps, out, ps, nullptr, &fl_);
+  fk_uniform_body<N, ROT, false, false, Form>(states, n, 0, K, tab, steps, nsteps, out, ps, nullptr, &fl_);
 
   ps.template sig_finish<false>();
   ps.finish();
diff --git a/profiles/count_isa.py b/profiles/count_isa.py
--- a/profiles/count_isa.py
+++ b/profiles/count_isa.py
@@ -29,6 +29,19 @@
 }
 }
 template __global__ void trk::rk4_step_only<%d>(const double*, int64_t, int64_t, RobotK, const double*, const StepK*, int, trk::FkOut);
+'''
+
+_RK4_ONLY_HELIX = r'''
+#include <hip/hip_runtime.h>
+#include "tr_types.hpp"
+#include "fk_kernel.hpp"
+namespace trk {
+template <int N> __global__ __launch_bounds__(64, 2) void rk4_step_only_helix(const double *states, int64_t n, int64_t ld, RobotK K,
+                                                                               const double *tab, const StepK *steps, int nsteps, FkOut out) {
+  fk_uniform_body<N, false, false, false, UniformHelix>(states, n, ld, K, tab, steps, nsteps, out);
+}
+}
+template __global__ void trk::rk4_step_only_helix<%d>(const double*, int64_t, int64_t, RobotK, const double*, const StepK*, int, trk::FkOut);
 '''
 
 KERNELS = {
@@ -73,6 +86,21 @@
 #include "fk_kernel.hpp"
 template __global__ void trk::fk_rk4_batch_uniform<4, false, false>(const double*, int64_t, int64_t, RobotK,
                                                                      const double*, const StepK*, int, trk::FkOut);
+''',
+    "rk4_step_helix<3>": _RK4_ONLY_HELIX % 3,
+    "rk4_step_helix<4>": _RK4_ONLY_HELIX % 4,
+    "fk_verdict_helix<3,false>": r'''
+#include <hip/hip_runtime.h>
+#include "tr_types.hpp"
+#include "verdict_kernel.hpp"
+template __global__ void trk::fk_verdict<3, false, false, false, trk::UniformHelix>(const double*, int64_t, RobotK, const double*, const StepK*, int, double*, const trk::VerdictArgs*);
+''',
+    "fk_sweep_fused_helix<3,false>": r'''
+#include <hip/hip_runtime.h>
+#include "tr_types.hpp"
+#include "fused_kernel.hpp"
+template __global__ void trk::fk_sweep_fused<3, false, trk::UniformHelix>(const double*, int64_t, int64_t, RobotK, const double*, const StepK*, int,
+                                                                          trk::FkOut, const trk::FusedSweepArgs*);
 ''',
 }
 
diff --git a/profiles/kbench.hip b/profiles/kbench.hip
--- a/profiles/kbench.hip
+++ b/profiles/kbench.hip
@@ -18,6 +18,12 @@
 #ifndef KB_N
 #define KB_N 3
 #endif
+#ifdef KB_HELIX
+static_assert(KB_N == 3, "-DKB_HELIX: only the KB_N == 3 robot is a uniform helix");
+using KbForm = trk::UniformHelix;
+#else
+using KbForm = trk::TableRouting;
+#endif
 #ifndef KB_LOG2
 #define KB_LOG2 20
 #endif
@@ -33,7 +39,7 @@
                                                                            const double *__restrict__ tab, const StepK *__restrict__ steps,
                                                                            int nsteps, double *__restrict__ tips) {
   FkOut out{nullptr, nullptr, nullptr, nullptr, nullptr, nullptr, tips, nullptr, nullptr, nullptr};
-  fk_uniform_body<N, false, false, false>(states, n, 0, K, tab, steps, nsteps, out);
+  fk_uniform_body<N, false, false, false, KbForm>(states, n, 0, K, tab, steps, nsteps, out);
 }
 }
 
@@ -67,6 +73,9 @@
     const double ro2 = ro * ro, ri2 = ri * ri, I = 0.25 * M_PI * (ro2 * ro2 - ri2 * ri2), Ar = M_PI * (ro2 - ri2), J = 2 * I, G = E / (2 * (1 + nu));
     K.kb0 = E * I; K.kb2 = J * G; K.dkb = K.kb2 - K.kb0; K.ikb0 = 1 / K.kb0; K.ikb2 = 1 / K.kb2; K.ks0 = G * Ar; K.ks2 = E * Ar; K.iks0 = 1 / K.ks0; K.iks2 = 1 / K.ks2;
   }
+#ifdef KB_HELIX
+  K.routing_form = TRK_ROUTING_HELIX; K.helix_omega = C[0][1]; K.helix_rho2 = D[0][0] * D[0][0];
+#endif
   K.residual_threshold = 5e-6; K.radius = 0.015; K.L = L; K.dL = dL; K.n_tendons = N; K.n_a = 3; K.n_m = 3; K.state_size = N; K.n_points = 129;
   std::vector<StepK> steps;
   std::vector<double> tab((1 + 3 * 128) * N * 6);
@@ -114,7 +123,7 @@
   for (int r = 0; r < KB_REPS + 2; r++) {
     CK(hipEventRecord(a));
 #ifdef KB_VERDICT
-    hipLaunchKernelGGL((trk::fk_verdict<N, false, false, kSig>), dim3((unsigned)((n + 63) / 64)), dim3(64), lds, nullptr, d_st, n, K, d_tab, d_steps, 128, d_tips, d_va);
+    hipLaunchKernelGGL((trk::fk_verdict<N, false, false, kSig, KbForm>), dim3((unsigned)((n + 63) / 64)), dim3(64), lds, nullptr, d_st, n, K, d_tab, d_steps, 128, d_tips, d_va);
 #else
     hipLaunchKernelGGL((trk::rk4_only<N>), dim3((unsigned)((n + 63) / 64)), dim3(64), 0, nullptr, d_st, n, K, d_tab, d_steps, 128, d_tips);
 #endif
@@ -128,7 +137,7 @@
   std::sort(ms.begin(), ms.end());
   hipFuncAttributes fa;
 #ifdef KB_VERDICT
-  CK(hipFuncGetAttributes(&fa, (const void *)trk::fk_verdict<N, false, false, kSig>));
+  CK(hipFuncGetAttributes(&fa, (const void *)trk::fk_verdict<N, false, false, kSig, KbForm>));
   {
     std::vector<uint64_t> bits((size_t)((n + 63) / 64));
     CK(hipMemcpy(bits.data(), d_bits, bits.size() * 8, hipMemcpyDeviceToHost));
@@ -139,6 +148,11 @@
 #else
   CK(hipFuncGetAttributes(&fa, (const void *)trk::rk4_only<N>));
 #endif
+#ifdef KB_HELIX
+  std::printf("routing form: uniform helix   ");
+#else
+  std::printf("routing form: table   ");
+#endif
   std::printf("N=%d n=%ld (2^%d unless KB_COUNT) waves/SIMD<=%d: best %.3f ms  median %.3f ms  -> %.4g FK/s   regs %d  scratch %zu B   tips sum %.17g abs %.17g\n", N, (long)n, KB_LOG2, KB_WAVES,
               ms.front(), ms[ms.size() / 2], (double)n / (ms.front() * 1e-3), fa.numRegs, (size_t)fa.localSizeBytes, sum, asum);
   return 0;
```

New measurement: 143.7 million, median of 6. 1.02x the previous value.
